# csukuangfj/kaldi-hmm-gmm

Hardware: AMD Instinct MI355X
Metric: frames/sec (whole node) per EM iter (align+acc-stats), 5k-pdf x 64-Gauss (higher is better)
Workload: dtype f32 via f16x2s

## Files before the change

### include/khg_hip.h

```cpp
#ifndef KHG_HIP_H_
#define KHG_HIP_H_
#include <stdint.h>

#ifdef __cplusplus
extern "C" {
#endif

#define KHG_OK 0
#define KHG_E_ARG (-1)
#define KHG_E_HIP (-2)
#define KHG_E_RUNTIME (-3)
#define KHG_E_UNSUPPORTED (-4)
#define KHG_MAX_DIM 512

typedef struct khg_ctx khg_ctx;
typedef struct khg_model khg_model;
typedef struct khg_tm khg_tm;
typedef struct khg_utts khg_utts;
typedef struct khg_accs khg_accs;

const char *khg_last_error(void);
int khg_version(void);

int khg_ctx_create(int device, void *stream, khg_ctx **out);
int khg_ctx_destroy(khg_ctx *ctx);
int khg_ctx_sync(khg_ctx *ctx);
int khg_ctx_set_timing(khg_ctx *ctx, int on);
int khg_ctx_get_timings(khg_ctx *ctx, char *names, int64_t names_cap, float *ms, int32_t cap,
                        int32_t *n_out);

#define KHG_K1_AUTO 0
#define KHG_K1_FP32_PDF 2
#define KHG_K1_FP32_UTT 3
#define KHG_K1_F16X2 4
#define KHG_K1_F16X2S 5
int khg_ctx_set_k1_form(khg_ctx *ctx, int form);

#define KHG_OPT_K1_FORM 0
#define KHG_OPT_K1_ORDER 1
#define KHG_OPT_K1_NF 2
#define KHG_OPT_K1P_TS 3
#define KHG_OPT_K1_INTERLEAVE 4
#define KHG_OPT_K1_DBG 5
#define KHG_OPT_K2_INORDER 6
#define KHG_OPT_K2_KS 7
#define KHG_OPT_K2_SERIAL 8
#define KHG_OPT_K2_PROF 9
#define KHG_OPT_K3_BUCKET 10
#define KHG_OPT_K3_FORM 11
#define KHG_OPT_K3_PHASE_B 12
#define KHG_OPT_K3_NY 13
#define KHG_OPT_DEBUG 14
#define KHG_OPT_K3_PHASE_A 15
#define KHG_OPT_K2_SPLIT 16
#define KHG_OPT_K2S_HUB 17
#define KHG_OPT_LAT_OPS_LDS 18
#define KHG_OPT_K1_LAUNCH 19
#define KHG_OPT_K1_PGRID 20
#define KHG_OPT_K1_PROF 21
#define KHG_OPT_COUNT 22
#define KHG_INFO_SCRATCH_BYTES 100
#define KHG_INFO_SCRATCH_BLOCKS 101
int khg_ctx_set_option(khg_ctx *ctx, int option, int value);
int khg_ctx_get_option(const khg_ctx *ctx, int option, int *value);
int khg_option_check(int option, int value);
int khg_option_from_env(const char *name, const char *text, int *option, int *value);

int khg_model_create(khg_ctx *ctx, int32_t num_pdfs, int32_t dim, const int32_t *gauss_off_h,
                     const float *gconsts_h, const float *means_invvars_h,
                     const float *inv_vars_h, khg_model **out);
int khg_model_destroy(khg_model *m);
int khg_model_invalidate(khg_model *m);

int khg_tm_create(khg_ctx *ctx, int32_t num_tids, const int32_t *id2pdf_h, khg_tm **out);
int khg_tm_set_trans_cost(khg_tm *tm, const float *trans_cost_h);
int khg_tm_destroy(khg_tm *tm);

int khg_utts_create(khg_ctx *ctx, const khg_tm *tm, int32_t n_utt, int32_t dim,
                    const int64_t *frame_off_h, const float *feats_h, const float *feats_d,
                    const int64_t *state_off_h, const int32_t *start_h, const int64_t *arc_off_h,
                    const int32_t *ilabel_h, const int32_t *olabel_h, const float *weight_h,
                    const int32_t *nextstate_h, const float *final_h, khg_utts **out);
int khg_utts_destroy(khg_utts *u);
typedef struct khg_graph khg_graph;
int khg_graph_create(khg_ctx *ctx, const khg_tm *tm, int32_t num_states, int32_t start, const int64_t *arc_off_h,
                     const int32_t *ilabel_h, const int32_t *olabel_h, const float *weight_h,
                     const int32_t *nextstate_h, const float *final_h, khg_graph **out);
int khg_graph_destroy(khg_graph *g);
int khg_graph_info(const khg_graph *g, int64_t *num_states, int64_t *num_arcs, int32_t *num_pdfs,
                   int32_t *max_in_degree, int64_t *device_bytes);
int khg_utts_create_on_graph(khg_ctx *ctx, const khg_tm *tm, khg_graph *g, int32_t n_utt, int32_t dim,
                             const int64_t *frame_off_h, const float *feats_h, const float *feats_d, khg_utts **out);
int khg_utts_graph_bytes(const khg_utts *u, int64_t *bytes);
int khg_utts_num_pdfs(const khg_utts *u, int64_t *pdf_off_h );
int khg_utts_pdfs(const khg_utts *u, int32_t *pdfs_h );
int khg_utts_k2_plan(khg_ctx *ctx, const khg_utts *u, int32_t out[8]);
int khg_utts_pdf_first(const khg_utts *u, int32_t *first_h );

int khg_loglikes(khg_ctx *ctx, const khg_model *m, khg_utts *u);
int khg_loglikes_reachable(khg_ctx *ctx, const khg_model *m, khg_utts *u);
int khg_loglikes_band(khg_ctx *ctx, const khg_model *m, khg_utts *u);
int khg_utts_pdf_last(const khg_utts *u, int32_t *last_h );
int khg_loglikes_layout(const khg_utts *u, int64_t *ll_off_h, int64_t *total);
int khg_loglikes_download(khg_ctx *ctx, const khg_utts *u, float *ll_h);
int khg_loglikes_upload(khg_ctx *ctx, khg_utts *u, const float *ll_h);
int khg_utts_set_pdf_list(khg_utts *u, int32_t n, const int32_t *pdfs_h);
int khg_utts_features_changed(khg_utts *u);

typedef struct {
  float beam;
  float retry_beam;
  int32_t careful;
  float acoustic_scale;
  int32_t max_active;
  int32_t min_active;
  float beam_delta;
  float hash_ratio;
  float like_scale;
} khg_align_config;
void khg_align_config_default(khg_align_config *c);

#define KHG_ALIGN_DONE 0
#define KHG_ALIGN_ERROR 1
#define KHG_ALIGN_RETRIED 2
#define KHG_ALIGN_EXACT_DP 4
#define KHG_ALIGN_FALLBACK 8

int khg_careful_graph(int32_t num_states, int32_t start, const int64_t *arc_off_h, const int32_t *ilabel_h,
                      const int32_t *olabel_h, const float *weight_h, const int32_t *nextstate_h, const float *final_h,
                      int32_t *out_num_states, int32_t *out_start, int64_t *out_arc_off_h, int32_t *out_ilabel_h,
                      int32_t *out_olabel_h, float *out_weight_h, int32_t *out_nextstate_h, float *out_final_h);

int khg_align(khg_ctx *ctx, const khg_tm *tm, khg_utts *u, const khg_align_config *cfg,
              int32_t *ali_h, int32_t *words_h, int64_t *words_off_h, int64_t words_cap,
              float *like_h, int32_t *status_h);
int khg_ali_upload(khg_ctx *ctx, khg_utts *u, const int32_t *ali_h);
int khg_ali_download(khg_ctx *ctx, khg_utts *u, int32_t *ali_h);

typedef struct {
  float beam;
  int32_t max_active;
  int32_t min_active;
  float lattice_beam;
  int32_t prune_interval;
  float beam_delta;
  float hash_ratio;
  float prune_scale;
  float acoustic_scale;
  int32_t allow_partial;
  int32_t scratch_per_frame;
} khg_lattice_faster_config;
void khg_lattice_faster_config_default(khg_lattice_faster_config *c);

#define KHG_LAT_SUCCEEDED 1
#define KHG_LAT_PARTIAL 2
#define KHG_LAT_SCRATCH 4
#define KHG_LAT_NO_PATH 8
#define KHG_LAT_EPS_LOOP 16
#define KHG_LAT_WORDS 32
#define KHG_LAT_NO_TRACEBACK 64

int khg_decode_lattice_faster(khg_ctx *ctx, const khg_tm *tm, khg_utts *u, const khg_lattice_faster_config *cfg,
                              int32_t *ali_h, int32_t *words_h, int64_t *words_off_h, int64_t words_cap,
                              double *like_h, int32_t *status_h);

typedef struct {
  float beam;
  float lattice_beam;
  int32_t prune_interval;
  float prune_scale;
  float acoustic_scale;
  int32_t allow_partial;
  int32_t scratch_per_frame;
} khg_lattice_simple_config;
void khg_lattice_simple_config_default(khg_lattice_simple_config *c);

#define KHG_LAT_NO_EPS_TOKEN 128
#define KHG_LAT_NAN 256

// ... 296 lines not shown
```

### kaldi_hmm_gmm_amd/_lib.py

```python
import ctypes as C
import os

import numpy as np

_HERE = os.path.dirname(os.path.abspath(__file__))
LIB_PATH = os.environ.get("KHG_LIBRARY") or os.path.join(_HERE, "libkhg_hip.so")


class KhgError(RuntimeError):
    """Mirror of the reference's std::runtime_error -> Python RuntimeError (csrc/log.h:46-53)."""


def _load():
    if not os.path.exists(LIB_PATH):
        raise ImportError(
            f"{LIB_PATH} not found: build it with `python -c 'import __graft_entry__ as g; g.build()'` "
            "(hipcc --offload-arch=gfx950). kaldi_hmm_gmm_amd has no CPU fallback."
        )
    try:
        import torch
    except ImportError:
        pass
    return C.CDLL(LIB_PATH)

# ... 41 lines not shown
class LatticeSimpleConfigC(C.Structure):
    _fields_ = [
        ("beam", C.c_float),
        ("lattice_beam", C.c_float),
        ("prune_interval", C.c_int32),
        ("prune_scale", C.c_float),
        ("acoustic_scale", C.c_float),
        ("allow_partial", C.c_int32),
        ("scratch_per_frame", C.c_int32),
    ]


class MleOptionsC(C.Structure):
    _fields_ = [
        ("min_gaussian_weight", C.c_float),
        ("min_gaussian_occupancy", C.c_float),
        ("min_variance", C.c_double),
        ("remove_low_count_gaussians", C.c_int32),
        ("variance_floor_vector", C.POINTER(C.c_double)),
    ]


class EbwOptionsC(C.Structure):
    _fields_ = [("E", C.c_double), ("tau", C.c_double)]


class EbwWeightOptionsC(C.Structure):
    _fields_ = [("min_num_count_weight_update", C.c_double), ("min_gaussian_weight", C.c_double), ("tau", C.c_double)]


class EbwResultsC(C.Structure):
    _fields_ = [("auxf_impr_gauss", C.c_double), ("count", C.c_double), ("auxf_impr_weights", C.c_double), ("floored", C.c_int32),
                ("failed", C.c_int32), ("skipped", C.c_int32), ("weights_skipped", C.c_int32)]


class FmllrOptionsC(C.Structure):
    _fields_ = [("min_count", C.c_double), ("num_iters", C.c_int32)]


class MlltOptionsC(C.Structure):
    _fields_ = [("num_iters", C.c_int32)]


class LdaOptionsC(C.Structure):
    _fields_ = [("target_dim", C.c_int32), ("remove_offset", C.c_int32), ("within_class_factor", C.c_double)]


class RescoreStatsC(C.Structure):
    _fields_ = [("arcs", C.c_int64), ("emitting_arcs", C.c_int64), ("cells", C.c_int64)]


SIGNATURES = {
    "khg_last_error": (C.c_char_p, []),
    "khg_version": (C.c_int, []),
    "khg_ctx_create": (C.c_int, [C.c_int, vp, C.POINTER(vp)]),
    "khg_ctx_destroy": (C.c_int, [vp]),
    "khg_ctx_sync": (C.c_int, [vp]),
    "khg_ctx_set_timing": (C.c_int, [vp, C.c_int]),
    "khg_ctx_set_k1_form": (C.c_int, [vp, C.c_int]),
    "khg_ctx_set_option": (C.c_int, [vp, C.c_int, C.c_int]),
    "khg_ctx_get_option": (C.c_int, [vp, C.c_int, C.POINTER(C.c_int)]),
    "khg_option_check": (C.c_int, [C.c_int, C.c_int]),
    "khg_option_from_env": (C.c_int, [C.c_char_p, C.c_char_p, C.POINTER(C.c_int), C.POINTER(C.c_int)]),
    "khg_ctx_get_timings": (C.c_int, [vp, C.c_char_p, C.c_int64, c_f32p, C.c_int32, c_i32p]),
    "khg_model_create": (C.c_int, [vp, C.c_int32, C.c_int32, c_i32p, c_f32p, c_f32p, c_f32p, C.POINTER(vp)]),
    "khg_model_destroy": (C.c_int, [vp]),
    "khg_tm_create": (C.c_int, [vp, C.c_int32, c_i32p, C.POINTER(vp)]),
    "khg_tm_set_trans_cost": (C.c_int, [vp, c_f32p]),
    "khg_tm_destroy": (C.c_int, [vp]),
    "khg_utts_create": (
        C.c_int,
        [vp, vp, C.c_int32, C.c_int32, c_i64p, c_f32p, vp, c_i64p, c_i32p, c_i64p, c_i32p, c_i32p, c_f32p, c_i32p,
         c_f32p, C.POINTER(vp)],
    ),
    "khg_utts_destroy": (C.c_int, [vp]),
    "khg_graph_create": (C.c_int, [vp, vp, C.c_int32, C.c_int32, c_i64p, c_i32p, c_i32p, c_f32p, c_i32p, c_f32p, C.POINTER(vp)]),
    "khg_graph_destroy": (C.c_int, [vp]),
    "khg_graph_info": (C.c_int, [vp, c_i64p, c_i64p, c_i32p, c_i32p, c_i64p]),
    "khg_utts_create_on_graph": (C.c_int, [vp, vp, vp, C.c_int32, C.c_int32, c_i64p, c_f32p, vp, C.POINTER(vp)]),
    "khg_utts_graph_bytes": (C.c_int, [vp, c_i64p]),
    "khg_utts_num_pdfs": (C.c_int, [vp, c_i64p]),
    "khg_utts_pdfs": (C.c_int, [vp, c_i32p]),
    "khg_utts_k2_plan": (C.c_int, [vp, vp, c_i32p]),
    "khg_utts_pdf_first": (C.c_int, [vp, c_i32p]),
    "khg_loglikes": (C.c_int, [vp, vp, vp]),
    "khg_loglikes_reachable": (C.c_int, [vp, vp, vp]),
    "khg_loglikes_band": (C.c_int, [vp, vp, vp]),
    "khg_utts_pdf_last": (C.c_int, [vp, c_i32p]),
    "khg_loglikes_layout": (C.c_int, [vp, c_i64p, c_i64p]),
    "khg_loglikes_download": (C.c_int, [vp, vp, c_f32p]),
    "khg_loglikes_upload": (C.c_int, [vp, vp, c_f32p]),
    "khg_utts_set_pdf_list": (C.c_int, [vp, C.c_int32, c_i32p]),
    "khg_utts_features_changed": (C.c_int, [vp]),
    "khg_comm_info": (C.c_int, [vp, c_i32p, c_i32p, c_i32p]),
    "khg_align_config_default": (None, [C.POINTER(AlignConfigC)]),
    "khg_align": (C.c_int, [vp, vp, vp, C.POINTER(AlignConfigC), c_i32p, c_i32p, c_i64p, C.c_int64, c_f32p, c_i32p]),
    "khg_ali_upload": (C.c_int, [vp, vp, c_i32p]),
    "khg_lattice_faster_config_default": (None, [C.POINTER(LatticeFasterConfigC)]),
    "khg_decode_lattice_faster": (C.c_int, [vp, vp, vp, C.POINTER(LatticeFasterConfigC), c_i32p, c_i32p, c_i64p, C.c_int64, c_f64p,
                                            c_i32p]),
    "khg_lattice_simple_config_default": (None, [C.POINTER(LatticeSimpleConfigC)]),
    "khg_decode_lattice_simple": (C.c_int, [vp, vp, vp, C.POINTER(LatticeSimpleConfigC), c_i32p, c_i32p, c_i64p, C.c_int64, c_f64p,
                                            c_i32p, c_i32p]),
    "khg_decode_lattice_simple_raw": (C.c_int, [vp, vp, vp, C.POINTER(LatticeSimpleConfigC), c_i32p, c_i32p, c_i64p, C.c_int64, c_f64p,
                                                c_i32p, c_i32p, C.POINTER(vp)]),
    "khg_decode_lattice_faster_raw": (C.c_int, [vp, vp, vp, C.POINTER(LatticeFasterConfigC), c_i32p, c_i32p, c_i64p, C.c_int64, c_f64p,
                                                c_i32p, C.POINTER(vp)]),
    "khg_lattices_sizes": (C.c_int, [vp, c_i64p, c_i64p]),
    "khg_lattices_download": (C.c_int, [vp, vp, c_i32p, c_i32p, c_f32p, c_f32p, c_f32p, c_i32p, c_i32p, c_i32p, c_f32p, c_f32p, c_i32p,
                                        c_i32p]),
    "khg_lattices_device_bytes": (C.c_int, [vp, c_i64p]),
    "khg_lattices_destroy": (C.c_int, [vp]),
    "khg_lattices_validate": (C.c_int, [C.c_int32, c_i64p, c_i64p, c_i32p, c_i32p, c_f32p, c_f32p, c_f32p, c_i32p, c_i32p, c_i32p, c_f32p,
                                        c_f32p, c_i32p, c_i32p]),
    "khg_lattices_upload": (C.c_int, [vp, C.c_int32, c_i64p, c_i64p, c_i32p, c_i32p, c_f32p, c_f32p, c_f32p, c_i32p, c_i32p, c_i32p, c_f32p,
                                      c_f32p, c_i32p, c_i32p, C.POINTER(vp)]),
    "khg_lattices_num_utts": (C.c_int, [vp, c_i32p]),
    "khg_lattices_ali_layout": (C.c_int, [vp, vp, c_i64p]),
    "khg_lattices_num_chunks": (C.c_int, [vp, c_i32p]),
    "khg_lattices_chunk_utts": (C.c_int, [vp, c_i32p]),
    "khg_lattices_best_path": (C.c_int, [vp, vp, C.c_int32, c_f32p, c_f32p, c_i32p, c_i32p, c_i64p, C.c_int64, c_f32p, c_i32p]),
    "khg_lattices_prune": (C.c_int, [vp, vp, C.c_float, C.c_float, C.c_float, c_i32p, C.POINTER(vp)]),
    "khg_lattices_posteriors": (C.c_int, [vp, vp, C.c_float, C.c_float, c_i32p, c_f64p, C.POINTER(vp)]),
    "khg_lattices_rescore": (C.c_int, [vp, vp, vp, vp, vp, C.c_float, C.c_int, C.POINTER(RescoreStatsC), C.POINTER(vp)]),
    "khg_lattices_op_status": (C.c_int, [vp, c_i32p]),
    "khg_lattices_boost": (C.c_int, [vp, vp, C.c_int32, c_i32p, C.c_int32, c_i32p, c_i64p, c_i32p, vp, C.c_float, C.c_float, c_i32p,
                                     C.POINTER(vp)]),
    "khg_lattices_mpe_posteriors": (C.c_int, [vp, vp, C.c_int32, c_i32p, c_i32p, C.c_int32, c_i32p, c_i64p, c_i32p, vp, C.c_int32, C.c_int32,
                                              C.c_float, C.c_float, c_i32p, c_f64p, c_f64p, C.POINTER(vp)]),
    "khg_posteriors_sizes": (C.c_int, [vp, c_i64p, c_i64p]),
    "khg_posteriors_download": (C.c_int, [vp, vp, c_i64p, c_i32p, c_f64p, c_f64p]),
    "khg_posteriors_device_bytes": (C.c_int, [vp, c_i64p]),
    "khg_posteriors_destroy": (C.c_int, [vp]),
    "khg_posteriors_validate": (C.c_int, [C.c_int32, c_i64p, c_i64p, C.c_int64, c_i32p, c_f64p]),
    "khg_posteriors_upload": (C.c_int, [vp, C.c_int32, c_i64p, c_i64p, c_i32p, c_f64p, C.POINTER(vp)]),
    "khg_ali_download": (C.c_int, [vp, vp, c_i32p]),
    "khg_accs_create": (C.c_int, [vp, vp, vp, C.POINTER(vp)]),
    "khg_accs_destroy": (C.c_int, [vp]),
    "khg_accs_zero": (C.c_int, [vp, vp]),
    "khg_accs_size": (C.c_int, [vp, c_i64p]),
    "khg_accs_device_ptr": (C.c_int, [vp, C.POINTER(vp)]),
    "khg_accs_download": (C.c_int, [vp, vp, c_f64p]),
    "khg_accs_upload": (C.c_int, [vp, vp, c_f64p]),
    "khg_acc_stats": (C.c_int, [vp, vp, vp, vp, C.c_float, vp]),
    "khg_acc_stats_post": (C.c_int, [vp, vp, vp, vp, vp, C.c_float, vp]),
    "khg_acc_stats_post2": (C.c_int, [vp, vp, vp, vp, vp, C.c_float, vp, vp]),
    "khg_accs_add": (C.c_int, [vp, vp, C.c_float, vp]),
    "khg_accs_scale": (C.c_int, [vp, vp, C.c_float]),
    "khg_accs_smooth_with_accum": (C.c_int, [vp, vp, C.c_float, vp, vp, c_i32p]),
    "khg_accs_allreduce": (C.c_int, [vp, vp, vp]),
    "khg_accs_allreduce_range": (C.c_int, [vp, vp, vp, C.c_int32, C.c_int32, vp]),
    "khg_acc_stats_reduce": (C.c_int, [vp, vp, vp, vp, C.c_float, vp, vp, C.c_int32]),
    "khg_accs_allreduce_f32": (C.c_int, [vp, vp, vp]),
    "khg_comm_unique_id": (C.c_int, [vp]),
    "khg_comm_create": (C.c_int, [vp, C.c_int32, C.c_int32, vp, C.POINTER(vp)]),
    "khg_comm_destroy": (C.c_int, [vp]),
    "khg_compute_gconsts": (C.c_int, [C.c_int32, C.c_int32, c_i32p, c_f32p, c_f32p, c_f32p, c_f32p, c_i32p]),
    "khg_mle_options_default": (None, [C.POINTER(MleOptionsC)]),
    "khg_mle_am_diag_gmm_update": (
        C.c_int,
        [C.POINTER(MleOptionsC), C.c_int32, C.c_int32, c_i32p, c_f64p, c_f64p, c_f64p, C.c_uint16, C.c_uint16, c_f32p,
         c_f32p, c_f32p, c_f32p, c_i32p, c_f32p, c_f32p, c_i32p, c_i32p, c_i32p],
    ),
    "khg_ebw_options_default": (None, [C.POINTER(EbwOptionsC)]),
    "khg_ebw_weight_options_default": (None, [C.POINTER(EbwWeightOptionsC)]),
    "khg_ebw_am_diag_gmm_update": (
# ... 104 lines not shown
```

### kaldi_hmm_gmm_amd/csrc/khg_ctx_model.hip

```cpp
#include "khg_internal.hpp"

#include <mutex>
#include "khg_k1_loglikes.hip.inc"

static thread_local std::string g_err;
extern "C" const char* khg_last_error(void) { return g_err.c_str(); }
int khg_set_error(int code, const std::string& msg) { g_err = msg; return code; }
extern "C" int khg_version(void) { return 100; }

static std::mutex g_ctx_mu;
static std::vector<khg_ctx*> g_ctxs;
static constexpr size_t KHG_ARENA_BYTES = size_t(24) << 20;
void* arena_alloc(khg_ctx* ctx, size_t bytes) {
  KhgArena& a = ctx->arena;
  if (!a.dev) {
    if (a.cap == SIZE_MAX) return nullptr;
    void *d = nullptr, *h = nullptr;
    if (hipMalloc(&d, KHG_ARENA_BYTES) != hipSuccess || hipHostMalloc(&h, KHG_ARENA_BYTES, hipHostMallocDefault) != hipSuccess) {
      if (d) (void)hipFree(d);
      (void)hipGetLastError();
      a.cap = SIZE_MAX;
      return nullptr;
    }
    a.dev = static_cast<char*>(d); a.host = static_cast<char*>(h); a.cap = KHG_ARENA_BYTES; a.top = a.base = 256;
// ... 51 lines not shown
  return false;
}
void khg_dev_free(void* p) {
  if (p && !khg_arena_release(p)) (void)hipFree(p);
}

static void ctx_defaults_from_env(khg_ctx* c);
extern "C" int khg_ctx_create(int device, void* stream, khg_ctx** out) {
  if (!out) return khg_set_error(KHG_E_ARG, "khg_ctx_create: out is NULL");
  int n = 0;
  hipError_t e = hipGetDeviceCount(&n);
  if (e != hipSuccess || n <= 0)
    return khg_set_error(KHG_E_HIP, "khg_ctx_create: no HIP device available (this library has no CPU fallback)");
  if (device < 0 || device >= n) return khg_set_error(KHG_E_ARG, "khg_ctx_create: bad device index");
  HIPCHK(hipSetDevice(device));
  hipDeviceProp_t prop;
  HIPCHK(hipGetDeviceProperties(&prop, device));
  if (std::string(prop.gcnArchName).rfind("gfx950", 0) != 0)
    return khg_set_error(KHG_E_UNSUPPORTED, std::string("khg_ctx_create: built for gfx950, device is ") + prop.gcnArchName);
  khg_ctx* c = new khg_ctx();
  c->device = device;
  if (stream) { c->stream = (hipStream_t)stream; c->own_stream = false; }
  else { HIPCHK(hipStreamCreateWithFlags(&c->stream, hipStreamNonBlocking)); c->own_stream = true; }
  for (auto& s : c->sides) HIPCHK(hipStreamCreateWithFlags(&s, hipStreamNonBlocking));
  ctx_defaults_from_env(c);
  int rc = dev_alloc(&c->err_flag_d, 1);
  if (!rc) rc = dev_alloc(&c->dump_d, 256);
  if (!rc && hipHostMalloc(reinterpret_cast<void**>(&c->err_host), 256, hipHostMallocDefault) != hipSuccess) rc = khg_set_error(KHG_E_HIP, "khg_ctx_create: hipHostMalloc failed");
  if (rc) { delete c; return rc; }
  HIPCHK(hipMemsetAsync(c->err_flag_d, 0, sizeof(int32_t), c->stream));
  { std::lock_guard<std::mutex> lk(g_ctx_mu); g_ctxs.push_back(c); }
  *out = c;
  return KHG_OK;
}
extern "C" int khg_ctx_destroy(khg_ctx* c) {
  if (!c) return KHG_OK;
  (void)hipStreamSynchronize(c->stream);
  for (auto& s : c->sides) (void)hipStreamSynchronize(s);
  {
    std::lock_guard<std::mutex> lk(g_ctx_mu);
    g_ctxs.erase(std::remove(g_ctxs.begin(), g_ctxs.end(), c), g_ctxs.end());
    if (c->arena.dev && !c->arena.blocks.empty()) {
      c->arena.dirty.clear();
      g_orphans.push_back(std::move(c->arena));
      c->arena = KhgArena();
    }
  }
  DEVFREE(c->err_flag_d); DEVFREE(c->dump_d); DEVFREE(c->k1_next_d);
  if (c->err_host) (void)hipHostFree(c->err_host);
  if (c->arena.dev) (void)hipFree(c->arena.dev);
  if (c->arena.host) (void)hipHostFree(c->arena.host);
  if (c->own_stream) (void)hipStreamDestroy(c->stream);
  for (auto& s : c->sides) (void)hipStreamDestroy(s);
  if (c->comm_stream) { (void)hipStreamSynchronize(c->comm_stream); (void)hipStreamDestroy(c->comm_stream); }
  if (c->ev_k3) (void)hipEventDestroy(c->ev_k3);
  if (c->ev_c1) (void)hipEventDestroy(c->ev_c1);
  delete c;
  return KHG_OK;
}
extern "C" int khg_ctx_set_timing(khg_ctx* c, int on) {
  if (!c) return khg_set_error(KHG_E_ARG, "ctx is NULL");
  c->timing = on != 0;
  return KHG_OK;
}
extern "C" int khg_ctx_get_timings(khg_ctx* c, char* names, int64_t names_cap, float* ms, int32_t cap, int32_t* n_out) {
  if (!c || !n_out) return khg_set_error(KHG_E_ARG, "bad arguments");
  HIPCHK(hipStreamSynchronize(c->stream));
  for (auto& s : c->sides) HIPCHK(hipStreamSynchronize(s));
  int n = 0; std::string all;
  for (auto& t : c->timings) {
    float v = 0.0f;
    (void)hipEventElapsedTime(&v, t.e0, t.e1);
    if (n < cap && ms) ms[n] = v;
    all += t.name; all += '\n';
    (void)hipEventDestroy(t.e0); (void)hipEventDestroy(t.e1);
    ++n;
  }
  c->timings.clear();
  if (names && names_cap > 0) { size_t k = std::min<size_t>(all.size(), (size_t)names_cap - 1); memcpy(names, all.data(), k); names[k] = 0; }
  *n_out = n;
  return KHG_OK;
}
static const struct { int lo, hi; } k_opt_range[KHG_OPT_COUNT] = {
  {KHG_K1_AUTO, KHG_K1_F16X2S}, {0, 4}, {0, 6}, {0, 1 << 20}, {-1, 1}, {0, 255}, {0, 1}, {0, 4}, {0, 3}, {0, 1}, {0, 2}, {0, 2}, {0, 2}, {0, 64}, {0, 1}, {0, 1}, {0, 1}, {0, 1 << 20}, {0, 1}, {0, 2}, {0, 1 << 16}, {0, 1}};
extern "C" int khg_option_check(int opt, int value) {
  if (opt < 0 || opt >= KHG_OPT_COUNT) return khg_set_error(KHG_E_ARG, "khg_option_check: no such option");
  if (value < k_opt_range[opt].lo || value > k_opt_range[opt].hi || (opt == KHG_OPT_K1_FORM && value == 1))
    return khg_set_error(KHG_E_ARG, "khg_ctx_set_option: option " + std::to_string(opt) + " takes values " + std::to_string(k_opt_range[opt].lo) + " .. " + std::to_string(k_opt_range[opt].hi));
  return KHG_OK;
}
extern "C" int khg_ctx_set_option(khg_ctx* c, int opt, int value) {
  if (!c || opt < 0 || opt >= KHG_OPT_COUNT) return khg_set_error(KHG_E_ARG, "khg_ctx_set_option: bad arguments");
  int rc = khg_option_check(opt, value);
  if (rc) return rc;
  c->opt[opt] = value;
  return KHG_OK;
}
extern "C" int khg_ctx_get_option(const khg_ctx* c, int opt, int* value) {
  if (c && value && (opt == KHG_INFO_SCRATCH_BYTES || opt == KHG_INFO_SCRATCH_BLOCKS)) {
    *value = opt == KHG_INFO_SCRATCH_BYTES ? (c->arena.dev ? (int)c->arena.top : 0) : (int)c->arena.blocks.size();
    return KHG_OK;
  }
  if (!c || !value || opt < 0 || opt >= KHG_OPT_COUNT) return khg_set_error(KHG_E_ARG, "khg_ctx_get_option: bad arguments");
  *value = c->opt[opt];
  return KHG_OK;
}
extern "C" int khg_ctx_set_k1_form(khg_ctx* c, int form) { return khg_ctx_set_option(c, KHG_OPT_K1_FORM, form); }
static const struct { const char* name; int opt; const char* words; } k_env_tab[] = {
  {"KHG_K1", KHG_OPT_K1_FORM, "auto=0,pdf=2,fp32=2,utt=3,f16x2=4,f16x2s=5"},
  {"KHG_K1_ORDER", KHG_OPT_K1_ORDER, "desc=0,none=1,asc=2,tiles=3,xcd=4"},
  {"KHG_K1_NF", KHG_OPT_K1_NF, ""}, {"KHG_K1P_TS", KHG_OPT_K1P_TS, ""}, {"KHG_K1_INTERLEAVE", KHG_OPT_K1_INTERLEAVE, ""},
  {"KHG_K1B_DBG", KHG_OPT_K1_DBG, ""}, {"KHG_K2_INORDER", KHG_OPT_K2_INORDER, ""}, {"KHG_K2_KS", KHG_OPT_K2_KS, ""},
  {"KHG_K2_SERIAL", KHG_OPT_K2_SERIAL, ""}, {"KHG_K2_PROF", KHG_OPT_K2_PROF, ""},
  {"KHG_K3_BUCKET", KHG_OPT_K3_BUCKET, "sort=0,atomic=1,count=2"}, {"KHG_K3_FORM", KHG_OPT_K3_FORM, "auto=0,block=1,valu=2"},
  {"KHG_K3_VALU", KHG_OPT_K3_FORM, "1=2"}, {"KHG_K3_PHASEB", KHG_OPT_K3_PHASE_B, "f64=0,f32=1,f16=2"},
  {"KHG_K3_NY", KHG_OPT_K3_NY, ""}, {"KHG_DEBUG", KHG_OPT_DEBUG, ""}, {"KHG_K3_PHASEA", KHG_OPT_K3_PHASE_A, "auto=0,f16=0,f32=1"},
  {"KHG_K2_SPLIT", KHG_OPT_K2_SPLIT, "on=0,off=1"}, {"KHG_K2S_HUB", KHG_OPT_K2S_HUB, ""},
  {"KHG_LAT_OPS_LDS", KHG_OPT_LAT_OPS_LDS, "on=0,off=1"},
  {"KHG_K1_LAUNCH", KHG_OPT_K1_LAUNCH, "auto=0,chunk=1,persistent=2"}, {"KHG_K1_PGRID", KHG_OPT_K1_PGRID, ""},
  {"KHG_K1_PROF", KHG_OPT_K1_PROF, ""}};
extern "C" int khg_option_from_env(const char* name, const char* text, int* option, int* value) {
  if (!name || !text || !*text || !option || !value) return khg_set_error(KHG_E_ARG, "khg_option_from_env: bad arguments");
  for (const auto& t : k_env_tab) {
    if (strcmp(t.name, name) != 0) continue;
    const char* e = text;
    int v = atoi(e);
    bool word = false;
    for (const char* w = t.words; *w;) {
      const char* eq = strchr(w, '=');
      const size_t n = (size_t)(eq - w);
      if (strlen(e) == n && strncmp(e, w, n) == 0) { v = atoi(eq + 1); word = true; break; }
      const char* comma = strchr(eq, ',');
      if (!comma) break;
      w = comma + 1;
    }
    if (!word && *t.words && !(e[0] >= '0' && e[0] <= '9') && e[0] != '-')
      return khg_set_error(KHG_E_ARG, std::string(name) + ": unknown word '" + text + "'");
    if (v < k_opt_range[t.opt].lo || v > k_opt_range[t.opt].hi)
      return khg_set_error(KHG_E_ARG, std::string(name) + " takes values " + std::to_string(k_opt_range[t.opt].lo) + " .. " + std::to_string(k_opt_range[t.opt].hi));
    *option = t.opt; *value = v;
    return KHG_OK;
  }
  return khg_set_error(KHG_E_ARG, std::string("khg_option_from_env: no such variable: ") + name);
}
static void ctx_defaults_from_env(khg_ctx* c) {
  c->opt[KHG_OPT_K1_INTERLEAVE] = -1;
  c->opt[KHG_OPT_K1P_TS] = 1024;
  c->opt[KHG_OPT_K2S_HUB] = 32;
  c->opt[KHG_OPT_K3_PHASE_B] = 2;
  for (const auto& t : k_env_tab) {
    const char* e = getenv(t.name);
    if (!e || !*e) continue;
    int opt = 0, v = 0;
    if (khg_option_from_env(t.name, e, &opt, &v) == KHG_OK) c->opt[opt] = v;
  }
}
extern "C" int khg_ctx_sync(khg_ctx* c) {
  if (!c) return khg_set_error(KHG_E_ARG, "ctx is NULL");
  return check_err_flag(c, "khg_ctx_sync");
}
int check_err_flag(khg_ctx* c, const char* where) {
  { int rf = arena_flush(c); if (rf) return rf; }
  for (int i = 0; i < khg_ctx::NSIDE; ++i)
    if (c->side_dirty[i]) { HIPCHK(hipStreamSynchronize(c->sides[i])); c->side_dirty[i] = false; }
  HIPCHK(hipMemcpyAsync(c->err_host, c->err_flag_d, sizeof(int32_t), hipMemcpyDeviceToHost, c->stream));
  HIPCHK(hipStreamSynchronize(c->stream));
  c->pageable_pending = false;
  const int32_t f = *c->err_host;
  if (f) {
    HIPCHK(hipMemsetAsync(c->err_flag_d, 0, sizeof(int32_t), c->stream));
    if (f & 1) return khg_set_error(KHG_E_RUNTIME, std::string(where) + ": Invalid answer (overflow or invalid variances/features?)");
    if (f & 2) return khg_set_error(KHG_E_RUNTIME, std::string(where) + ": internal queue overflow in the faithful decoder");
    if (f & 8) return khg_set_error(KHG_E_RUNTIME, std::string(where) + ": internal error: K3 work items exceed their bound");
    return khg_set_error(KHG_E_RUNTIME, std::string(where) + ": pdf-id out of range (graph/model mismatch)");
  }
  return KHG_OK;
}

template <int KQ>
__global__ __launch_bounds__(256) void k0_pack_tiles(const float* __restrict__ gconsts, const float* __restrict__ miv,
                                                      const float* __restrict__ iv, const int32_t* __restrict__ gauss_off,
                                                      const int32_t* __restrict__ pdf_tile_off, const int32_t* __restrict__ tile_pdf,
                                                      int D, float* __restrict__ wimg, float* __restrict__ nhiv) {
  constexpr int ROW = khg_row_floats(KQ), TILE = khg_tile_floats(KQ);
  const int t = blockIdx.x, p = tile_pdf[t];
  const int g_first = gauss_off[p] + 32 * (t - pdf_tile_off[p]);
  const int nrow = min(32, gauss_off[p + 1] - g_first);
  float* img = wimg + (size_t)t * TILE;
  for (int i = threadIdx.x; i < TILE; i += 256) {
    float v = 0.0f;
    if (i < 4 * 32 * ROW) {
      const int q = i / (32 * ROW), r = (i / ROW) & 31, s = i % ROW;
      const int d = 2 * s + (q & 1);
      if (r < nrow && d < D) {
        const size_t src = (size_t)(g_first + r) * D + d;
        v = (q & 2) ? -0.5f * iv[src] : miv[src];
      }
    } else if (i < 4 * 32 * ROW + 32) {
      const int r = i - 4 * 32 * ROW;
      v = r < nrow ? gconsts[g_first + r] : -INFINITY;
    }
    img[i] = v;
  }
// ... 271 lines not shown
```

### kaldi_hmm_gmm_amd/csrc/khg_internal.hpp

```cpp
#pragma once
#include <hip/hip_runtime.h>

#include <algorithm>
#include <climits>
#include <cmath>
#include <cstdint>
#include <cstdio>
#include <cstdlib>
#include <cstring>
#include <deque>
#include <limits>
#include <string>
#include <type_traits>
#include <utility>
#include <vector>

#include "../../include/khg_hip.h"
#include "khg_dev_types.hip.inc"

int khg_set_error(int code, const std::string& msg);

#define HIPCHK(expr)                                                                         \
  do {                                                                                       \
    hipError_t e_ = (expr);                                                                  \
// ... 86 lines not shown
    for (auto& r : readers)
      if (r.first != s) HIPCHK(hipStreamWaitEvent(s, r.second, 0));
    return KHG_OK;
  }
  int after_pack(hipStream_t s) {
    if (!packed) HIPCHK(hipEventCreateWithFlags(&packed, hipEventDisableTiming));
    HIPCHK(hipEventRecord(packed, s));
    pack_stream = s;
    return KHG_OK;
  }
  int before_read(hipStream_t s) {
    if (packed && pack_stream != s) HIPCHK(hipStreamWaitEvent(s, packed, 0));
    return KHG_OK;
  }
  int after_read(hipStream_t s) {
    for (auto& r : readers)
      if (r.first == s) { HIPCHK(hipEventRecord(r.second, s)); return KHG_OK; }
    hipEvent_t e = nullptr;
    HIPCHK(hipEventCreateWithFlags(&e, hipEventDisableTiming));
    HIPCHK(hipEventRecord(e, s));
    readers.emplace_back(s, e);
    return KHG_OK;
  }
  void destroy() {
    if (packed) (void)hipEventDestroy(packed);
    for (auto& r : readers) (void)hipEventDestroy(r.second);
    packed = nullptr; readers.clear();
  }
};

struct khg_model {
  khg_ctx* ctx = nullptr;
  uint64_t serial = 0;
  uint64_t version = 0;
  int32_t P = 0, D = 0, KQ = 0, ntiles = 0;
  int64_t sumG = 0;
  std::vector<int32_t> gauss_off, pdf_tile_off;
  float* wimg_d = nullptr;
  int32_t* pdf_tile_off_d = nullptr;
  int32_t* gauss_off_d = nullptr;
  float *gconsts_d = nullptr, *miv_d = nullptr, *iv_d = nullptr, *nhiv_d = nullptr;
  float* weights_d = nullptr;
  bool has_weights = false;
  int32_t wimg_tiles = 0;
  int32_t KS = 0;
  char* wimgh_d = nullptr;
  int32_t wimgh_tiles = 0;
  std::vector<int32_t> wimgh_ex;
  ImgSync wimgh_sync;
  char* wimgs_d = nullptr;
  int32_t wimgs_tiles = 0;
  std::vector<int32_t> wimgs_key;
  float* ubound_d = nullptr; int32_t ubound_tiles = 0; bool ubound_valid = false;
  std::vector<int32_t> xs_ex_seen;
  ImgSync wimgs_sync;
  std::vector<float> wmax;
  std::vector<float> k3_xb;
  std::vector<float> k3_xb_raw;
  uint32_t* stats_d = nullptr;
  std::vector<int32_t> k3_ex;
  int32_t k3_S = 0;
  bool k3_f16_ok = false;
  int32_t* k3_ex_d = nullptr;
  float gcmax = 0.0f;
  int32_t* tile_pdf_d = nullptr;
  K4Res* k4_res_d = nullptr;
  int32_t k4_res_P = 0;
};

struct khg_tm {
  khg_ctx* ctx = nullptr;
  int32_t num_tids = 0, max_pdf = -1;
  std::vector<int32_t> id2pdf;
  int32_t* id2pdf_d = nullptr;
  float* trans_cost_d = nullptr;
  bool has_trans_cost = false;
};

struct khg_graph {
  khg_ctx* ctx = nullptr;
  int32_t refs = 1;
  int64_t S = 0, A = 0, nwords = 0, device_bytes = 0;
  int32_t start = -1, max_indeg = 0, max_outdeg = 0;
  bool same_col = true, has_eps = false;
  std::vector<int32_t> pdfs, pdf_first, pdf_dfin;
  int64_t *state_off_d = nullptr, *in_off_d = nullptr, *out_off_d = nullptr;
  int32_t *start_d = nullptr, *in_src_d = nullptr, *in_col_d = nullptr, *in_tid_d = nullptr, *in_olabel_d = nullptr, *out_inidx_d = nullptr;
  float *in_w_d = nullptr, *final_d = nullptr;
};
void khg_graph_release(khg_graph* g);

struct khg_utts {
  khg_ctx* ctx = nullptr;
  khg_graph* graph = nullptr;
  int32_t* gidx_d = nullptr;
  int64_t graph_bytes = 0;
  bool small = false;
  int32_t n_utt = 0, D = 0;
  int64_t N = 0;
  bool has_graphs = false;
  std::vector<int64_t> frame_off, state_off, pdf_off, ll_off, bp_off, path_off, words_off;
  std::vector<int32_t> pdfs;
  int32_t max_states = 0, max_inarcs = 0, max_indeg = 0, max_outdeg = 0;
  bool same_col = true;
  int32_t pdfs_checked_P = -1;
  bool has_eps = false;
  const float* feats_d = nullptr; bool own_feats = false;
  int64_t *frame_off_d = nullptr, *state_off_d = nullptr, *pdf_off_d = nullptr, *ll_off_d = nullptr;
  int32_t *pdfs_d = nullptr, *start_d = nullptr;
  KwChunk* wchunks_d = nullptr;
  int32_t n_wchunks = 0;
  int64_t *in_off_d = nullptr, *out_off_d = nullptr;
  int32_t *in_src_d = nullptr, *in_col_d = nullptr, *in_tid_d = nullptr, *in_olabel_d = nullptr, *out_inidx_d = nullptr;
  float *in_w_d = nullptr, *final_d = nullptr;
  K1Chunk* chunks_d = nullptr; int32_t n_chunks = 0; int32_t chunk_kq = 0;
  int64_t* tile_off_d = nullptr; int32_t* tiles_d = nullptr;
  std::vector<int32_t> pdf_first;
  std::vector<int32_t> pdf_last;
  int ll_mode = 0;
  void* band_args = nullptr;
  khg_model* band_model = nullptr; int band_ks = 0; size_t band_lds = 0; uint64_t band_serial = 0, band_version = 0; std::vector<int32_t> band_key;
  int tiles_reach = -1;
  std::vector<int32_t> tiles_pto;
  float* ll_d = nullptr; int64_t ll_total = 0; bool ll_valid = false;
  float* xpl_d = nullptr; int64_t* utt_xtile_off_d = nullptr; int32_t xpl_kq = 0;
  K1pEntry* p_ents_d = nullptr; K1pSlice* p_slices_d = nullptr; int32_t p_nslices = 0; int p_reach = -1; int32_t p_P = -1;
  int32_t p_grp[10] = {0, 0, 0, 0, 0, 0, 0, 0, 0, 0};
  std::vector<int32_t> p_goff;
  int64_t* utt_x32_off_d = nullptr;
  K1bChunk* bchunks_d = nullptr; int32_t n_bchunks = 0, bchunk_nt = 0;
  int32_t* x32_utt_d = nullptr; int64_t n_x32 = 0;
  k1b_u32x4* xh_d = nullptr; int32_t xh_ks = 0; std::vector<int32_t> xh_ex; int32_t* xh_ex_d = nullptr;
  std::vector<float> xmax;
  k1b_u32x4* xs_d = nullptr; int32_t xs_ks = 0; std::vector<int32_t> xs_ex; int32_t* xs_ex_d = nullptr;
  K1sChunk* schunks_d = nullptr; int32_t n_schunks = 0, schunk_nmax = 0;
  K1sUnit* sunits_d = nullptr; std::vector<int32_t> sunits_pto; int sunits_reach = -1;
  uint8_t* bp_d = nullptr; int64_t *bp_off_d = nullptr, *path_off_d = nullptr, *words_off_d = nullptr;
  double* layer_best_d = nullptr; int32_t* layer_cnt_d = nullptr; int32_t* path_d = nullptr;
  unsigned char* k2_gscratch_d = nullptr; size_t k2_gscratch_bytes = 0;
  int32_t* k2_order_d = nullptr;
  int32_t *ali_d = nullptr, *words_d = nullptr, *num_words_d = nullptr, *status_d = nullptr;
  float* like_d = nullptr;
  bool ali_valid = false;
  char* out_blk_d = nullptr; size_t out_blk_bytes = 0;
  hipEvent_t ev_dp = nullptr, ev_ali = nullptr;
  bool ali_pending = false;
  int32_t *ali2_d = nullptr, *unc_d = nullptr, *unc_cnt_h = nullptr, *unc_cnt_dev = nullptr;
  int64_t* sub_off_d = nullptr;
  bool ali_split = false;
  int32_t *pdf_count_d = nullptr, *pdf_cursor_d = nullptr, *frame_ids_d = nullptr;
  uint32_t *sort_keys_d = nullptr, *sort_keys_out_d = nullptr, *sort_vals_d = nullptr; void* sort_tmp_d = nullptr; size_t sort_tmp_bytes = 0;
  int32_t* cs_hist_d = nullptr; size_t cs_hist_n = 0; int64_t* cs_tot_d = nullptr; size_t cs_tot_n = 0;
  double *k3_part_d = nullptr, *k3_llpart_d = nullptr; size_t k3_part_n = 0, k3_llpart_n = 0;
  void* k3_items_d = nullptr; int32_t* k3_item_off_d = nullptr; size_t k3_items_n = 0, k3_item_off_n = 0;
  int64_t* pdf_start_d = nullptr; unsigned long long* tid_count_d = nullptr;
  int32_t k3_P = 0, k3_tids = 0;
  int32_t *pe_row_d = nullptr, *pe_tid_d = nullptr, *pe_ids_d = nullptr; float* pe_w_d = nullptr; size_t pe_cap = 0;
  uint32_t *pe_keys_d = nullptr, *pe_keys_out_d = nullptr, *pe_vals_d = nullptr; void* pe_tmp_d = nullptr; size_t pe_tmp_bytes = 0;
  int64_t* pe_start_d = nullptr; int32_t pe_P = 0;
  uint64_t *rc_keys_d = nullptr, *rc_keys_out_d = nullptr; uint32_t *rc_vals_d = nullptr, *rc_vals_out_d = nullptr;
  int32_t *rc_flag_d = nullptr, *rc_inc_d = nullptr, *rc_row_d = nullptr; float* rc_cell_d = nullptr; size_t rc_cap = 0;
  void* rc_tmp_d = nullptr; size_t rc_tmp_bytes = 0;
  int32_t *rc_cell_start_d = nullptr, *rc_item_off_d = nullptr; int64_t* rc_stats_d = nullptr; int32_t rc_P = -1;
};

static inline int64_t utt_states(const khg_utts* u, int i) { return u->graph ? u->state_off[1] : u->state_off[(size_t)i + 1] - u->state_off[(size_t)i]; }

struct khg_accs {
  khg_ctx* ctx = nullptr;
  int64_t sumG = 0; int32_t D = 0, num_tids = 0;
  int64_t n = 0, cap = 0;
  double* buf_d = nullptr;
  float* wire_d = nullptr; int64_t wire_cap = 0;
  double* occ() const { return buf_d; }
  double* mean() const { return buf_d + sumG; }
  double* var() const { return buf_d + sumG + sumG * D; }
  double* trans() const { return buf_d + sumG + 2 * sumG * D; }
  double* scalars() const { return trans() + num_tids + 1; }
};

constexpr size_t KHG_ARENA_MAX_REQ = size_t(4) << 20;
template <class T>
inline int u_alloc(khg_utts* u, T** p, size_t n) {
  if (n == 0) n = 1;
  if (u->small && n * sizeof(T) <= KHG_ARENA_MAX_REQ) {
    *p = static_cast<T*>(arena_alloc(u->ctx, n * sizeof(T)));
    if (*p) return KHG_OK;
// ... 49 lines not shown
```

### kaldi_hmm_gmm_amd/csrc/khg_k2.hip

```cpp
#include "khg_internal.hpp"

#include "khg_k2_hashlist.hip.inc"
#include "khg_k2_viterbi.hip.inc"

extern "C" void khg_align_config_default(khg_align_config* c) {
  c->beam = 200.0f; c->retry_beam = 0.0f; c->careful = 0; c->acoustic_scale = 1.0f;
  c->max_active = INT32_MAX; c->min_active = 20; c->beam_delta = 0.5f; c->hash_ratio = 2.0f;
  c->like_scale = 0.0f;
}

static int ensure_ali(khg_ctx* ctx, khg_utts* u) {
  if (u->ali_d) return KHG_OK;
  if (u->small && u->has_graphs) {
    const size_t nu = (size_t)u->n_utt, nw = (size_t)u->words_off[u->n_utt];
    const size_t bytes = 4 * (3 * nu + nw + (size_t)u->N) + 64;
    int rc = u_alloc(u, &u->out_blk_d, bytes);
    if (rc) return rc;
    u->out_blk_bytes = bytes;
    int32_t* p = reinterpret_cast<int32_t*>(u->out_blk_d);
    u->status_d = p; u->like_d = reinterpret_cast<float*>(p + nu); u->num_words_d = p + 2 * nu; u->words_d = p + 3 * nu; u->ali_d = p + 3 * nu + nw;
    return KHG_OK;
  }
  return u_alloc(u, &u->ali_d, (size_t)u->N);
}

struct K2Plan {
  int KS = 1, DEG = 1;
  bool FAST = false, GMEM = false, SC = false;
  int nthr = 64;
  size_t lds_dp = 0;
  size_t max_npdf = 0;
  int faithful = 0;
  int odeg_w = 0, odeg_c = 1;
  size_t lds_f = 0, lds_w_mut = 0, lds_w_graph = 0, lds_chain = 0;
  size_t gscratch_stride = 0;
};

static K2Plan k2_plan(const khg_ctx* ctx, const khg_utts* u) {
  K2Plan p;
  const size_t S = (size_t)u->max_states, A = (size_t)u->max_inarcs;
  size_t max_npdf = 0;
  for (int i = 0; i < u->n_utt; ++i) max_npdf = std::max<size_t>(max_npdf, (size_t)(u->pdf_off[i + 1] - u->pdf_off[i]));
  p.max_npdf = max_npdf;
  int nthr = (int)std::min<size_t>(1024, (S + 63) / 64 * 64);
  const int ks_force = ctx->opt[KHG_OPT_K2_KS];
  if (ks_force == 2 || ks_force == 4) nthr = (int)std::min<size_t>(1024, ((S + ks_force - 1) / ks_force + 63) / 64 * 64);
  p.nthr = nthr;
  const size_t nwave = nthr / 64;
  const bool deg6 = !u->has_eps && u->max_indeg > 3 && u->max_indeg <= 6 && S <= 1024;
  const bool fast = deg6 || (!u->has_eps && u->max_indeg <= 3 && S <= 4096);
  const int KSsel = !fast ? 0 : ((ks_force == 2 || ks_force == 4) && !deg6 && S <= (size_t)1024 * ks_force ? ks_force : (S <= 1024 ? 1 : (S <= 2048 ? 2 : 4)));
  const size_t NSl = fast ? KSsel : 1;
  const size_t tb_bytes = fast ? std::max<size_t>(5 * (size_t)nthr * NSl * 4, 2560 * nwave) : (K2_FB + 1) * ((S + 15) & ~size_t(15));
  size_t lds_dp = 16 * S + 8 * K2_MAXW + 8 * A + 4 * (S + 1) + 8 * K2_FB * nwave + 32 + 8 * K2_MAXW + 16 +
                  std::max<size_t>(fast ? 0 : 4 * K2_SB * (max_npdf | 1), tb_bytes) + 64;
  size_t HB = std::max<size_t>(2 * S, 1000);
  const size_t lds_f = 32 * S + 8 * HB + 4 * (S + A) + 4 * S + 4 * (S + 1) + 16 * A + A + 64;
  const int odeg_w = u->max_outdeg <= 8 ? std::max(1, (int)u->max_outdeg) : 0;
  const bool use_pos = u->has_eps || S > 1000;
  const size_t lds_w_mut = 16 * S + 8 * S + 4 * 4 * S + 4 * S + 4 * max_npdf + (odeg_w ? 0 : 4 * A + 4 * S) + (use_pos ? 4 * S : 0) +
                           (u->has_eps ? 4 * (S + A + 1) : 0) + 8 + 8 * ((std::max(A, S * (size_t)odeg_w) + 63) / 64 + 1);
  const size_t lds_w_graph = 8 * (S + 1) + 5 * 4 * A + (u->has_eps ? 4 * (S + 1) + 4 * A : 0) + A + S + 64;
  const int fmode = ctx->opt[KHG_OPT_K2_SERIAL];
  const int odeg_c = (int)std::max<int32_t>(1, u->max_outdeg);
  const size_t S4 = (S + 3) & ~size_t(3);
  const size_t lds_chain = std::max<size_t>(36 * S4 + 21 * S4 * (size_t)odeg_c + 4 * max_npdf,
                                            4 * (S4 + 1) + 2 * A + 16 + 9 * ((S + 15) & ~size_t(15))) + 128;
  const bool chain = fmode == 0 && !u->has_eps && S <= 1000 && u->max_outdeg <= 4 && lds_chain <= 64 * 1024 && max_npdf <= 32767;
  const bool wave_lds = (fmode == 0 || fmode == 3) && S <= 65535 && lds_w_mut + lds_w_graph <= 160 * 1024;
  const bool wave_gm = fmode != 1 && !wave_lds && S <= 65535 && lds_w_mut <= 160 * 1024;
  const bool lane_gm = !wave_lds && !wave_gm && lds_f > 160 * 1024;
  p.faithful = chain ? 4 : wave_gm ? 3 : wave_lds ? 2 : lane_gm ? 1 : 0;
  p.odeg_w = odeg_w; p.odeg_c = odeg_c;
  p.lds_f = lds_f; p.lds_w_mut = lds_w_mut; p.lds_w_graph = lds_w_graph; p.lds_chain = lds_chain;
  const bool gmem = lds_dp > 160 * 1024;
  if (gmem)
    lds_dp = 16 * S + 8 * K2_MAXW + 8 * A + 4 * (S + 1) + 8 * K2_FB * nwave + 32 + 8 * K2_MAXW + 16 +
             std::max<size_t>(4 * K2_SB * (max_npdf | 1), (K2_FB + 1) * ((S + 15) & ~size_t(15))) + 64;
  p.lds_dp = lds_dp;
  if (gmem || wave_gm || lane_gm)
    p.gscratch_stride = (std::max(gmem ? lds_dp : 0, std::max(wave_gm ? lds_w_graph : 0, lane_gm ? lds_f : 0)) + 255) & ~size_t(255);
  if (gmem) { p.GMEM = true; return p; }
  const bool deg2 = fast && !deg6 && KSsel == 1 && u->max_indeg <= 2 && ctx->opt[KHG_OPT_K2_KS] != 3;
  const bool sc2 = deg2 && u->same_col;
  const bool sc3 = fast && !deg6 && !deg2 && KSsel == 1 && u->same_col && ctx->opt[KHG_OPT_K2_KS] != 3;
  const bool deg2m = fast && !deg6 && KSsel > 1 && u->max_indeg <= 2;
  auto form = [&](int ks, int deg, bool sc) { p.KS = ks; p.DEG = deg; p.FAST = true; p.SC = sc; };
  if (deg6) form(1, 6, false);
  else if (sc2) form(1, 2, true);
  else if (deg2) form(1, 2, false);
  else if (sc3) form(1, 3, true);
  else if (KSsel == 1) form(1, 3, false);
  else if (KSsel == 2 && deg2m && u->same_col) form(2, 2, true);
  else if (KSsel == 2 && deg2m) form(2, 2, false);
  else if (KSsel == 2) form(2, 3, false);
  else if (KSsel == 4 && deg2m && u->same_col) form(4, 2, true);
  else if (KSsel == 4 && deg2m) form(4, 2, false);
  else if (KSsel == 4) form(4, 3, false);
  return p;
}

extern "C" int khg_utts_k2_plan(khg_ctx* ctx, const khg_utts* u, int32_t out[8]) {
  if (ctx_dead(ctx) || !u || !out) return khg_set_error(KHG_E_ARG, "khg_utts_k2_plan: bad arguments");
  { int rf = utts_foreign_ctx(ctx, u, "khg_utts_k2_plan"); if (rf) return rf; }
  if (!u->has_graphs) return khg_set_error(KHG_E_ARG, "khg_utts_k2_plan: the utterance set has no decoding graphs");
  const K2Plan p = k2_plan(ctx, u);
  out[0] = p.KS; out[1] = p.DEG; out[2] = p.FAST ? 1 : 0; out[3] = p.GMEM ? 1 : 0; out[4] = p.SC ? 1 : 0;
  out[5] = p.nthr; out[6] = p.GMEM ? 0 : (int32_t)p.lds_dp; out[7] = p.faithful;
  return KHG_OK;
}

extern "C" int khg_align(khg_ctx* ctx, const khg_tm* tm, khg_utts* u, const khg_align_config* cfg,
                         int32_t* ali_h, int32_t* words_h, int64_t* words_off_h, int64_t words_cap,
                         float* like_h, int32_t* status_h) {
  if (ctx_dead(ctx) || !tm || !u || !cfg) return khg_set_error(KHG_E_ARG, "khg_align: bad arguments");
  { int rf = utts_foreign_ctx(ctx, u, "khg_align"); if (rf) return rf; }
  if (!u->has_graphs) return khg_set_error(KHG_E_ARG, "khg_align: the utterance set has no decoding graphs");
  if (!u->ll_valid) return khg_set_error(KHG_E_ARG, "khg_align: call khg_loglikes first");
  if (u->max_states > 65535)
    return khg_set_error(KHG_E_UNSUPPORTED, "khg_align: more than 65535 states in one decoding graph (" + std::to_string(u->max_states) + "); the aligner's limit");
  if (u->max_indeg > 254)
    return khg_set_error(KHG_E_UNSUPPORTED, "khg_align: a state has more than 254 incoming arcs (" + std::to_string(u->max_indeg) + "); the aligner's limit");
  if ((cfg->retry_beam != 0 && cfg->retry_beam <= cfg->beam) || cfg->beam <= 0.0)
    return khg_set_error(KHG_E_RUNTIME, "Beams do not make sense: beam " + std::to_string(cfg->beam) + ", retry-beam " + std::to_string(cfg->retry_beam));
  if (!(cfg->hash_ratio >= 1.0) || !(cfg->max_active > 1) || !(cfg->min_active >= 0 && cfg->min_active < cfg->max_active))
    return khg_set_error(KHG_E_RUNTIME, "FasterDecoderOptions assertion failed");
  int rc = wait_ali(ctx, u);
  if (!rc) rc = k1_band_check(ctx, u);
  if (!rc) rc = ensure_ali(ctx, u);
  if (rc) return rc;
  if (!u->bp_d) {
    rc = u_alloc(u, &u->bp_d, (size_t)u->bp_off[u->n_utt]);
    if (!rc) rc = u_alloc(u, &u->layer_best_d, (size_t)(u->N + u->n_utt));
    if (!rc) rc = u_alloc(u, &u->layer_cnt_d, (size_t)(u->N + u->n_utt));
    if (!rc) rc = u_alloc(u, &u->path_d, (size_t)u->path_off[u->n_utt]);
    if (!rc && !u->out_blk_d) {
      rc = u_alloc(u, &u->words_d, (size_t)u->words_off[u->n_utt]);
      if (!rc) rc = u_alloc(u, &u->num_words_d, (size_t)u->n_utt);
      if (!rc) rc = u_alloc(u, &u->status_d, (size_t)u->n_utt);
      if (!rc) rc = u_alloc(u, &u->like_d, (size_t)u->n_utt);
    }
    if (rc) return rc;
  }
  rc = arena_flush(ctx);
  if (rc) return rc;
  HIPCHK(hipMemsetAsync(u->ali_d, 0, sizeof(int32_t) * (size_t)u->N, ctx->stream));
  K2Args a;
  a.frame_off = u->frame_off_d; a.gidx = u->gidx_d; a.state_off = u->state_off_d; a.start = u->start_d;
  a.in_off = u->in_off_d; a.in_src = u->in_src_d; a.in_col = u->in_col_d; a.in_tid = u->in_tid_d;
  a.in_olabel = u->in_olabel_d; a.in_w = u->in_w_d; a.out_off = u->out_off_d; a.out_inidx = u->out_inidx_d;
  a.final_w = u->final_d; a.trans_cost = tm->has_trans_cost ? tm->trans_cost_d : nullptr;
  a.ll = u->ll_d; a.ll_off = u->ll_off_d;
  a.bp = u->bp_d; a.bp_off = u->bp_off_d; a.layer_best = u->layer_best_d; a.layer_cnt = u->layer_cnt_d;
  a.path = u->path_d; a.path_off = u->path_off_d;
  a.ali = u->ali_d; a.ali_fb = u->ali_d; a.unc = nullptr; a.unc_cnt = nullptr; a.words = u->words_d; a.words_off = u->words_off_d; a.num_words = u->num_words_d;
  a.like = u->like_d; a.status = u->status_d; a.err_flag = ctx->err_flag_d;
  a.prof = nullptr;
  if (!u->k2_order_d && u->n_utt > 1) {
    std::vector<int32_t> ord((size_t)u->n_utt);
    for (int i = 0; i < u->n_utt; ++i) ord[(size_t)i] = i;
    std::stable_sort(ord.begin(), ord.end(), [&](int32_t x, int32_t y) {
      return u->frame_off[x + 1] - u->frame_off[x] > u->frame_off[y + 1] - u->frame_off[y];
    });
    int rc2 = u_upload(ctx, u, &u->k2_order_d, ord);
    if (!rc2) rc2 = sync_pageable(ctx);
    if (rc2) return rc2;
  }
  a.order = ctx->opt[KHG_OPT_K2_INORDER] ? nullptr : u->k2_order_d;
  const bool split = !(ali_h || like_h || status_h || words_h) && u->n_utt > 64 && !u->small && ctx->opt[KHG_OPT_K2_SPLIT] == 0;
  if (split) {
    if (!u->ali2_d) {
      rc = u_alloc(u, &u->ali2_d, (size_t)u->N);
      if (!rc) rc = u_alloc(u, &u->unc_d, (size_t)u->n_utt + 2);
      if (rc) return rc;
      u->unc_cnt_dev = u->unc_d + u->n_utt;
      HIPCHK(hipHostMalloc(reinterpret_cast<void**>(&u->unc_cnt_h), 64, 0));
    }
    HIPCHK(hipMemsetAsync(u->unc_d, 0, sizeof(int32_t) * ((size_t)u->n_utt + 2), ctx->stream));
    a.ali_fb = u->ali2_d; a.unc = u->unc_d; a.unc_cnt = u->unc_cnt_dev;
  }
  const bool k2prof = ctx->opt[KHG_OPT_K2_PROF] != 0;
  if (k2prof) { HIPCHK(hipMalloc(reinterpret_cast<void**>(&a.prof), sizeof(long long) * 16 * (size_t)u->n_utt)); HIPCHK(hipMemset(a.prof, 0, sizeof(long long) * 16 * (size_t)u->n_utt)); }
  a.beam = cfg->beam; a.retry_beam = cfg->retry_beam; a.acoustic_scale = cfg->acoustic_scale;
  a.like_scale = cfg->like_scale != 0.0f ? cfg->like_scale : cfg->acoustic_scale;
  a.beam_delta = cfg->beam_delta; a.hash_ratio = cfg->hash_ratio;
  a.max_active = cfg->max_active; a.min_active = cfg->min_active;
  a.max_states = u->max_states; a.max_inarcs = u->max_inarcs;
  const K2Plan plan = k2_plan(ctx, u);
  const int nthr = plan.nthr;
  const size_t lds_dp = plan.lds_dp, max_npdf = plan.max_npdf;
  a.gscratch = nullptr; a.gscratch_stride = 0;
  if (plan.gscratch_stride) {
    const size_t need = plan.gscratch_stride * (size_t)u->n_utt;
    if (need > u->k2_gscratch_bytes) {
      DEVFREE(u->k2_gscratch_d);
      { int rg = u_alloc(u, &u->k2_gscratch_d, need); if (rg) return rg; }
      u->k2_gscratch_bytes = need;
    }
    a.gscratch = u->k2_gscratch_d; a.gscratch_stride = (int64_t)plan.gscratch_stride;
  }
  if (plan.GMEM) {
    KernelTimer kt(ctx, "k2_viterbi_dp");
    KHG_LAUNCH(ctx, (k2_viterbi_dp<1, 1, false, true>), dim3(u->n_utt), dim3(nthr), 0, ctx->stream, a);
  } else {
    const int form = plan.FAST ? 100 * plan.KS + 10 * plan.DEG + (plan.SC ? 1 : 0) : 0;
#define K2_DP_CASES(X)                                                                                         \
    if (form == 160) X((k2_viterbi_dp<1, 6, true>));                                                           \
    else if (form == 121) X((k2_viterbi_dp<1, 2, true, false, true>));                                         \
    else if (form == 120) X((k2_viterbi_dp<1, 2, true>));                                                      \
    else if (form == 131) X((k2_viterbi_dp<1, 3, true, false, true>));                                         \
    else if (form == 130) X((k2_viterbi_dp<1, 3, true>));                                                      \
    else if (form == 221) X((k2_viterbi_dp<2, 2, true, false, true>));                                         \
    else if (form == 220) X((k2_viterbi_dp<2, 2, true>));                                                      \
    else if (form == 230) X((k2_viterbi_dp<2, 3, true>));                                                      \
    else if (form == 421) X((k2_viterbi_dp<4, 2, true, false, true>));                                         \
    else if (form == 420) X((k2_viterbi_dp<4, 2, true>));                                                      \
    else if (form == 430) X((k2_viterbi_dp<4, 3, true>));                                                      \
    else X((k2_viterbi_dp<1, 1, false>));
#define K2_SET_LDS(FN) HIPCHK(hipFuncSetAttribute((const void*)FN, hipFuncAttributeMaxDynamicSharedMemorySize, (int)lds_dp))
#define K2_LAUNCH(FN) KHG_LAUNCH(ctx, FN, dim3(u->n_utt), dim3(nthr), lds_dp, ctx->stream, a)
    if (lds_dp > 48 * 1024) { K2_DP_CASES(K2_SET_LDS) }
    KernelTimer kt(ctx, "k2_viterbi_dp");
    K2_DP_CASES(K2_LAUNCH)
#undef K2_LAUNCH
#undef K2_SET_LDS
#undef K2_DP_CASES
  }
  HIPCHK(hipGetLastError());
  const bool sync_call = ali_h || like_h || status_h || words_h;
  hipStream_t side = ctx->stream;
  if (!sync_call) {
    if (!u->ev_dp) { HIPCHK(hipEventCreateWithFlags(&u->ev_dp, hipEventDisableTiming)); HIPCHK(hipEventCreateWithFlags(&u->ev_ali, hipEventDisableTiming)); }
    if (split) HIPCHK(hipMemcpyAsync(u->unc_cnt_h, u->unc_cnt_dev, 2 * sizeof(int32_t), hipMemcpyDeviceToHost, ctx->stream));
    HIPCHK(hipEventRecord(u->ev_dp, ctx->stream));
    side = ctx->sides[ctx->next_side];
    ctx->side_dirty[ctx->next_side] = true;
    ctx->next_side = (ctx->next_side + 1) % khg_ctx::NSIDE;
    HIPCHK(hipStreamWaitEvent(side, u->ev_dp, 0));
  }
  rc = k1_band_repair(ctx, u, u->status_d, K2_ST_NEED_FALLBACK, side);
  if (rc) return rc;
  {
    KernelTimer kt(ctx, "k2_viterbi_faithful", side);
    if (plan.faithful == 4) {
#define K2_CHAIN(OD)                                                                                                            \
  do {                                                                                                                          \
    if (plan.lds_chain > 48 * 1024) HIPCHK(hipFuncSetAttribute((const void*)k2_viterbi_faithful_chain<OD>, hipFuncAttributeMaxDynamicSharedMemorySize, (int)plan.lds_chain)); \
    KHG_LAUNCH(ctx, k2_viterbi_faithful_chain<OD>, dim3(u->n_utt), dim3(64), plan.lds_chain, side, a, (int)max_npdf);                \
  } while (0)
      switch (plan.odeg_c) { case 1: K2_CHAIN(1); break; case 2: K2_CHAIN(2); break; case 3: K2_CHAIN(3); break; default: K2_CHAIN(4); break; }
#undef K2_CHAIN
    } else if (plan.faithful == 3) {
      if (plan.lds_w_mut > 48 * 1024) HIPCHK(hipFuncSetAttribute((const void*)k2_viterbi_faithful_wave<true>, hipFuncAttributeMaxDynamicSharedMemorySize, (int)plan.lds_w_mut));
      KHG_LAUNCH(ctx, k2_viterbi_faithful_wave<true>, dim3(u->n_utt), dim3(64), plan.lds_w_mut, side, a, u->has_eps ? 1 : 0, plan.odeg_w, (int)max_npdf);
    } else if (plan.faithful == 2) {
      const size_t lds_w = plan.lds_w_mut + plan.lds_w_graph;
      if (lds_w > 48 * 1024) HIPCHK(hipFuncSetAttribute((const void*)k2_viterbi_faithful_wave<false>, hipFuncAttributeMaxDynamicSharedMemorySize, (int)lds_w));
      KHG_LAUNCH(ctx, k2_viterbi_faithful_wave<false>, dim3(u->n_utt), dim3(64), lds_w, side, a, u->has_eps ? 1 : 0, plan.odeg_w, (int)max_npdf);
    } else if (plan.faithful == 1) {
      KHG_LAUNCH(ctx, k2_viterbi_faithful<true>, dim3(u->n_utt), dim3(64), 0, side, a);
    } else {
      if (plan.lds_f > 48 * 1024) HIPCHK(hipFuncSetAttribute((const void*)k2_viterbi_faithful<false>, hipFuncAttributeMaxDynamicSharedMemorySize, (int)plan.lds_f));
      KHG_LAUNCH(ctx, k2_viterbi_faithful<false>, dim3(u->n_utt), dim3(64), plan.lds_f, side, a);
    }
  }
  HIPCHK(hipGetLastError());
  if (!sync_call) { HIPCHK(hipEventRecord(u->ev_ali, side)); u->ali_pending = true; }
  u->ali_split = split;
  u->ali_valid = true;
  if (k2prof) {
    std::vector<long long> pr(16 * (size_t)u->n_utt);
    HIPCHK(hipStreamSynchronize(ctx->stream));
    HIPCHK(hipStreamSynchronize(side));
    HIPCHK(hipMemcpy(pr.data(), a.prof, pr.size() * 8, hipMemcpyDeviceToHost));
    (void)hipFree(a.prof);
    double ph[4] = {0, 0, 0, 0}, sT = 0, sS = 0, sf = 0; int n = 0;
    for (int i = 0; i < u->n_utt; ++i) if (pr[i * 8 + 4]) { for (int k = 0; k < 4; ++k) ph[k] += (double)(pr[i * 8 + k + 1] - pr[i * 8 + k]); sT += pr[i * 8 + 5]; sS += pr[i * 8 + 6]; sf += pr[i * 8 + 7]; ++n; }
    if (n) fprintf(stderr, "[KHG_K2_PROF] %d utts, avg T %.1f S %.1f fast %.2f threads %d lds %zu | ticks: setup %.0f forward %.0f traceback %.0f replay %.0f\n",
                   n, sT / n, sS / n, sf / n, nthr, lds_dp, ph[0] / n, ph[1] / n, ph[2] / n, ph[3] / n);
    const long long* pc = pr.data() + 8 * (size_t)u->n_utt;
    double cs[3] = {0, 0, 0}, cf = 0, cp[3] = {0, 0, 0}; int nc = 0;
    for (int i = 0; i < u->n_utt; ++i) if (pc[i * 8 + 3]) { for (int k = 0; k < 3; ++k) { cs[k] += (double)(pc[i * 8 + k + 1] - pc[i * 8 + k]); cp[k] += (double)pc[i * 8 + 5 + k]; } cf += (double)pc[i * 8 + 4]; ++nc; }
    if (nc) fprintf(stderr, "[KHG_K2_PROF] chain decoder: %d utts, avg frames decoded %.1f | ticks: setup %.0f frames %.0f (%.1f per frame: GetCutoff %.1f, pass 1 %.1f, pass 2 %.1f, rest = row flush + score staging) finish %.0f\n",
                    nc, cf / nc, cs[0] / nc, cs[1] / nc, cs[1] / std::max(1.0, cf), cp[0] / std::max(1.0, cf), cp[1] / std::max(1.0, cf), cp[2] / std::max(1.0, cf), cs[2] / nc);
  }
  if (!ali_h && !like_h && !status_h && !words_h) return KHG_OK;
  rc = wait_ali(ctx, u);
  if (rc) return rc;
  if (u->out_blk_d && ctx->arena.owns(u->out_blk_d)) {
    char* hm = ctx->arena.mirror(u->out_blk_d);
// ... 76 lines not shown
```

### kaldi_hmm_gmm_amd/csrc/khg_k2_viterbi.hip.inc

```

struct K2Args {
  const int64_t* frame_off;
  const int32_t* gidx;
  const int64_t* state_off;
  const int32_t* start;
  const int64_t* in_off;
  const int32_t* in_src;
  const int32_t* in_col;
  const int32_t* in_tid;
  const int32_t* in_olabel;
  const float* in_w;
  const int64_t* out_off;
  const int32_t* out_inidx;
  const float* final_w;
  const float* trans_cost;
  const float* ll;
  const int64_t* ll_off;
  uint8_t* bp;
  const int64_t* bp_off;
  double* layer_best;
  int32_t* layer_cnt;
  int32_t* path;
  const int64_t* path_off;
  int32_t* ali;
// ... 54 lines not shown
    if (n >= path_cap) { overflow = true; break; }
    path[n++] = ai;
    if (s_col[ai] >= 0) --layer;
    s = s_src[ai];
  }
  if (overflow || layer != 0) return KHG_ALIGN_ERROR;

  double cost = 0.0;
  float v1 = 0.0f, v2 = 0.0f;
  int t = 0, nw = 0;
  const int64_t wcap = a.words_off[u + 1] - a.words_off[u];
  int32_t* words = a.words + a.words_off[u];
  bool ok = true;
  const double beam = (double)a.beam;
  auto node_ok = [&](double c, int L) {
    if (c < lbest[L] + beam) return true;
    return lcnt[L] <= a.min_active && (L == 0 || lcnt[L - 1] <= a.min_active);
  };
  if (certify) ok = node_ok(0.0, 0);
  for (int i = n - 1; i >= 0; --i) {
    int ai = path[i];
    float w = s_w[ai];
    double ncost;
    int col = s_col[ai];
    if (col >= 0) {
      float ac = -1 * (a.acoustic_scale * llu[(int64_t)col * tpad + t]);
      ncost = (cost + w) + ac;
      a.ali_fb[f0 + t] = a.in_tid[in0 + ai];
      ++t;
    } else {
      ncost = cost + w;
    }
    float tot_cost = (float)(ncost - cost);
    float ac_cost = tot_cost - w;
    v1 = w + v1;
    v2 = ac_cost + v2;
    int ol = a.in_olabel[in0 + ai];
    if (ol != 0) { if (nw < wcap) words[nw] = ol; ++nw; }
    cost = ncost;
    if (certify && ok) ok = node_ok(cost, t);
  }
  v1 = a.final_w[a.state_off[a.gidx[u]] + best_state] + v1;
  v2 = 0.0f + v2;
  a.num_words[u] = nw;
  a.like[u] = -(v1 + v2) / a.like_scale;
  if (certified) *certified = ok;
  if (nw > wcap) return KHG_ALIGN_ERROR;
  return KHG_ALIGN_DONE;
}

struct K2Arc { uint16_t src; int16_t col; float w; };

#define K2_FB 32
#define K2_SB 16
#define K2_MAXW 16

__device__ __forceinline__ void k2_lds_sync() {
  asm volatile("s_waitcnt lgkmcnt(0)" ::: "memory");
  __builtin_amdgcn_wave_barrier();
}
__device__ __forceinline__ void k2_block_sync() {
  asm volatile("s_waitcnt lgkmcnt(0)\n\ts_barrier" ::: "memory");
}
__device__ __forceinline__ void k2_global_sync() {
  asm volatile("s_waitcnt vmcnt(0) lgkmcnt(0)" ::: "memory");
  __builtin_amdgcn_wave_barrier();
}
__device__ __forceinline__ float k2_wave_minf_lane63(float v) {
  asm volatile("s_nop 1\n\t"
               "v_min_f32_dpp %0, %0, %0 row_ror:8 row_mask:0xf bank_mask:0xf\n\ts_nop 1\n\t"
               "v_min_f32_dpp %0, %0, %0 row_ror:4 row_mask:0xf bank_mask:0xf\n\ts_nop 1\n\t"
               "v_min_f32_dpp %0, %0, %0 row_ror:2 row_mask:0xf bank_mask:0xf\n\ts_nop 1\n\t"
               "v_min_f32_dpp %0, %0, %0 row_ror:1 row_mask:0xf bank_mask:0xf\n\ts_nop 1\n\t"
               "v_min_f32_dpp %0, %0, %0 row_bcast:15 row_mask:0xa bank_mask:0xf\n\ts_nop 1\n\t"
               "v_min_f32_dpp %0, %0, %0 row_bcast:31 row_mask:0xc bank_mask:0xf\n\ts_nop 1"
               : "+v"(v));
  return v;
}
__device__ __forceinline__ double k2_wave_min(double v) {
#pragma unroll
  for (int o = 32; o > 0; o >>= 1) { double t = __shfl_xor(v, o); v = t < v ? t : v; }
  return v;
}
__device__ __forceinline__ int k2_wave_sum(int v) {
#pragma unroll
  for (int o = 32; o > 0; o >>= 1) v += __shfl_xor(v, o);
  return v;
}
__device__ __forceinline__ float k2_round_down(double d) {
  float f = (float)d;
  if ((double)f > d) f = __int_as_float(__float_as_int(f) + (f > 0.0f ? -1 : (f < 0.0f ? 1 : (int)0x80000001)));
  return f;
}

template <int DEG, int NB>
__device__ __forceinline__ void k2_decode_nibble(int nib, int& ord, int& tie) {
  if constexpr (DEG == 2) { ord = (nib & 1) ? 0 : ((nib & 2) ? 1 : (1 << NB) - 1); tie = (nib & 3) == 3 ? 1 : 0; }
  else { ord = nib & ((1 << NB) - 1); tie = (nib >> NB) & 1; }
}

template <int KS, int DEG, bool FAST, bool GMEM = false, bool SC = false>
__global__ __attribute__((amdgpu_waves_per_eu(KS == 1 ? K2_WAVES_PER_EU : 4))) void k2_viterbi_dp(K2Args a) {
  extern __shared__ __attribute__((aligned(16))) unsigned char k2_lds[];
  unsigned char* const smem = GMEM ? a.gscratch + (size_t)blockIdx.x * a.gscratch_stride : k2_lds;
  constexpr int NS = FAST ? KS : 1;
  constexpr int NSD = FAST ? KS * DEG : 1;
  constexpr int NB = DEG <= 3 ? 2 : 3;
  constexpr int BNONE = (1 << NB) - 1;
  const int u = a.order ? a.order[blockIdx.x] : (int)blockIdx.x;
  const int tid = threadIdx.x, lane = tid & 63;
  const int nthr = min((int)blockDim.x, max(64, (((int)(a.state_off[a.gidx[u] + 1] - a.state_off[a.gidx[u]]) + (FAST ? KS : 1) - 1) / (FAST ? KS : 1) + 63) & ~63));
  if (tid >= nthr) return;
  const int wave = __builtin_amdgcn_readfirstlane(tid >> 6), nwave = nthr >> 6;
  const int64_t f0 = a.frame_off[u];
  const int T = (int)(a.frame_off[u + 1] - f0);
  const int tpad = (T + 31) & ~31;
  const int64_t s0 = a.state_off[a.gidx[u]];
  const int S = (int)(a.state_off[a.gidx[u] + 1] - s0);
  const int64_t in0 = a.in_off[s0];
  const int A = (int)(a.in_off[s0 + S] - in0);
  const int start = a.start[a.gidx[u]];
  const int npdf = (int)((a.ll_off[u + 1] - a.ll_off[u]) / (tpad > 0 ? tpad : 1));
  const int PP = npdf | 1;
  const int Sp = (S + 15) & ~15;
  const int GW = FAST ? nthr * KS : 0;
  const int LB = Sp;

  double* cur = reinterpret_cast<double*>(smem);
  double* nxt = cur + a.max_states;
  double* s_red = nxt + a.max_states;
  K2Arc* s_arc = reinterpret_cast<K2Arc*>(s_red + K2_MAXW);
  int32_t* s_in_off = reinterpret_cast<int32_t*>(s_arc + a.max_inarcs);
  float* s_wmin = reinterpret_cast<float*>(s_in_off + a.max_states + 1);
  int32_t* s_wcnt = reinterpret_cast<int32_t*>(s_wmin + K2_FB * nwave);
  int32_t* s_flags = s_wcnt + K2_FB * nwave;
  int32_t* s_redi = s_flags + 8;
  float* s_ac = reinterpret_cast<float*>(smem + (((reinterpret_cast<unsigned char*>(s_redi + 2 * K2_MAXW) - smem) + 15) & ~ptrdiff_t(15)));
  uint8_t* s_bp = reinterpret_cast<uint8_t*>(s_ac);

  if (tid == 0) { a.num_words[u] = 0; a.like[u] = 0.0f; }
  if (start < 0 || S == 0) {
    if (tid == 0) a.status[u] = KHG_ALIGN_ERROR;
    return;
  }
  if (a.prof && tid == 0) a.prof[u * 8 + 0] = clock64();
  if (tid < 8) s_flags[tid] = 0;
  for (int s = tid; s <= S; s += nthr) s_in_off[s] = (int32_t)(a.in_off[s0 + s] - in0);
  k2_block_sync();
  for (int i = tid; i < A; i += nthr) {
    int col = a.in_col[in0 + i];
    int tidl = a.in_tid[in0 + i];
    float w = a.in_w[in0 + i];
    if (a.trans_cost && tidl >= 1) w = w + a.trans_cost[tidl];
    s_arc[i] = K2Arc{(uint16_t)a.in_src[in0 + i], (int16_t)col, w};
    if (col < 0) s_flags[1] = 1;
  }
  for (int s = tid; s < S; s += nthr) cur[s] = (s == start) ? 0.0 : INFINITY;
  k2_block_sync();
  const bool has_eps = !FAST && s_flags[1] != 0;
  const float* llu = a.ll + a.ll_off[u];
  uint8_t* bp = a.bp + a.bp_off[u];
  double* lbest = a.layer_best + f0 + u;
  int32_t* lcnt = a.layer_cnt + f0 + u;

  int e_src[NSD], e_col[NSD];
  double e_w[NSD];
  const bool have_ll = npdf > 0 && T > 0;
  if (FAST) {
#pragma unroll
    for (int k = 0; k < NS; ++k) {
      const int sk = tid + nthr * k;
      const int ib = sk < S ? s_in_off[sk] : 0, ie = sk < S ? s_in_off[sk + 1] : 0;
#pragma unroll
      for (int j = 0; j < DEG; ++j) {
        const bool v = ib + j < ie;
        K2Arc ar = s_arc[v ? ib + j : 0];
        e_src[k * DEG + j] = v ? ar.src : 0;
        e_col[k * DEG + j] = v ? ar.col : 0;
        e_w[k * DEG + j] = v ? (double)ar.w : (double)INFINITY;
      }
    }
  } else {
    for (int s = tid; s < S; s += nthr) bp[s] = K2_BP_NONE;
  }
  if (a.prof && tid == 0) a.prof[u * 8 + 1] = clock64();
  int tie = 0;
  const double* g_even[NSD]; const double* g_odd[NSD];
  double* st_even[NS]; double* st_odd[NS];
#pragma unroll
  for (int i = 0; i < NSD; ++i) { g_even[i] = cur + (FAST ? e_src[i] : 0); g_odd[i] = nxt + (FAST ? e_src[i] : 0); }
#pragma unroll
  for (int k = 0; k < NS; ++k) { const int sk = min(tid + nthr * k, S > 0 ? S - 1 : 0); st_even[k] = nxt + sk; st_odd[k] = cur + sk; }
  double mine[NS];
  unsigned bpw[NS];
#pragma unroll
  for (int k = 0; k < NS; ++k) bpw[k] = 0u;
#pragma unroll
  for (int k = 0; k < NS; ++k) mine[k] = (tid + nthr * k == start) ? 0.0 : INFINITY;
  int mine_live[NS];
#pragma unroll
  for (int k = 0; k < NS; ++k) mine_live[k] = (tid + nthr * k == start) ? 1 : 0;
  constexpr int NSC = SC ? (FAST ? KS : 1) : NSD;
  f32x4 sc_a[NSC], sc_b[NSC];
  constexpr bool SC3 = FAST && NSC == 1;
  f32x4 sc_c[NSC];
  if (FAST) {
#pragma unroll
    for (int i = 0; i < NSC; ++i) {
      sc_a[i] = have_ll ? *reinterpret_cast<const f32x4*>(llu + (int64_t)e_col[SC ? i * DEG : i] * tpad) : f32x4{0, 0, 0, 0};
      sc_b[i] = f32x4{0, 0, 0, 0};
      sc_c[i] = (SC3 && have_ll) ? *reinterpret_cast<const f32x4*>(llu + (int64_t)e_col[SC ? i * DEG : i] * tpad + 4) : f32x4{0, 0, 0, 0};
    }
  }

  auto layer_step = [&](const int layer, auto subc) -> bool {
    constexpr int SUB8 = decltype(subc)::value;
    constexpr int SUB = SUB8 & 3;
    uint8_t* bpl = bp + (int64_t)layer * Sp;
    if (has_eps) {
      for (int it = 0; it <= S + 1; ++it) {
        if (tid == 0) s_flags[2] = 0;
        k2_block_sync();
        for (int s = tid; s < S; s += nthr) {
          double best = cur[s];
          int barg = -1;
          for (int i = s_in_off[s]; i < s_in_off[s + 1]; ++i) {
            K2Arc ar = s_arc[i];
            if (ar.col >= 0) continue;
            double c = cur[ar.src];
            if (c == INFINITY) continue;
            double nw = c + ar.w;
            if (nw < best) { best = nw; barg = i - s_in_off[s]; }
            else if (nw == best && (barg >= 0 ? barg : (int)bpl[s]) != i - s_in_off[s]) tie = 1;
          }
          nxt[s] = best;
          if (barg >= 0) { bpl[s] = (uint8_t)barg; s_flags[2] = 1; }
        }
        k2_block_sync();
        for (int s = tid; s < S; s += nthr) cur[s] = nxt[s];
        const int changed = s_flags[2];
        k2_block_sync();
        if (!changed) break;
      }
    }
    {
      double lm = INFINITY;
      int lc = 0;
      if (FAST) {
#pragma unroll
        for (int k = 0; k < NS; ++k) { lc += mine_live[k]; lm = k == 0 ? mine[0] : (mine[k] < lm ? mine[k] : lm); }
      } else {
        for (int s = tid; s < S; s += nthr) { double c = cur[s]; if (c != INFINITY) { ++lc; if (c < lm) lm = c; } }
      }
      const int slot = layer & (K2_FB - 1);
      if constexpr (FAST) {
        float* pm = s_ac + wave * 640;
        uint8_t* pc = reinterpret_cast<uint8_t*>(pm + 512);
        pm[(layer & 7) * 64 + lane] = (float)lm;
        pc[(layer & 7) * 64 + lane] = (uint8_t)lc;
        if ((layer & 7) == 7 || layer == T) {
          k2_lds_sync();
          const int ly = lane >> 3, sub = lane & 7;
          const f32x4 m0 = *reinterpret_cast<const f32x4*>(pm + ly * 64 + sub * 8), m1 = *reinterpret_cast<const f32x4*>(pm + ly * 64 + sub * 8 + 4);
          const uint2 cb = *reinterpret_cast<const uint2*>(pc + ly * 64 + sub * 8);
          auto vmin = [](float x, float y) { float r; asm("v_min_f32 %0, %1, %2" : "=v"(r) : "v"(x), "v"(y)); return r; };
          float m = vmin(vmin(vmin(m0[0], m0[1]), vmin(m0[2], m0[3])), vmin(vmin(m1[0], m1[1]), vmin(m1[2], m1[3])));
          int cn = (int)__builtin_amdgcn_sad_u8(cb.y, 0u, __builtin_amdgcn_sad_u8(cb.x, 0u, 0u));
          m = vmin(m, __int_as_float(__builtin_amdgcn_update_dpp(0, __float_as_int(m), 0xB1, 0xf, 0xf, false)));
          cn += __builtin_amdgcn_update_dpp(0, cn, 0xB1, 0xf, 0xf, false);
          m = vmin(m, __int_as_float(__builtin_amdgcn_update_dpp(0, __float_as_int(m), 0x4E, 0xf, 0xf, false)));
          cn += __builtin_amdgcn_update_dpp(0, cn, 0x4E, 0xf, 0xf, false);
          m = vmin(m, __int_as_float(__builtin_amdgcn_update_dpp(0, __float_as_int(m), 0x141, 0xf, 0xf, false)));
          cn += __builtin_amdgcn_update_dpp(0, cn, 0x141, 0xf, 0xf, false);
          if (sub == 0 && ly <= (layer & 7)) {
            const int sl = (layer & ~7 & (K2_FB - 1)) + ly;
            s_wmin[sl * nwave + wave] = m; s_wcnt[sl * nwave + wave] = cn;
          }
          k2_lds_sync();
        }
      } else {
        const float wm = k2_wave_minf_lane63((float)lm);
        const int wc = k2_wave_sum(lc);
        if (lane == 63) { s_wmin[slot * nwave + wave] = wm; s_wcnt[slot * nwave + wave] = wc; }
      }
      if (slot == K2_FB - 1 || layer == T) {
        k2_block_sync();
        if (tid <= slot) {
          float m = INFINITY; int cn = 0;
          for (int w2 = 0; w2 < nwave; ++w2) { m = fminf(m, s_wmin[tid * nwave + w2]); cn += s_wcnt[tid * nwave + w2]; }
          if (m == INFINITY) { if (cn > 0) m = 3.402823466e38f; }
          else m = __int_as_float(__float_as_int(m) + (m > 0.0f ? -1 : (m < 0.0f ? 1 : (int)0x80000001)));
          lbest[layer - slot + tid] = (double)m;
          lcnt[layer - slot + tid] = cn;
        }
      }
    }
    if (layer == T) return false;
    if (FAST) {
      if constexpr (SC3) {
        if constexpr (SUB8 == 0) {
#pragma unroll
          for (int i = 0; i < NSC; ++i) sc_b[i] = sc_c[i];
        }
        if constexpr (SUB8 == 4) {
#pragma unroll
          for (int i = 0; i < NSC; ++i)
            if (have_ll && layer + 4 < tpad) {
              const float* src = llu + (int64_t)e_col[SC ? i * DEG : i] * tpad + layer + 4;
              sc_a[i] = *reinterpret_cast<const f32x4*>(src);
              sc_c[i] = *reinterpret_cast<const f32x4*>(src + 4);
            }
        }
      } else if (SUB == 0) {
#pragma unroll
        for (int i = 0; i < NSC; ++i)
          if (have_ll && layer + 4 < tpad) {
            const f32x4 v = *reinterpret_cast<const f32x4*>(llu + (int64_t)e_col[SC ? i * DEG : i] * tpad + layer + 4);
            if constexpr ((SUB8 & 4) != 0) sc_a[i] = v; else sc_b[i] = v;
          }
      }
      double cc[NSD];
#pragma unroll
      for (int i = 0; i < NSD; ++i) cc[i] = (SUB & 1) ? *g_odd[i] : *g_even[i];
#pragma unroll
      for (int k = 0; k < NS; ++k) {
        double nwv[DEG];
#pragma unroll
        for (int j = 0; j < DEG; ++j) {
          const int i = k * DEG + j;
          const int si = SC ? k : i;
          float sc;
          if constexpr ((SUB8 & 4) != 0) sc = sc_b[si][SUB]; else sc = sc_a[si][SUB];
          const float ac = -1 * (a.acoustic_scale * sc);
          nwv[j] = (cc[i] + e_w[i]) + ac;
        }
        double best = INFINITY;
#pragma unroll
        for (int j = 0; j < DEG; ++j) best = __builtin_fmin(best, nwv[j]);
        const bool live = __double2hiint(best) != 0x7FF00000;
        int code;
        if constexpr (DEG == 2) {
          const bool e0 = live && nwv[0] == best, e1 = live && nwv[1] == best;
          code = (e0 ? 1 : 0) | (e1 ? 2 : 0);
        } else {
          int barg = BNONE, neq = 0;
#pragma unroll
          for (int j = DEG - 1; j >= 0; --j) {
            const bool e = nwv[j] == best;
            barg = e ? j : barg;
            neq += e ? 1 : 0;
          }
          barg = live ? barg : BNONE;
          const int ctie = (live && neq > 1) ? 1 : 0;
          code = barg | (ctie << NB);
        }
        const int sk = tid + nthr * k;
        if (sk < S) *((SUB & 1) ? st_odd[k] : st_even[k]) = best;
        mine[k] = best;
        mine_live[k] = live ? 1 : 0;
        bpw[k] = (bpw[k] >> 4) | ((unsigned)code << 28);
        const int lb = layer + 1;
        if ((lb & 7) == 7 || lb == T) {
          const unsigned wv = (lb & 7) == 7 ? bpw[k] : bpw[k] >> (4 * (7 - (lb & 7)));
          reinterpret_cast<unsigned*>(bp)[(int64_t)(lb >> 3) * GW + sk] = wv;
        }
      }
    } else {
      if ((layer & (K2_SB - 1)) == 0) {
        k2_block_sync();
        const int tt = tid & (K2_SB - 1), hh = tid / K2_SB, nh = nthr / K2_SB;
        for (int c0 = 0; c0 < npdf; c0 += 8 * nh) {
          float v[8];
#pragma unroll
          for (int k = 0; k < 8; ++k) {
            const int col = c0 + nh * k + hh;
            v[k] = col < npdf ? llu[(int64_t)col * tpad + layer + tt] : 0.0f;
          }
#pragma unroll
          for (int k = 0; k < 8; ++k) {
            const int col = c0 + nh * k + hh;
            if (col < npdf) s_ac[tt * PP + col] = -1 * (a.acoustic_scale * v[k]);
          }
        }
        k2_block_sync();
      }
      const float* acr = s_ac + (layer & (K2_SB - 1)) * PP;
      uint8_t* bpn = bp + (int64_t)(layer + 1) * Sp;
      for (int s = tid; s < S; s += nthr) {
        double best = INFINITY;
        int barg = K2_BP_NONE;
        const int ib = s_in_off[s], ie = s_in_off[s + 1];
        for (int i = ib; i < ie; ++i) {
          K2Arc ar = s_arc[i];
          if (ar.col < 0) continue;
          double c = cur[ar.src];
          if (c == INFINITY) continue;
          double nw = (c + ar.w) + acr[ar.col];
          if (nw < best) { best = nw; barg = i - ib; }
          else if (nw == best) tie = 1;
        }
        nxt[s] = best;
        bpn[s] = (uint8_t)barg;
      }
    }
    k2_block_sync();
    double* tsw = cur; cur = nxt; nxt = tsw;
    return true;
  };
  if constexpr (FAST) {
    for (int base = 0; base <= T; base += 8) {
      if (!layer_step(base, std::integral_constant<int, 0>{})) break;
      if (!layer_step(base + 1, std::integral_constant<int, 1>{})) break;
      if (!layer_step(base + 2, std::integral_constant<int, 2>{})) break;
      if (!layer_step(base + 3, std::integral_constant<int, 3>{})) break;
      if (!layer_step(base + 4, std::integral_constant<int, 4>{})) break;
      if (!layer_step(base + 5, std::integral_constant<int, 5>{})) break;
      if (!layer_step(base + 6, std::integral_constant<int, 6>{})) break;
      if (!layer_step(base + 7, std::integral_constant<int, 7>{})) break;
    }
  } else {
    for (int layer = 0; layer <= T; ++layer)
      if (!layer_step(layer, std::integral_constant<int, 0>{})) break;
  }
  {
    double bc = INFINITY;
    int bs = INT32_MAX;
    for (int s = tid; s < S; s += nthr) {
      double c = cur[s] + a.final_w[s0 + s];
      if (c != INFINITY && c < bc) { bc = c; bs = s; }
    }
    const double g = k2_wave_min(bc);
    int nb = 0;
    if (g != INFINITY) {
      for (int s = tid; s < S; s += nthr) { double c = cur[s] + a.final_w[s0 + s]; if (c == g) { ++nb; if (s < bs || bc != g) { bs = s; bc = g; } } }
    }
    if (bc != g || g == INFINITY) bs = INT32_MAX;
#pragma unroll
    for (int o = 32; o > 0; o >>= 1) { int t2 = __shfl_xor(bs, o); bs = t2 < bs ? t2 : bs; }
    nb = k2_wave_sum(nb);
    if (tie) s_flags[0] = 1;
    if (lane == 0) { s_red[wave] = g; s_redi[2 * wave] = bs; s_redi[2 * wave + 1] = nb; }
  }
  asm volatile("s_waitcnt vmcnt(0)" ::: "memory");
  k2_block_sync();
  if (a.prof && tid == 0) a.prof[u * 8 + 2] = clock64();
  if (wave != 0) return;
  int best_state = -1;
  {
    double g = INFINITY;
    for (int w2 = 0; w2 < nwave; ++w2) if (s_red[w2] < g) g = s_red[w2];
    int nb = 0;
    if (g != INFINITY)
      for (int w2 = 0; w2 < nwave; ++w2) if (s_red[w2] == g) { nb += s_redi[2 * w2 + 1]; if (best_state < 0 || s_redi[2 * w2] < best_state) best_state = s_redi[2 * w2]; }
    tie = s_flags[0] != 0 || nb > 1;
  }
  if (best_state < 0) {
    for (int t = lane; t < T; t += 64) a.ali[f0 + t] = 0;
    if (lane == 0) a.status[u] = KHG_ALIGN_ERROR | (a.retry_beam != 0.0f ? KHG_ALIGN_RETRIED : 0);
    return;
  }
  int32_t* path = a.path + a.path_off[u];
  const int path_cap = (int)(a.path_off[u + 1] - a.path_off[u]);
  int n = 0, st = best_state, bad = 0, ptie = 0;
  k2_global_sync();
  bool traced = false;
  if constexpr (FAST) {
    if (S <= 256 && T <= path_cap) {
      traced = true;
      const unsigned* W = reinterpret_cast<const unsigned*>(bp);
      const uint32_t* arcw = reinterpret_cast<const uint32_t*>(s_arc);
      auto trace = [&](auto nslot_c) {
        constexpr int NSLOT = decltype(nslot_c)::value;
        int ioff[NSLOT];
        unsigned w[NSLOT], wn[NSLOT];
        int g = T >> 3;
#pragma unroll
        for (int q = 0; q < NSLOT; ++q) {
          const int sq = lane + 64 * q;
          ioff[q] = sq < S ? s_in_off[sq] : 0;
          w[q] = W[(int64_t)g * GW + min(sq, GW - 1)];
          wn[q] = 0u;
        }
        int sst = __builtin_amdgcn_readfirstlane(st);
        for (; g >= 0 && !bad; --g) {
          if (g > 0) {
#pragma unroll
            for (int q = 0; q < NSLOT; ++q) wn[q] = W[(int64_t)(g - 1) * GW + min(lane + 64 * q, GW - 1)];
          }
          int aiv[8][NSLOT], srcv[8][NSLOT];
#pragma unroll
          for (int k = 0; k < 8; ++k)
#pragma unroll
// ... 899 lines not shown
  int st = best_state, bad = 0;
  for (int hi = T; hi > 0 && !bad; ) {
    const int lo = hi > K2_TB ? hi - K2_TB : 0;
    const int nv = (hi - lo) * (Sp >> 4);
    const uint4* src = reinterpret_cast<const uint4*>(bp + (int64_t)(lo + 1) * Sp);
    uint4* dst = reinterpret_cast<uint4*>(stage);
    for (int i0 = 0; i0 < nv; i0 += 256) {
      uint4 v[4];
#pragma unroll
      for (int k = 0; k < 4; ++k) { const int i = i0 + 64 * k + lane; if (i < nv) v[k] = src[i]; }
#pragma unroll
      for (int k = 0; k < 4; ++k) { const int i = i0 + 64 * k + lane; if (i < nv) dst[i] = v[k]; }
    }
    k2_lds_sync();
    int mine = 0;
    for (int layer = hi; layer > lo; --layer) {
      const int ord = stage[(layer - lo - 1) * Sp + st];
      if (ord == K2_BP_NONE) { bad = 1; break; }
      const int ai = s_in_off[st] + ord;
      if (lane == hi - layer) mine = ai;
      st = s_src[ai];
    }
    if (!bad && lane < hi - lo) path[T - hi + lane] = mine;
    hi = lo;
    k2_lds_sync();
  }
  if (bad) return KHG_ALIGN_ERROR;
  const int n = T;
  k2_global_sync();
  double cost = 0.0;
  float v1 = 0.0f, v2 = 0.0f;
  int nw = 0;
  const int64_t wcap = a.words_off[u + 1] - a.words_off[u];
  int32_t* words = a.words + a.words_off[u];
  for (int base = n - 1; base >= 0; base -= 64) {
    const int idx = base - lane;
    const int tf = n - 1 - base + lane;
    int ol = 0; float w = 0.0f, ac = 0.0f;
    if (idx >= 0) {
      const int ai = path[idx];
      const int tidl = a.in_tid[in0 + ai];
      w = a.in_w[in0 + ai];
      if (a.trans_cost && tidl >= 1) w = w + a.trans_cost[tidl];
      ol = a.in_olabel[in0 + ai];
      ac = -1 * (a.acoustic_scale * llu[(int64_t)a.in_col[in0 + ai] * tpad + tf]);
      a.ali_fb[f0 + tf] = tidl;
    }
    const int cnt = base >= 63 ? 64 : base + 1;
    const double cost_in = cost;
    double ca = 0.0;
    for (int k = 0; k < cnt; ++k) {
      const float wk = __int_as_float(__builtin_amdgcn_readlane(__float_as_int(w), k));
      const float ack = __int_as_float(__builtin_amdgcn_readlane(__float_as_int(ac), k));
      const double ncost = (cost + wk) + ack;
      ca = lane == k ? ncost : ca;
      cost = ncost;
    }
    double cb = __shfl_up(ca, 1);
    if (lane == 0) cb = cost_in;
    const bool mine = idx >= 0;
    const float tot_cost = (float)(ca - cb);
    const float ac_cost = tot_cost - w;
    {
      const unsigned long long wm = __ballot(mine && ol != 0);
      if (mine && ol != 0) { const int pos = nw + __popcll(wm & ((1ull << lane) - 1ull)); if (pos < wcap) words[pos] = ol; }
      nw += __popcll(wm);
    }
    for (int k = 0; k < cnt; ++k) {
      v1 = __int_as_float(__builtin_amdgcn_readlane(__float_as_int(w), k)) + v1;
      v2 = __int_as_float(__builtin_amdgcn_readlane(__float_as_int(ac_cost), k)) + v2;
    }
  }
  v1 = a.final_w[a.state_off[a.gidx[u]] + best_state] + v1;
  v2 = 0.0f + v2;
  if (lane == 0) {
    a.num_words[u] = nw;
    a.like[u] = -(v1 + v2) / a.like_scale;
  }
  return nw > wcap ? KHG_ALIGN_ERROR : KHG_ALIGN_DONE;
}

struct K2ChainArc { float w; int16_t col; uint16_t dst; };

template <int CTRL, int ROWMASK>
__device__ __forceinline__ double k2_dpp_d(double old, double v) {
  const int lo = __builtin_amdgcn_update_dpp(__double2loint(old), __double2loint(v), CTRL, ROWMASK, 0xf, false);
  const int hi = __builtin_amdgcn_update_dpp(__double2hiint(old), __double2hiint(v), CTRL, ROWMASK, 0xf, false);
  return __hiloint2double(hi, lo);
}
__device__ __forceinline__ double k2_scan_min_d(double v) {
  const double inf = INFINITY;
  v = __builtin_fmin(v, k2_dpp_d<0x111, 0xf>(inf, v));
  v = __builtin_fmin(v, k2_dpp_d<0x112, 0xf>(inf, v));
  v = __builtin_fmin(v, k2_dpp_d<0x114, 0xf>(inf, v));
  v = __builtin_fmin(v, k2_dpp_d<0x118, 0xf>(inf, v));
  v = __builtin_fmin(v, k2_dpp_d<0x142, 0xa>(inf, v));
  v = __builtin_fmin(v, k2_dpp_d<0x143, 0xc>(inf, v));
  return v;
}
__device__ __forceinline__ double k2_lane63_d(double v) {
  return __hiloint2double(__builtin_amdgcn_readlane(__double2hiint(v), 63), __builtin_amdgcn_readlane(__double2loint(v), 63));
}
__device__ __forceinline__ int k2_wave_min_i(int v) {
  v = min(v, __builtin_amdgcn_update_dpp(INT32_MAX, v, 0x111, 0xf, 0xf, false));
  v = min(v, __builtin_amdgcn_update_dpp(INT32_MAX, v, 0x112, 0xf, 0xf, false));
  v = min(v, __builtin_amdgcn_update_dpp(INT32_MAX, v, 0x114, 0xf, 0xf, false));
  v = min(v, __builtin_amdgcn_update_dpp(INT32_MAX, v, 0x118, 0xf, 0xf, false));
  v = min(v, __builtin_amdgcn_update_dpp(INT32_MAX, v, 0x142, 0xa, 0xf, false));
  v = min(v, __builtin_amdgcn_update_dpp(INT32_MAX, v, 0x143, 0xc, 0xf, false));
  return __builtin_amdgcn_readlane(v, 63);
}

template <int ODEG>
__global__ __launch_bounds__(64) void k2_viterbi_faithful_chain(K2Args a, int maxp) {
  extern __shared__ __attribute__((aligned(16))) unsigned char k2_lds[];
  unsigned char* const smem = k2_lds;
  const int u = blockIdx.x;
  if (a.status[u] != K2_ST_NEED_FALLBACK) return;
  const int lane = threadIdx.x;
  const int64_t f0 = a.frame_off[u];
  const int T = (int)(a.frame_off[u + 1] - f0);
  const int tpad = (T + 31) & ~31;
  const int64_t s0 = a.state_off[a.gidx[u]];
  const int S = (int)(a.state_off[a.gidx[u] + 1] - s0);
  const int64_t in0 = a.in_off[s0];
  const int A = (int)(a.in_off[s0 + S] - in0);
  const int64_t o0 = a.out_off[s0];
  const int start = a.start[a.gidx[u]];
  const float* llu = a.ll + a.ll_off[u];
  uint8_t* bp = a.bp + a.bp_off[u];
  const int Sp = (S + 15) & ~15;
  const int MS = (a.max_states + 3) & ~3, MA = a.max_inarcs;
  const int P = tpad > 0 ? (int)((a.ll_off[u + 1] - a.ll_off[u]) / tpad) : 0;

  double* tkc0 = reinterpret_cast<double*>(smem);
  double* tkc1 = tkc0 + MS;
  unsigned long long* st_key = reinterpret_cast<unsigned long long*>(tkc1 + MS);
  double* sl_cost = reinterpret_cast<double*>(st_key + MS);
  K2ChainArc* oarc = reinterpret_cast<K2ChainArc*>(sl_cost + MS * ODEG);
  int32_t* sl_info = reinterpret_cast<int32_t*>(oarc + MS * ODEG);
  float* tmp = reinterpret_cast<float*>(sl_info);
  int32_t* st_first = sl_info + MS * ODEG;
  int32_t* st_win = st_first + MS;
  float* sc = reinterpret_cast<float*>(st_win + MS);
  uint16_t* tks0 = reinterpret_cast<uint16_t*>(sc + maxp);
  uint16_t* tks1 = tks0 + MS;
  uint8_t* o_ord = reinterpret_cast<uint8_t*>(tks1 + MS);
  int32_t* s_in_off = reinterpret_cast<int32_t*>(smem);
  uint16_t* s_src = reinterpret_cast<uint16_t*>(s_in_off + MS + 1);
  uint8_t* stage = smem + (((reinterpret_cast<unsigned char*>(s_src + MA) - smem) + 15) & ~ptrdiff_t(15));
  long long* const prof = a.prof ? a.prof + 8 * ((size_t)gridDim.x + (size_t)u) : nullptr;
  int prof_frames = 0;
  long long pt[4] = {0, 0, 0, 0}, p0 = 0;
#define K2C_STAMP(k) do { if (prof) { const long long now_ = clock64(); pt[k] += now_ - p0; p0 = now_; } } while (0)
  if (prof && lane == 0) prof[0] = clock64();
  for (int s = lane; s <= S; s += 64) s_in_off[s] = (int32_t)(a.in_off[s0 + s] - in0);
  k2_lds_sync();
  for (int s = lane; s < S; s += 64) {
    const int ob = (int)(a.out_off[s0 + s] - o0), oe = (int)(a.out_off[s0 + s + 1] - o0);
#pragma unroll
    for (int j = 0; j < ODEG; ++j) {
      K2ChainArc r{INFINITY, (int16_t)-1, (uint16_t)0};
      int ord = 0;
      if (ob + j < oe) {
        const int ai = a.out_inidx[o0 + ob + j];
        int lo = 0, hi = S - 1;
        while (lo < hi) { const int mid = (lo + hi + 1) >> 1; if (s_in_off[mid] <= ai) lo = mid; else hi = mid - 1; }
        const int tidl = a.in_tid[in0 + ai];
        float w = a.in_w[in0 + ai];
        if (a.trans_cost && tidl >= 1) w = w + a.trans_cost[tidl];
        r = K2ChainArc{w, (int16_t)a.in_col[in0 + ai], (uint16_t)lo};
        ord = ai - s_in_off[lo];
// ... 252 lines not shown
```

### kaldi_hmm_gmm_amd/csrc/khg_pybind.cpp

```cpp
#include <chrono>

#include <pybind11/numpy.h>
#include <pybind11/pybind11.h>
#include <pybind11/stl.h>

#include <cstdint>
#include <cstring>
#include <limits>
#include <string>
#include <vector>

#include "../../include/khg_hip.h"
#include "khg_py_ebw.hpp"
#include "khg_py_lattices.hpp"

namespace py = pybind11;

namespace {

py::object g_khg_error;

void Check(int rc) {
  if (rc == KHG_OK) return;
  const char* msg = khg_last_error();
  if (g_khg_error && !g_khg_error.is_none()) {
    PyErr_SetString(g_khg_error.ptr(), msg ? msg : "khg error");
    throw py::error_already_set();
  }
  throw std::runtime_error(msg ? msg : "khg error");
}

template <class F>
int NoGil(F&& f) {
  py::gil_scoped_release release;
  return f();
}

template <class T>
using Arr = py::array_t<T, py::array::c_style | py::array::forcecast>;

template <class T>
Arr<T> Zeros(std::vector<py::ssize_t> shape) {
  Arr<T> a(shape);
  std::memset(a.mutable_data(), 0, sizeof(T) * (size_t)a.size());
  return a;
}

struct KContext {
  khg_ctx* h = nullptr;
  int device = 0;
  KContext(int dev, py::object stream) : device(dev) {
    void* st = stream.is_none() ? nullptr : reinterpret_cast<void*>(stream.cast<uintptr_t>());
    Check(khg_ctx_create(dev, st, &h));
  }
  ~KContext() { close(); }
  void close() { if (h) { khg_ctx_destroy(h); h = nullptr; } }
  void sync() { Check(NoGil([&] { return khg_ctx_sync(h); })); }
  void set_timing(bool on) { Check(khg_ctx_set_timing(h, on ? 1 : 0)); }
  void set_k1_form(const std::string& f) {
    int v = f == "auto" ? KHG_K1_AUTO : (f == "pdf" || f == "fp32") ? KHG_K1_FP32_PDF : f == "utt" ? KHG_K1_FP32_UTT : f == "f16x2" ? KHG_K1_F16X2 : f == "f16x2s" ? KHG_K1_F16X2S : -1;
    if (v < 0) throw py::key_error(f);
    Check(khg_ctx_set_k1_form(h, v));
  }
  static int opt_id(const py::object& o) {
    if (py::isinstance<py::int_>(o)) return o.cast<int>();
    static const char* names[KHG_OPT_COUNT] = {"k1_form", "k1_order", "k1_nf", "k1p_ts", "k1_interleave", "k1_dbg", "k2_inorder", "k2_ks", "k2_serial",
                                               "k2_prof", "k3_bucket", "k3_form", "k3_phase_b", "k3_ny", "debug", "k3_phase_a", "k2_split", "k2s_hub", "lat_ops_lds", "k1_launch", "k1_pgrid", "k1_prof"};
    const std::string n = o.cast<std::string>();
    for (int i = 0; i < KHG_OPT_COUNT; ++i) if (n == names[i]) return i;
    if (n == "scratch_bytes") return KHG_INFO_SCRATCH_BYTES;
    if (n == "scratch_blocks") return KHG_INFO_SCRATCH_BLOCKS;
    throw py::key_error(n);
  }
  int get_option(py::object name) { int v = 0; Check(khg_ctx_get_option(h, opt_id(name), &v)); return v; }
  int set_option(py::object name, int value) {
    const int id = opt_id(name);
    int old = 0;
    Check(khg_ctx_get_option(h, id, &old));
    Check(khg_ctx_set_option(h, id, value));
    return old;
  }
  py::list timings() {
    const int cap = 4096;
    std::vector<char> names(1 << 16);
    std::vector<float> ms(cap);
    int32_t n = 0;
    Check(khg_ctx_get_timings(h, names.data(), (int64_t)names.size(), ms.data(), cap, &n));
    py::list out;
    const char* p = names.data();
    for (int i = 0; i < n && i < cap; ++i) {
      const char* e = std::strchr(p, '\n');
      std::string nm = e ? std::string(p, e) : std::string(p);
      out.append(py::make_tuple(nm, ms[i]));
      if (!e) break;
      p = e + 1;
    }
    return out;
  }
};

struct KComm {
  void* h = nullptr;
  int nranks = 1, rank = 0;
  static py::bytes unique_id() {
    char id[KHG_COMM_ID_BYTES];
    Check(khg_comm_unique_id(id));
    return py::bytes(id, KHG_COMM_ID_BYTES);
  }
  KComm(KContext& ctx, int n, int r, py::bytes uid) : nranks(n), rank(r) {
    std::string s = uid;
    if (s.size() != KHG_COMM_ID_BYTES) throw py::value_error("Comm: the id is 128 bytes");
    Check(NoGil([&] { return khg_comm_create(ctx.h, n, r, s.data(), &h); }));
  }
  py::dict info() {
    int32_t n = 0, r = -1, v = 0;
    Check(khg_comm_info(h, &n, &r, &v));
    py::dict d;
    d["nranks"] = n; d["rank"] = r; d["version"] = v;
    return d;
  }
  ~KComm() { close(); }
  void close() { if (h) { khg_comm_destroy(h); h = nullptr; } }
};

struct KAccs;

struct KModel {
  khg_model* h = nullptr;
  py::object ctx_obj;
  KContext* ctx;
  int num_pdfs = 0, dim = 0;
  Arr<int32_t> gauss_off;
  KModel(py::object ctx_o, Arr<int32_t> go, Arr<float> gc, Arr<float> miv, Arr<float> iv, py::object weights)
      : ctx_obj(ctx_o), ctx(ctx_o.cast<KContext*>()), gauss_off(go) {
    num_pdfs = (int)go.shape(0) - 1;
    if (miv.ndim() != 2 || iv.ndim() != 2 || miv.shape(0) != iv.shape(0) || miv.shape(1) != iv.shape(1) || num_pdfs < 1 ||
        miv.shape(0) != go.at(num_pdfs) || gc.shape(0) != miv.shape(0))
      throw py::value_error("DeviceModel: inconsistent shapes");
    dim = (int)miv.shape(1);
    Check(khg_model_create(ctx->h, num_pdfs, dim, go.data(), gc.data(), miv.data(), iv.data(), &h));
    if (!weights.is_none()) set_weights(weights.cast<Arr<float>>());
  }
  ~KModel() { close(); }
  void close() { if (h) { khg_model_destroy(h); h = nullptr; } }
  int64_t sumG() const { return gauss_off.at(num_pdfs); }
  void set_weights(Arr<float> w) {
    if (w.shape(0) != sumG()) throw py::value_error("set_weights: one weight per Gaussian");
    Check(khg_model_set_weights(ctx->h, h, w.data()));
  }
  py::dict mle_update(KAccs& accs, py::object opts, int flags);
// ... 351 lines not shown
    Arr<int32_t> keys({K1, (py::ssize_t)N + 1});
    Arr<double> cnt({K1}), x({K1, (py::ssize_t)dim}), x2({K1, (py::ssize_t)dim});
    Check(NoGil([&] { return khg_tree_stats_download(ctx->h, h, keys.mutable_data(), cnt.mutable_data(), x.mutable_data(), x2.mutable_data()); }));
    py::dict d;
    const py::slice sl(0, K, 1);
    d["keys"] = py::array(keys)[sl]; d["count"] = py::array(cnt)[sl]; d["x"] = py::array(x)[sl]; d["x2"] = py::array(x2)[sl];
    return d;
  }
  void upload(Arr<int32_t> keys, Arr<double> cnt, Arr<double> x, Arr<double> x2) {
    const py::ssize_t K = cnt.size();
    if (keys.size() != K * (N + 1) || x.size() != K * dim || x2.size() != K * dim)
      throw py::value_error("DeviceTreeStats.upload: keys [num_keys, N + 1], count [num_keys], x and x2 [num_keys, dim]");
    Check(NoGil([&] { return khg_tree_stats_upload(ctx->h, h, (int64_t)K, keys.data(), cnt.data(), x.data(), x2.data()); }));
  }
  void add(float scale, KTreeStats& src) { Check(NoGil([&] { return khg_tree_stats_add(ctx->h, h, scale, src.h); })); }
};

struct KUtts {
  khg_utts* h = nullptr;
  py::object ctx_obj, keep, keep_model;
  KContext* ctx;
  Arr<int64_t> frame_off;
  int n_utt = 0, dim = 0;
  int64_t state_total = 0;
  KUtts(py::object ctx_o, py::object tm, Arr<int64_t> fo, py::object feats, py::object dim_o, py::object graphs, py::object graph)
      : ctx_obj(ctx_o), ctx(ctx_o.cast<KContext*>()), frame_off(fo) {
    if (!graphs.is_none() && !graph.is_none()) throw py::value_error("UtteranceSet: exactly one of graphs / graph");
    n_utt = (int)fo.shape(0) - 1;
    const float* feats_h = nullptr;
    const float* feats_d = nullptr;
    Arr<float> fh;
    if (py::isinstance<py::tuple>(feats)) {
      py::tuple t = feats;
      feats_d = reinterpret_cast<const float*>(t[0].cast<uintptr_t>());
      keep = t[1];
      if (dim_o.is_none()) throw py::value_error("UtteranceSet: dim is required with device features");
      dim = dim_o.cast<int>();
    } else {
      fh = feats.cast<Arr<float>>();
      if (fh.ndim() != 2 || fh.shape(0) != fo.at(n_utt)) throw py::value_error("UtteranceSet: feats must be [frames, dim]");
      dim = (int)fh.shape(1);
      feats_h = fh.data();
    }
    const khg_tm* tmh = tm.is_none() ? nullptr : tm.cast<KTransitions*>()->h;
    if (!graph.is_none()) {
      khg_graph* gh = reinterpret_cast<khg_graph*>(graph.attr("h").cast<uintptr_t>());
      if (!gh) throw py::value_error("UtteranceSet: the DecodingGraph is closed");
      Check(khg_utts_create_on_graph(ctx->h, tmh, gh, n_utt, dim, fo.data(), feats_h, feats_d, &h));
      state_total = graph.attr("num_states").cast<int64_t>() * n_utt;
    } else if (graphs.is_none()) {
      Check(khg_utts_create(ctx->h, tmh, n_utt, dim, fo.data(), feats_h, feats_d, nullptr, nullptr, nullptr, nullptr, nullptr, nullptr,
                            nullptr, nullptr, &h));
    } else {
      py::dict g = graphs;
      auto so = g["state_off"].cast<Arr<int64_t>>(); auto st = g["start"].cast<Arr<int32_t>>();
      auto ao = g["arc_off"].cast<Arr<int64_t>>(); auto il = g["ilabel"].cast<Arr<int32_t>>();
      auto ol = g["olabel"].cast<Arr<int32_t>>(); auto w = g["weight"].cast<Arr<float>>();
      auto ns = g["nextstate"].cast<Arr<int32_t>>(); auto fin = g["final"].cast<Arr<float>>();
      Check(khg_utts_create(ctx->h, tmh, n_utt, dim, fo.data(), feats_h, feats_d, so.data(), st.data(), ao.data(), il.data(), ol.data(),
                            w.data(), ns.data(), fin.data(), &h));
      state_total = so.at(n_utt);
    }
  }
  ~KUtts() { close(); }
  void close() { if (h) { khg_utts_destroy(h); h = nullptr; } }
  void set_pdf_list(Arr<int32_t> p) { Check(khg_utts_set_pdf_list(h, (int32_t)p.shape(0), p.data())); }
  void features_changed() { Check(khg_utts_features_changed(h)); }
  py::tuple pdf_lists() {
    Arr<int64_t> off({(py::ssize_t)n_utt + 1});
    Check(khg_utts_num_pdfs(h, off.mutable_data()));
    const py::ssize_t n = off.at(n_utt);
    Arr<int32_t> pdfs({n > 0 ? n : 1});
    Check(khg_utts_pdfs(h, pdfs.mutable_data()));
    return py::make_tuple(off, py::array(pdfs)[py::slice(0, n, 1)]);
  }
  py::dict k2_plan(py::object ctx_o) {
    int32_t o[8];
    Check(khg_utts_k2_plan(ctx_o.cast<KContext*>()->h, h, o));
    py::dict d;
    d["KS"] = o[0]; d["DEG"] = o[1]; d["FAST"] = o[2] != 0; d["GMEM"] = o[3] != 0; d["SC"] = o[4] != 0;
    d["nthr"] = o[5]; d["lds_bytes"] = o[6]; d["faithful_form"] = o[7];
    return d;
  }
  py::object pdf_first_frames() {
    Arr<int64_t> off({(py::ssize_t)n_utt + 1});
    Check(khg_utts_num_pdfs(h, off.mutable_data()));
    const py::ssize_t n = off.at(n_utt);
    Arr<int32_t> first({n > 0 ? n : 1});
    Check(khg_utts_pdf_first(h, first.mutable_data()));
    return py::array(first)[py::slice(0, n, 1)];
  }
  py::object pdf_last_frames() {
    Arr<int64_t> off({(py::ssize_t)n_utt + 1});
    Check(khg_utts_num_pdfs(h, off.mutable_data()));
    const py::ssize_t n = off.at(n_utt);
    Arr<int32_t> last({n > 0 ? n : 1});
    Check(khg_utts_pdf_last(h, last.mutable_data()));
    return py::array(last)[py::slice(0, n, 1)];
  }
  void loglikes(KModel& m, bool reachable_only, bool band) {
    keep_model = band ? py::cast(&m) : py::object();
    Check(NoGil([&] { return band ? khg_loglikes_band(ctx->h, m.h, h) : reachable_only ? khg_loglikes_reachable(ctx->h, m.h, h) : khg_loglikes(ctx->h, m.h, h); }));
  }
  py::tuple loglikes_layout() {
    Arr<int64_t> off({(py::ssize_t)n_utt + 1});
    int64_t tot = 0;
    Check(khg_loglikes_layout(h, off.mutable_data(), &tot));
    return py::make_tuple(off, tot);
  }
  py::list download_loglikes() {
    Arr<int64_t> off({(py::ssize_t)n_utt + 1}), poff({(py::ssize_t)n_utt + 1});
    int64_t tot = 0;
    Check(khg_loglikes_layout(h, off.mutable_data(), &tot));
    Check(khg_utts_num_pdfs(h, poff.mutable_data()));
    std::vector<float> buf((size_t)(tot > 0 ? tot : 1));
    Check(NoGil([&] { return khg_loglikes_download(ctx->h, h, buf.data()); }));
    py::list out;
    for (int u = 0; u < n_utt; ++u) {
      const int64_t T = frame_off.at(u + 1) - frame_off.at(u), tpad = (T + 31) / 32 * 32, n = poff.at(u + 1) - poff.at(u);
      Arr<float> m({(py::ssize_t)n, (py::ssize_t)T});
      for (int64_t j = 0; j < n; ++j) std::memcpy(m.mutable_data() + j * T, buf.data() + off.at(u) + j * tpad, sizeof(float) * (size_t)T);
      out.append(m);
    }
    return out;
  }
  void upload_loglikes(py::list mats) {
    Arr<int64_t> off({(py::ssize_t)n_utt + 1});
    int64_t tot = 0;
    Check(khg_loglikes_layout(h, off.mutable_data(), &tot));
    std::vector<float> buf((size_t)(tot > 0 ? tot : 1), 0.0f);
    for (int u = 0; u < n_utt && u < (int)mats.size(); ++u) {
      Arr<float> m = mats[u].cast<Arr<float>>();
      const int64_t T = frame_off.at(u + 1) - frame_off.at(u), tpad = (T + 31) / 32 * 32;
      for (py::ssize_t j = 0; j < m.shape(0); ++j) std::memcpy(buf.data() + off.at(u) + j * tpad, m.data() + j * m.shape(1), sizeof(float) * (size_t)T);
    }
    Check(NoGil([&] { return khg_loglikes_upload(ctx->h, h, buf.data()); }));
  }
  py::dict decode_lattice_faster(KTransitions& tm, float beam, int32_t max_active, int32_t min_active, float lattice_beam, int32_t prune_interval,
                                 float beam_delta, float hash_ratio, float prune_scale, float acoustic_scale, bool allow_partial, int32_t scratch_per_frame) {
    khg_lattice_faster_config c;
    khg_lattice_faster_config_default(&c);
    c.beam = beam; c.max_active = max_active; c.min_active = min_active; c.lattice_beam = lattice_beam; c.prune_interval = prune_interval;
    c.beam_delta = beam_delta; c.hash_ratio = hash_ratio; c.prune_scale = prune_scale; c.acoustic_scale = acoustic_scale;
    c.allow_partial = allow_partial ? 1 : 0; c.scratch_per_frame = scratch_per_frame;
    const int64_t N = frame_off.at(n_utt), wcap = 2 * N + 1024 * (int64_t)n_utt + 1024;
    Arr<int32_t> ali({(py::ssize_t)(N > 0 ? N : 1)}), words({(py::ssize_t)wcap}), status({(py::ssize_t)n_utt});
    Arr<int64_t> woff({(py::ssize_t)n_utt + 1});
    Arr<double> like({(py::ssize_t)n_utt});
    Check(NoGil([&] { return khg_decode_lattice_faster(ctx->h, tm.h, h, &c, ali.mutable_data(), words.mutable_data(), woff.mutable_data(), wcap,
                                                       like.mutable_data(), status.mutable_data()); }));
    py::dict d;
    d["ali"] = py::array(ali)[py::slice(0, N, 1)];
    d["like"] = like; d["status"] = status;
    d["words"] = py::array(words)[py::slice(0, woff.at(n_utt), 1)];
    d["words_off"] = woff;
    return d;
  }
  py::dict raw_lattice_faster_impl(KTransitions& tm, float beam, int32_t max_active, int32_t min_active, float lattice_beam, int32_t prune_interval,
                                   float beam_delta, float hash_ratio, float prune_scale, float acoustic_scale, bool allow_partial,
                                   int32_t scratch_per_frame, bool device) {
    khg_lattice_faster_config c;
    khg_lattice_faster_config_default(&c);
    c.beam = beam; c.max_active = max_active; c.min_active = min_active; c.lattice_beam = lattice_beam; c.prune_interval = prune_interval;
    c.beam_delta = beam_delta; c.hash_ratio = hash_ratio; c.prune_scale = prune_scale; c.acoustic_scale = acoustic_scale;
    c.allow_partial = allow_partial ? 1 : 0; c.scratch_per_frame = scratch_per_frame;
    const int64_t N = frame_off.at(n_utt), wcap = 2 * N + 1024 * (int64_t)n_utt + 1024;
// ... 225 lines not shown
    float* od = out.is_none() ? nullptr : reinterpret_cast<float*>(out.cast<uintptr_t>());
    Check(NoGil([&] { return khg_utts_transform_feats(ctx->h, h, n_spk, utt2spk.data(), wh, wd, od); }));
  }
};

}

void BindHost(py::module_& m, py::object* error_class);

PYBIND11_MODULE(_kaldi_hmm_gmm_amd, m) {
  m.doc() = "pybind11 host surface of libkhg_hip.so (include/khg_hip.h): the accelerated EM hot path of kaldi-hmm-gmm on MI355X";
  m.def("_set_error_class", [](py::object cls) { g_khg_error = cls; });
  BindHost(m, &g_khg_error);
  m.def("version", [] { return khg_version(); });
  m.attr("ALIGN_DONE") = KHG_ALIGN_DONE; m.attr("ALIGN_ERROR") = KHG_ALIGN_ERROR; m.attr("ALIGN_RETRIED") = KHG_ALIGN_RETRIED;
  m.attr("ALIGN_EXACT_DP") = KHG_ALIGN_EXACT_DP; m.attr("ALIGN_FALLBACK") = KHG_ALIGN_FALLBACK;

  py::class_<KContext>(m, "Context")
      .def(py::init<int, py::object>(), py::arg("device") = 0, py::arg("stream") = py::none())
      .def_property_readonly("h", [](KContext& c) { return reinterpret_cast<uintptr_t>(c.h); })
      .def_readonly("device", &KContext::device)
      .def("sync", &KContext::sync).def("set_timing", &KContext::set_timing).def("timings", &KContext::timings)
      .def("set_k1_form", &KContext::set_k1_form).def("set_option", &KContext::set_option, py::arg("name"), py::arg("value"))
      .def("get_option", &KContext::get_option, py::arg("name")).def("close", &KContext::close);

  py::class_<KComm>(m, "Comm")
      .def_static("unique_id", &KComm::unique_id)
      .def(py::init<KContext&, int, int, py::bytes>(), py::arg("ctx"), py::arg("nranks"), py::arg("rank"), py::arg("uid"), py::keep_alive<1, 2>())
      .def_property_readonly("h", [](KComm& c) { return reinterpret_cast<uintptr_t>(c.h); })
      .def_readonly("nranks", &KComm::nranks).def_readonly("rank", &KComm::rank).def("close", &KComm::close).def("info", &KComm::info)
      .def_property_readonly_static("ID_BYTES", [](py::object) { return KHG_COMM_ID_BYTES; });

  py::class_<KModel>(m, "DeviceModel")
      .def(py::init<py::object, Arr<int32_t>, Arr<float>, Arr<float>, Arr<float>, py::object>(), py::arg("ctx"), py::arg("gauss_off"),
           py::arg("gconsts"), py::arg("means_invvars"), py::arg("inv_vars"), py::arg("weights") = py::none())
      .def_property_readonly("h", [](KModel& x) { return reinterpret_cast<uintptr_t>(x.h); })
      .def_readonly("ctx", &KModel::ctx_obj).def_readonly("num_pdfs", &KModel::num_pdfs).def_readonly("dim", &KModel::dim)
      .def_readonly("gauss_off", &KModel::gauss_off)
      .def("set_weights", &KModel::set_weights)
      .def("mle_update", &KModel::mle_update, py::arg("accs"), py::arg("opts") = py::none(), py::arg("flags") = 0x7)
      .def("mle_update_sharded", &KModel::mle_update_sharded, py::arg("accs"), py::arg("opts") = py::none(), py::arg("flags") = 0x7,
           py::arg("comm") = py::none())
      .def("mle_update_range", &KModel::mle_update_range, py::arg("accs"), py::arg("opts"), py::arg("flags"), py::arg("first_pdf"), py::arg("n_pdf"))
      .def("mle_rows_download", &KModel::mle_rows_download).def("mle_rows_upload", &KModel::mle_rows_upload)
      .def("mle_update_finish", &KModel::mle_update_finish)
      .def("ebw_update", &KModel::ebw_update, py::arg("num_accs"), py::arg("den_accs"), py::arg("opts") = py::none(),
           py::arg("weight_opts") = py::none(), py::arg("flags") = 0x7)
      .def("scale_weights", &KModel::scale_weights)
      .def("invalidate", &KModel::invalidate)
      .def("transform_means", &KModel::transform_means, py::arg("M"))
      .def("split", &KModel::split, py::arg("targets"), py::arg("perturb_factor"), py::arg("randn"))
      .def("merge", &KModel::merge, py::arg("targets"))
      .def("download", &KModel::download, py::arg("weights") = true)
      .def("close", &KModel::close);

  py::class_<KTransitions>(m, "DeviceTransitions")
      .def(py::init<py::object, Arr<int32_t>>(), py::arg("ctx"), py::arg("id2pdf"))
      .def_property_readonly("h", [](KTransitions& x) { return reinterpret_cast<uintptr_t>(x.h); })
      .def_readonly("ctx", &KTransitions::ctx_obj).def_readonly("id2pdf", &KTransitions::id2pdf).def_readonly("num_tids", &KTransitions::num_tids)
      .def("set_trans_cost", &KTransitions::set_trans_cost).def("close", &KTransitions::close);

  py::class_<KAccs>(m, "DeviceAccs")
      .def(py::init<py::object, KModel&, KTransitions&>(), py::arg("ctx"), py::arg("model"), py::arg("tm"))
      .def_property_readonly("h", [](KAccs& x) { return reinterpret_cast<uintptr_t>(x.h); })
      .def_readonly("ctx", &KAccs::ctx_obj).def_readonly("sumG", &KAccs::sumG).def_readonly("dim", &KAccs::dim)
      .def_readonly("num_tids", &KAccs::num_tids).def_readonly("size", &KAccs::size)
      .def("zero", &KAccs::zero).def("device_ptr", &KAccs::device_ptr)
      .def("allreduce", &KAccs::allreduce, py::arg("comm") = py::none(), py::arg("wire_fp32") = false)
      .def("allreduce_range", &KAccs::allreduce_range, py::arg("model"), py::arg("first_pdf"), py::arg("n_pdf"), py::arg("comm") = py::none())
      .def("split", &KAccs::split).def("relayout", &KAccs::relayout).def("download_range", &KAccs::download_range)
      .def("download_occ", [](KAccs& a) { return a.download_range(0, a.sumG); })
      .def("download_trans", &KAccs::download_trans).def("download", &KAccs::download).def("upload", &KAccs::upload)
      .def("add", &KAccs::add, py::arg("scale"), py::arg("src")).def("scale", &KAccs::scale, py::arg("f"))
      .def("smooth_with_accum", &KAccs::smooth_with_accum, py::arg("tau"), py::arg("src"), py::arg("model"), py::arg("count") = true)
      .def("close", &KAccs::close);

  py::class_<KUtts>(m, "UtteranceSet")
      .def(py::init<py::object, py::object, Arr<int64_t>, py::object, py::object, py::object, py::object>(), py::arg("ctx"), py::arg("tm"), py::arg("frame_off"),
           py::arg("feats"), py::arg("dim") = py::none(), py::arg("graphs") = py::none(), py::arg("graph") = py::none())
      .def_property_readonly("graph_bytes", [](KUtts& x) { int64_t b = 0; Check(khg_utts_graph_bytes(x.h, &b)); return b; })
      .def_property_readonly("h", [](KUtts& x) { return reinterpret_cast<uintptr_t>(x.h); })
      .def_readonly("ctx", &KUtts::ctx_obj).def_readonly("frame_off", &KUtts::frame_off).def_readonly("n_utt", &KUtts::n_utt)
      .def_readonly("dim", &KUtts::dim)
      .def("set_pdf_list", &KUtts::set_pdf_list).def("features_changed", &KUtts::features_changed).def("pdf_lists", &KUtts::pdf_lists).def("k2_plan", &KUtts::k2_plan, py::arg("ctx")).def("pdf_first_frames", &KUtts::pdf_first_frames)
      .def("pdf_last_frames", &KUtts::pdf_last_frames)
      .def("loglikes", &KUtts::loglikes, py::arg("model"), py::arg("reachable_only") = false, py::arg("band") = false)
      .def("loglikes_layout", &KUtts::loglikes_layout).def("download_loglikes", &KUtts::download_loglikes)
      .def("upload_loglikes", &KUtts::upload_loglikes)
      .def("align", &KUtts::align, py::arg("tm"), py::arg("beam") = 200.0f, py::arg("retry_beam") = 0.0f, py::arg("acoustic_scale") = 1.0f,
           py::arg("careful") = false, py::arg("max_active") = (int64_t)std::numeric_limits<int32_t>::max(), py::arg("min_active") = 20,
           py::arg("beam_delta") = 0.5f, py::arg("hash_ratio") = 2.0f, py::arg("download") = true)
      .def("decode_lattice_faster", &KUtts::decode_lattice_faster, py::arg("tm"), py::arg("beam") = 16.0f,
           py::arg("max_active") = std::numeric_limits<int32_t>::max(), py::arg("min_active") = 200, py::arg("lattice_beam") = 10.0f,
           py::arg("prune_interval") = 25, py::arg("beam_delta") = 0.5f, py::arg("hash_ratio") = 2.0f, py::arg("prune_scale") = 0.1f,
           py::arg("acoustic_scale") = 1.0f, py::arg("allow_partial") = true, py::arg("scratch_per_frame") = 0)
      .def("raw_lattice_faster", &KUtts::raw_lattice_faster, py::arg("tm"), py::arg("beam") = 16.0f,
           py::arg("max_active") = std::numeric_limits<int32_t>::max(), py::arg("min_active") = 200, py::arg("lattice_beam") = 10.0f,
           py::arg("prune_interval") = 25, py::arg("beam_delta") = 0.5f, py::arg("hash_ratio") = 2.0f, py::arg("prune_scale") = 0.1f,
           py::arg("acoustic_scale") = 1.0f, py::arg("allow_partial") = true, py::arg("scratch_per_frame") = 0)
      .def("raw_lattices_faster_device", &KUtts::raw_lattices_faster_device, py::arg("tm"), py::arg("beam") = 16.0f,
           py::arg("max_active") = std::numeric_limits<int32_t>::max(), py::arg("min_active") = 200, py::arg("lattice_beam") = 10.0f,
           py::arg("prune_interval") = 25, py::arg("beam_delta") = 0.5f, py::arg("hash_ratio") = 2.0f, py::arg("prune_scale") = 0.1f,
           py::arg("acoustic_scale") = 1.0f, py::arg("allow_partial") = true, py::arg("scratch_per_frame") = 0)
      .def("decode_lattice_simple", &KUtts::decode_lattice_simple, py::arg("tm"), py::arg("beam") = 16.0f, py::arg("lattice_beam") = 10.0f,
           py::arg("prune_interval") = 25, py::arg("prune_scale") = 0.1f, py::arg("acoustic_scale") = 1.0f, py::arg("allow_partial") = true,
           py::arg("scratch_per_frame") = 0)
      .def("raw_lattice_simple", &KUtts::raw_lattice_simple, py::arg("tm"), py::arg("beam") = 16.0f, py::arg("lattice_beam") = 10.0f,
           py::arg("prune_interval") = 25, py::arg("prune_scale") = 0.1f, py::arg("acoustic_scale") = 1.0f, py::arg("scratch_per_frame") = 0)
      .def("raw_lattices_simple_device", &KUtts::raw_lattices_simple_device, py::arg("tm"), py::arg("beam") = 16.0f, py::arg("lattice_beam") = 10.0f,
           py::arg("prune_interval") = 25, py::arg("prune_scale") = 0.1f, py::arg("acoustic_scale") = 1.0f, py::arg("scratch_per_frame") = 0)
      .def("upload_ali", &KUtts::upload_ali).def("download_ali", &KUtts::download_ali)
      .def("acc_stats", &KUtts::acc_stats, py::arg("model"), py::arg("tm"), py::arg("accs"), py::arg("weight") = 1.0f)
      .def("acc_stats_post", &KUtts::acc_stats_post, py::arg("model"), py::arg("tm"), py::arg("post"), py::arg("accs"), py::arg("scale") = 1.0f)
      .def("acc_stats_post2", &KUtts::acc_stats_post2, py::arg("model"), py::arg("tm"), py::arg("post"), py::arg("num_accs"), py::arg("den_accs"),
           py::arg("scale") = 1.0f)
      .def("acc_stats_reduce", &KUtts::acc_stats_reduce, py::arg("model"), py::arg("tm"), py::arg("accs"), py::arg("weight") = 1.0f,
           py::arg("comm") = py::none(), py::arg("nparts") = 4)
      .def("acc_fmllr_stats_post", &KUtts::acc_fmllr_stats_post, py::arg("model"), py::arg("tm"), py::arg("post"), py::arg("utt2spk"), py::arg("stats"),
           py::arg("scale") = 1.0f)
      .def("acc_mllt_stats_post", &KUtts::acc_mllt_stats_post, py::arg("model"), py::arg("tm"), py::arg("post"), py::arg("stats"), py::arg("scale") = 1.0f)
      .def("acc_lda_stats_post", &KUtts::acc_lda_stats_post, py::arg("tm"), py::arg("post"), py::arg("stats"), py::arg("scale") = 1.0f)
      .def("_acc_tree_stats", &KUtts::acc_tree_stats, py::arg("tid2phone"), py::arg("tid2pdf_class"), py::arg("tid_flags"), py::arg("ci_phones"), py::arg("stats"))
      .def("splice_transform_feats", &KUtts::splice_transform_feats, py::arg("left"), py::arg("right"), py::arg("M"), py::arg("out"))
      .def("transform_feats", &KUtts::transform_feats, py::arg("utt2spk"), py::arg("W"), py::arg("out") = py::none(), py::arg("n_spk") = 0)
      .def("close", &KUtts::close);

  py::class_<KFmllrStats>(m, "DeviceFmllrStats")
      .def(py::init<py::object, int, int>(), py::arg("ctx"), py::arg("n_spk"), py::arg("dim"))
      .def_property_readonly("h", [](KFmllrStats& x) { return reinterpret_cast<uintptr_t>(x.h); })
      .def_readonly("ctx", &KFmllrStats::ctx_obj).def_readonly("n_spk", &KFmllrStats::n_spk).def_readonly("dim", &KFmllrStats::dim)
      .def("zero", &KFmllrStats::zero).def("download", &KFmllrStats::download)
      .def("upload", &KFmllrStats::upload, py::arg("beta"), py::arg("K"), py::arg("G"))
      .def("add", &KFmllrStats::add, py::arg("scale"), py::arg("src"))
      .def("estimate", &KFmllrStats::estimate, py::arg("min_count") = 500.0, py::arg("num_iters") = 40, py::arg("W_d") = py::none())
      .def("set_chunk_frames", &KFmllrStats::set_chunk_frames, py::arg("frames")).def("num_chunks", &KFmllrStats::num_chunks)
      .def("close", &KFmllrStats::close);

  py::class_<KMlltStats>(m, "DeviceMlltStats")
      .def(py::init<py::object, int>(), py::arg("ctx"), py::arg("dim"))
      .def_property_readonly("h", [](KMlltStats& x) { return reinterpret_cast<uintptr_t>(x.h); })
      .def_readonly("ctx", &KMlltStats::ctx_obj).def_readonly("dim", &KMlltStats::dim)
      .def("zero", &KMlltStats::zero).def("download", &KMlltStats::download)
      .def("upload", &KMlltStats::upload, py::arg("beta"), py::arg("G"))
      .def("add", &KMlltStats::add, py::arg("scale"), py::arg("src"))
      .def("set_chunk_frames", &KMlltStats::set_chunk_frames, py::arg("frames")).def("num_chunks", &KMlltStats::num_chunks)
      .def("close", &KMlltStats::close);

  py::class_<KLdaStats>(m, "DeviceLdaStats")
      .def(py::init<py::object, int, int, int, int>(), py::arg("ctx"), py::arg("num_classes"), py::arg("dim"), py::arg("left") = 4, py::arg("right") = 4)
      .def_property_readonly("h", [](KLdaStats& x) { return reinterpret_cast<uintptr_t>(x.h); })
      .def_readonly("ctx", &KLdaStats::ctx_obj).def_readonly("num_classes", &KLdaStats::num_classes).def_readonly("dim", &KLdaStats::dim)
      .def_readonly("left", &KLdaStats::left).def_readonly("right", &KLdaStats::right).def_readonly("dim_z", &KLdaStats::dim_z)
      .def("zero", &KLdaStats::zero).def("download", &KLdaStats::download)
      .def("upload", &KLdaStats::upload, py::arg("zero_acc"), py::arg("first_acc"), py::arg("total_second_acc"))
      .def("add", &KLdaStats::add, py::arg("scale"), py::arg("src"))
      .def("set_chunk_frames", &KLdaStats::set_chunk_frames, py::arg("frames")).def("num_chunks", &KLdaStats::num_chunks)
      .def("close", &KLdaStats::close);

  py::class_<KTreeStats>(m, "DeviceTreeStats", py::dynamic_attr())
      .def(py::init<py::object, int, int, int>(), py::arg("ctx"), py::arg("dim"), py::arg("N") = 3, py::arg("P") = 1)
      .def_property_readonly("h", [](KTreeStats& x) { return reinterpret_cast<uintptr_t>(x.h); })
      .def_readonly("ctx", &KTreeStats::ctx_obj).def_readonly("dim", &KTreeStats::dim).def_readonly("N", &KTreeStats::N).def_readonly("P", &KTreeStats::P)
      .def("zero", &KTreeStats::zero).def("num_keys", &KTreeStats::num_keys).def("download", &KTreeStats::download)
      .def("upload", &KTreeStats::upload, py::arg("keys"), py::arg("count"), py::arg("x"), py::arg("x2"))
      .def("add", &KTreeStats::add, py::arg("scale"), py::arg("src"))
      .def("close", &KTreeStats::close);

// ... 124 lines not shown
```

### kaldi_hmm_gmm_amd/csrc/khg_utts.hip

```cpp
#include "khg_internal.hpp"

static void plan_ll(khg_utts* u) {
  u->ll_off.assign(u->n_utt + 1, 0);
  for (int i = 0; i < u->n_utt; ++i) {
    int64_t T = u->frame_off[i + 1] - u->frame_off[i];
    int64_t tpad = (T + 31) & ~int64_t(31);
    u->ll_off[i + 1] = u->ll_off[i] + (u->pdf_off[i + 1] - u->pdf_off[i]) * tpad;
  }
  u->ll_total = u->ll_off[u->n_utt];
}

struct GraphTables {
  std::vector<int64_t> in_off;
  std::vector<int32_t> in_src, in_col, in_tid, in_ol, out_inidx;
  std::vector<float> in_w;
  void size(int64_t NS, int64_t NA) {
    in_off.assign((size_t)NS + 1, 0);
    in_src.resize((size_t)NA); in_col.resize((size_t)NA); in_tid.resize((size_t)NA); in_ol.resize((size_t)NA); out_inidx.resize((size_t)NA);
    in_w.resize((size_t)NA);
  }
};
struct GraphFacts {
  int32_t max_indeg = 0, max_outdeg = 0;
  bool same_col = true, has_eps = false;
  int64_t nwords = 0;
  std::vector<int32_t> pdfs, pdf_first, pdf_dfin;
};
static int plan_graph(const std::string& where, const khg_tm* tm, bool aligner_limits, int64_t s0, int64_t S, int32_t start,
                      const int64_t* arc_off, const int32_t* ilabel, const int32_t* olabel, const float* weight, const int32_t* nextstate,
                      const float* final_w, GraphTables* gt, GraphFacts* gf, std::string* msg) {
  auto fail = [&](int code, const std::string& m) { *msg = m; return code; };
  const int64_t a0 = arc_off[s0], a1 = arc_off[s0 + S], A = a1 - a0;
  if (S < 0 || A < 0) return fail(KHG_E_ARG, where + ": offsets not monotone");
  if (start >= S) return fail(KHG_E_ARG, where + ": start state out of range");
  if (aligner_limits && S > 65535) return fail(KHG_E_UNSUPPORTED, where + ": more than 65535 states in one decoding graph");
  if (S > INT32_MAX / 2 || A > INT32_MAX / 2) return fail(KHG_E_UNSUPPORTED, where + ": decoding graph too large");
  for (int64_t s = 0; s < S; ++s) gf->max_outdeg = std::max<int32_t>(gf->max_outdeg, (int32_t)(arc_off[s0 + s + 1] - arc_off[s0 + s]));
  std::vector<int32_t>& tmp_pdfs = gf->pdfs;
  tmp_pdfs.clear();
  for (int64_t a = a0; a < a1; ++a) {
    int l = ilabel[a];
    if (l < 0 || l > tm->num_tids)
      return fail(KHG_E_RUNTIME, "AddTransitionProbs: invalid symbol " + std::to_string(l) + " on graph input side.");
    if (l >= 1) tmp_pdfs.push_back(tm->id2pdf[l]); else gf->has_eps = true;
    if (nextstate[a] < 0 || nextstate[a] >= S) return fail(KHG_E_ARG, where + ": nextstate out of range");
    if (olabel[a] != 0) ++gf->nwords;
  }
  std::sort(tmp_pdfs.begin(), tmp_pdfs.end());
  tmp_pdfs.erase(std::unique(tmp_pdfs.begin(), tmp_pdfs.end()), tmp_pdfs.end());
  if (tmp_pdfs.size() > 32767) return fail(KHG_E_UNSUPPORTED, where + ": more than 32767 distinct pdfs on one decoding graph");
  {
    std::vector<int32_t> dmin((size_t)S, INT32_MAX);
    if (start >= 0) {
      std::deque<int32_t> q;
      dmin[start] = 0; q.push_back(start);
      while (!q.empty()) {
        const int s = q.front(); q.pop_front();
        for (int64_t a = arc_off[s0 + s]; a < arc_off[s0 + s + 1]; ++a) {
          const int d = nextstate[a], wgt = ilabel[a] >= 1 ? 1 : 0;
          if (dmin[s] + wgt < dmin[d]) {
            dmin[d] = dmin[s] + wgt;
            if (wgt) q.push_back(d); else q.push_front(d);
          }
        }
      }
    }
    std::vector<int32_t> dfin((size_t)S, INT32_MAX);
    {
      std::vector<int64_t> roff((size_t)S + 1, 0);
      for (int64_t a = a0; a < a1; ++a) roff[(size_t)nextstate[a] + 1]++;
      for (int64_t s = 0; s < S; ++s) roff[(size_t)s + 1] += roff[(size_t)s];
      std::vector<int32_t> rsrc((size_t)A), rw((size_t)A), rc_((size_t)S, 0);
      for (int64_t s = 0; s < S; ++s)
        for (int64_t a = arc_off[s0 + s]; a < arc_off[s0 + s + 1]; ++a) {
          const size_t pos = (size_t)(roff[(size_t)nextstate[a]] + rc_[(size_t)nextstate[a]]++);
          rsrc[pos] = (int32_t)s; rw[pos] = ilabel[a] >= 1 ? 1 : 0;
        }
      std::deque<int32_t> q;
      for (int64_t s = 0; s < S; ++s)
        if (final_w[s0 + s] != std::numeric_limits<float>::infinity()) { dfin[(size_t)s] = 0; q.push_back((int32_t)s); }
      while (!q.empty()) {
        const int d = q.front(); q.pop_front();
        for (int64_t k = roff[(size_t)d]; k < roff[(size_t)d + 1]; ++k) {
          const int s = rsrc[(size_t)k], wgt = rw[(size_t)k];
          if (dfin[(size_t)d] + wgt < dfin[(size_t)s]) {
            dfin[(size_t)s] = dfin[(size_t)d] + wgt;
            if (wgt) q.push_back(s); else q.push_front(s);
          }
        }
      }
    }
    gf->pdf_first.assign(tmp_pdfs.size(), INT32_MAX);
    gf->pdf_dfin.assign(tmp_pdfs.size(), INT32_MAX);
    for (int64_t s = 0; s < S; ++s) {
      if (dmin[s] == INT32_MAX) continue;
      for (int64_t a = arc_off[s0 + s]; a < arc_off[s0 + s + 1]; ++a) {
        if (ilabel[a] < 1) continue;
        const size_t j = (size_t)(std::lower_bound(tmp_pdfs.begin(), tmp_pdfs.end(), tm->id2pdf[ilabel[a]]) - tmp_pdfs.begin());
        gf->pdf_first[j] = std::min(gf->pdf_first[j], dmin[s]);
        gf->pdf_dfin[j] = std::min(gf->pdf_dfin[j], dfin[(size_t)nextstate[a]]);
      }
    }
  }
  std::vector<int64_t>& in_off = gt->in_off;
  for (int64_t a = a0; a < a1; ++a) in_off[s0 + nextstate[a] + 1]++;
  in_off[s0] = a0;
  for (int64_t s = 0; s < S; ++s) {
    if (aligner_limits && in_off[s0 + s + 1] > 254) return fail(KHG_E_UNSUPPORTED, where + ": a state has more than 254 incoming arcs");
    gf->max_indeg = std::max<int32_t>(gf->max_indeg, (int32_t)in_off[s0 + s + 1]);
    in_off[s0 + s + 1] += in_off[s0 + s];
  }
  std::vector<int32_t> cursor((size_t)S, 0);
  for (int64_t s = 0; s < S; ++s) {
    for (int64_t a = arc_off[s0 + s]; a < arc_off[s0 + s + 1]; ++a) {
      int d = nextstate[a];
      int64_t pos = in_off[s0 + d] + cursor[d]++;
      gt->in_src[pos] = (int32_t)s;
      gt->in_tid[pos] = ilabel[a];
      gt->in_ol[pos] = olabel[a];
      gt->in_w[pos] = weight[a];
      int col = -1;
      if (ilabel[a] >= 1)
        col = (int)(std::lower_bound(tmp_pdfs.begin(), tmp_pdfs.end(), tm->id2pdf[ilabel[a]]) - tmp_pdfs.begin());
      gt->in_col[pos] = col;
      gt->out_inidx[a] = (int32_t)(pos - a0);
    }
  }
  for (int64_t s = 0; s < S && gf->same_col; ++s)
    for (int64_t k = in_off[s0 + s] + 1; k < in_off[s0 + s + 1]; ++k)
      if (gt->in_col[k] != gt->in_col[in_off[s0 + s]]) { gf->same_col = false; break; }
  return KHG_OK;
}

static void plan_utt_on_graph(khg_utts* u, int i, int64_t T, int64_t S, const GraphFacts& gf) {
  u->pdf_off[i + 1] = u->pdf_off[i] + (int64_t)gf.pdfs.size();
  u->pdfs.insert(u->pdfs.end(), gf.pdfs.begin(), gf.pdfs.end());
  u->pdf_first.insert(u->pdf_first.end(), gf.pdf_first.begin(), gf.pdf_first.end());
  for (size_t j = 0; j < gf.pdfs.size(); ++j) {
    const int32_t first = gf.pdf_first[j], df = gf.pdf_dfin[j];
    u->pdf_last.push_back(first == INT32_MAX || df == INT32_MAX ? -1 : (int32_t)std::max<int64_t>(-1, T - 1 - df));
  }
  u->bp_off[i + 1] = u->bp_off[i] + std::max<int64_t>((T + 1) * std::max<int64_t>((S + 15) & ~int64_t(15), 512), ((T >> 3) + 1) * (S + 256) * 4);
  u->path_off[i + 1] = u->path_off[i] + T + S + 8;
  u->words_off[i + 1] = u->words_off[i] + gf.nwords;
}

static int utts_begin(const char* where, khg_ctx* ctx, int32_t n_utt, int32_t D, const int64_t* frame_off, const float* feats_h,
                      const float* feats_dv, bool small_graphs, khg_utts** out) {
  if (frame_off[0] != 0) return khg_set_error(KHG_E_ARG, std::string(where) + ": frame_off[0] != 0");
  for (int i = 0; i < n_utt; ++i)
    if (frame_off[i + 1] < frame_off[i]) return khg_set_error(KHG_E_ARG, std::string(where) + ": frame_off not monotone");
  khg_utts* u = new khg_utts();
  u->ctx = ctx; u->n_utt = n_utt; u->D = D;
  u->frame_off.assign(frame_off, frame_off + n_utt + 1);
  u->N = frame_off[n_utt];
  u->small = n_utt <= 16 && u->N <= 16384 && u->N * (int64_t)D <= (int64_t)(512 << 10) && small_graphs;
  int rc = KHG_OK;
  auto fail = [&](int code, const std::string& msg) { khg_utts_destroy(u); return khg_set_error(code, msg); };
  if (feats_dv) { u->feats_d = feats_dv; u->own_feats = false; }
  else {
    float* p = nullptr;
    rc = u_alloc(u, &p, (size_t)u->N * D);
    if (rc) { khg_utts_destroy(u); return rc; }
    u->feats_d = p; u->own_feats = true;
    if (u->N) {
      const size_t nb = sizeof(float) * (size_t)u->N * D;
      if (ctx->arena.owns(p)) { memcpy(ctx->arena.mirror(p), feats_h, nb); arena_mark_dirty(ctx, p, nb); }
      else {
        hipError_t e = hipMemcpyAsync(p, feats_h, nb, hipMemcpyHostToDevice, ctx->stream);
        if (e != hipSuccess) return fail(KHG_E_HIP, hipGetErrorString(e));
        ctx->pageable_pending = true;
      }
    }
    if (u->small && u->N > 0) {
      u->xmax.assign((size_t)D, 0.0f);
      for (int64_t t = 0; t < u->N; ++t) {
        const float* x = feats_h + (size_t)t * D;
        for (int d = 0; d < D; ++d) {
          const float v = x[d], m = u->xmax[(size_t)d];
          if (v == -std::numeric_limits<float>::infinity()) continue;
          u->xmax[(size_t)d] = (std::fabs(v) <= 3.0e38f) ? std::fmax(m, std::fabs(v)) : std::numeric_limits<float>::infinity();
        }
      }
    }
  }
  rc = u_upload(ctx, u, &u->frame_off_d, u->frame_off);
  if (rc) { khg_utts_destroy(u); return rc; }
  u->pdf_off.assign(n_utt + 1, 0);
  *out = u;
  return KHG_OK;
}
static int utts_finish(khg_ctx* ctx, khg_utts* u, khg_utts** out) {
  plan_ll(u);
  int rc = arena_flush(ctx);
  if (!rc) rc = sync_pageable(ctx);
  if (rc) { khg_utts_destroy(u); return rc; }
  *out = u;
  return KHG_OK;
}
static int64_t graph_table_bytes(int64_t rows, int64_t NS, int64_t NA) { return 8 * (rows + 1) + 4 * rows + 2 * 8 * (NS + 1) + 6 * 4 * NA + 4 * NS; }

extern "C" int khg_utts_create(khg_ctx* ctx, const khg_tm* tm, int32_t n_utt, int32_t D,
                               const int64_t* frame_off, const float* feats_h, const float* feats_dv,
                               const int64_t* state_off, const int32_t* start, const int64_t* arc_off,
                               const int32_t* ilabel, const int32_t* olabel, const float* weight,
                               const int32_t* nextstate, const float* final_w, khg_utts** out) {
  if (ctx_dead(ctx) || !out || n_utt <= 0 || D <= 0 || !frame_off || (!feats_h && !feats_dv))
    return khg_set_error(KHG_E_ARG, "khg_utts_create: bad arguments");
  khg_utts* u = nullptr;
  int rc = utts_begin("khg_utts_create", ctx, n_utt, D, frame_off, feats_h, feats_dv,
                      !state_off || (state_off[n_utt] <= 32768 && arc_off && arc_off[state_off[n_utt]] <= 65536), &u);
  if (rc) return rc;
  auto fail = [&](int code, const std::string& msg) { khg_utts_destroy(u); return khg_set_error(code, msg); };

  if (state_off && state_off[n_utt] > 0) {
    if (!tm || !start || !arc_off || !ilabel || !olabel || !weight || !nextstate || !final_w)
      return fail(KHG_E_ARG, "khg_utts_create: graph arrays / tm missing");
    u->has_graphs = true;
    u->state_off.assign(state_off, state_off + n_utt + 1);
    const int64_t NS = state_off[n_utt], NA = arc_off[NS];
    std::vector<int64_t> out_off(arc_off, arc_off + NS + 1);
    GraphTables gt;
    gt.size(NS, NA);
    u->bp_off.assign(n_utt + 1, 0); u->path_off.assign(n_utt + 1, 0); u->words_off.assign(n_utt + 1, 0);
    std::string msg;
    for (int i = 0; i < n_utt; ++i) {
      const int64_t s0 = state_off[i], S = state_off[i + 1] - s0;
      const int64_t T = frame_off[i + 1] - frame_off[i];
      GraphFacts gf;
      rc = plan_graph("khg_utts_create", tm, true, s0, S, start[i], arc_off, ilabel, olabel, weight, nextstate, final_w, &gt, &gf, &msg);
      if (rc) return fail(rc, msg);
      u->max_states = std::max<int64_t>(u->max_states, S);
      u->max_inarcs = std::max<int64_t>(u->max_inarcs, arc_off[s0 + S] - arc_off[s0]);
      u->max_outdeg = std::max(u->max_outdeg, gf.max_outdeg);
      u->max_indeg = std::max(u->max_indeg, gf.max_indeg);
      u->has_eps = u->has_eps || gf.has_eps;
      u->same_col = u->same_col && gf.same_col;
      plan_utt_on_graph(u, i, T, S, gf);
    }
    gt.in_off[NS] = NA;
    std::vector<int32_t> startv(start, start + n_utt), gidx((size_t)n_utt);
    for (int i = 0; i < n_utt; ++i) gidx[(size_t)i] = i;
    std::vector<float> finalv(final_w, final_w + NS);
    rc = u_upload(ctx, u, &u->state_off_d, u->state_off);
    if (!rc) rc = u_upload(ctx, u, &u->start_d, startv);
    if (!rc) rc = u_upload(ctx, u, &u->gidx_d, gidx);
    if (!rc) rc = u_upload(ctx, u, &u->in_off_d, gt.in_off);
    if (!rc) rc = u_upload(ctx, u, &u->out_off_d, out_off);
    if (!rc) rc = u_upload(ctx, u, &u->in_src_d, gt.in_src);
    if (!rc) rc = u_upload(ctx, u, &u->in_col_d, gt.in_col);
    if (!rc) rc = u_upload(ctx, u, &u->in_tid_d, gt.in_tid);
    if (!rc) rc = u_upload(ctx, u, &u->in_olabel_d, gt.in_ol);
    if (!rc) rc = u_upload(ctx, u, &u->out_inidx_d, gt.out_inidx);
    if (!rc) rc = u_upload(ctx, u, &u->in_w_d, gt.in_w);
    if (!rc) rc = u_upload(ctx, u, &u->final_d, finalv);
    if (!rc) rc = u_upload(ctx, u, &u->bp_off_d, u->bp_off);
    if (!rc) rc = u_upload(ctx, u, &u->path_off_d, u->path_off);
    if (!rc) rc = u_upload(ctx, u, &u->words_off_d, u->words_off);
    if (rc) { khg_utts_destroy(u); return rc; }
    u->graph_bytes = graph_table_bytes(n_utt, NS, NA);
  }
  return utts_finish(ctx, u, out);
}

extern "C" int khg_graph_create(khg_ctx* ctx, const khg_tm* tm, int32_t num_states, int32_t start, const int64_t* arc_off,
                                const int32_t* ilabel, const int32_t* olabel, const float* weight, const int32_t* nextstate,
                                const float* final_w, khg_graph** out) {
  if (ctx_dead(ctx) || !out || num_states <= 0)
    return khg_set_error(KHG_E_ARG, "khg_graph_create: bad arguments");
  if (!tm || !arc_off || !ilabel || !olabel || !weight || !nextstate || !final_w)
    return khg_set_error(KHG_E_ARG, "khg_graph_create: graph arrays / tm missing");
  const int64_t S = num_states, A = arc_off[S] - arc_off[0];
  if (arc_off[0] != 0) return khg_set_error(KHG_E_ARG, "khg_graph_create: arc_off[0] != 0");
  for (int64_t s = 0; s < S; ++s)
    if (arc_off[s + 1] < arc_off[s]) return khg_set_error(KHG_E_ARG, "khg_graph_create: offsets not monotone");
  GraphTables gt;
  gt.size(S, A);
  GraphFacts gf;
  std::string msg;
  int rc = plan_graph("khg_graph_create", tm, false, 0, S, start, arc_off, ilabel, olabel, weight, nextstate, final_w, &gt, &gf, &msg);
  if (rc) return khg_set_error(rc, msg);
  gt.in_off[S] = A;
  khg_graph* g = new khg_graph();
  g->ctx = ctx; g->S = S; g->A = A; g->start = start; g->nwords = gf.nwords;
  g->max_indeg = gf.max_indeg; g->max_outdeg = gf.max_outdeg; g->same_col = gf.same_col; g->has_eps = gf.has_eps;
  g->pdfs = gf.pdfs; g->pdf_first = gf.pdf_first; g->pdf_dfin = gf.pdf_dfin;
  std::vector<int64_t> so{0, S}, out_off(arc_off, arc_off + S + 1);
  std::vector<int32_t> startv{start};
  std::vector<float> finalv(final_w, final_w + S);
  rc = dev_upload(ctx, &g->state_off_d, so);
  if (!rc) rc = dev_upload(ctx, &g->start_d, startv);
  if (!rc) rc = dev_upload(ctx, &g->in_off_d, gt.in_off);
  if (!rc) rc = dev_upload(ctx, &g->out_off_d, out_off);
  if (!rc) rc = dev_upload(ctx, &g->in_src_d, gt.in_src);
  if (!rc) rc = dev_upload(ctx, &g->in_col_d, gt.in_col);
  if (!rc) rc = dev_upload(ctx, &g->in_tid_d, gt.in_tid);
  if (!rc) rc = dev_upload(ctx, &g->in_olabel_d, gt.in_ol);
  if (!rc) rc = dev_upload(ctx, &g->out_inidx_d, gt.out_inidx);
  if (!rc) rc = dev_upload(ctx, &g->in_w_d, gt.in_w);
  if (!rc) rc = dev_upload(ctx, &g->final_d, finalv);
  if (!rc) rc = sync_pageable(ctx);
  if (rc) { khg_graph_release(g); return rc; }
  g->device_bytes = graph_table_bytes(1, S, A);
  *out = g;
  return KHG_OK;
}
void khg_graph_release(khg_graph* g) {
  if (!g || --g->refs > 0) return;
  DEVFREE(g->state_off_d); DEVFREE(g->start_d); DEVFREE(g->in_off_d); DEVFREE(g->out_off_d); DEVFREE(g->in_src_d); DEVFREE(g->in_col_d);
  DEVFREE(g->in_tid_d); DEVFREE(g->in_olabel_d); DEVFREE(g->out_inidx_d); DEVFREE(g->in_w_d); DEVFREE(g->final_d);
  delete g;
}
extern "C" int khg_graph_destroy(khg_graph* g) {
  khg_graph_release(g);
  return KHG_OK;
}
extern "C" int khg_graph_info(const khg_graph* g, int64_t* num_states, int64_t* num_arcs, int32_t* num_pdfs, int32_t* max_in_degree,
                              int64_t* device_bytes) {
  if (!g) return khg_set_error(KHG_E_ARG, "khg_graph_info: bad arguments");
  if (num_states) *num_states = g->S;
  if (num_arcs) *num_arcs = g->A;
  if (num_pdfs) *num_pdfs = (int32_t)g->pdfs.size();
  if (max_in_degree) *max_in_degree = g->max_indeg;
  if (device_bytes) *device_bytes = g->device_bytes;
  return KHG_OK;
}

extern "C" int khg_utts_create_on_graph(khg_ctx* ctx, const khg_tm* tm, khg_graph* g, int32_t n_utt, int32_t D, const int64_t* frame_off,
                                        const float* feats_h, const float* feats_dv, khg_utts** out) {
  (void)tm;
  if (ctx_dead(ctx) || !out || !g || n_utt <= 0 || D <= 0 || !frame_off || (!feats_h && !feats_dv))
    return khg_set_error(KHG_E_ARG, "khg_utts_create_on_graph: bad arguments");
  if (g->ctx != ctx)
    return khg_set_error(KHG_E_ARG, "khg_utts_create_on_graph: a decoding graph must be used with the context that created it");
  khg_utts* u = nullptr;
  int rc = utts_begin("khg_utts_create_on_graph", ctx, n_utt, D, frame_off, feats_h, feats_dv, g->S <= 32768 && g->A <= 65536, &u);
  if (rc) return rc;
  u->has_graphs = true;
  u->graph = g; ++g->refs;
  u->state_off.assign({0, g->S});
  u->max_states = (int32_t)g->S; u->max_inarcs = (int32_t)g->A; u->max_indeg = g->max_indeg; u->max_outdeg = g->max_outdeg;
  u->has_eps = g->has_eps; u->same_col = g->same_col;
  u->bp_off.assign(n_utt + 1, 0); u->path_off.assign(n_utt + 1, 0); u->words_off.assign(n_utt + 1, 0);
  GraphFacts gf;
  gf.pdfs = g->pdfs; gf.pdf_first = g->pdf_first; gf.pdf_dfin = g->pdf_dfin; gf.nwords = g->nwords;
  for (int i = 0; i < n_utt; ++i) plan_utt_on_graph(u, i, frame_off[i + 1] - frame_off[i], g->S, gf);
  u->state_off_d = g->state_off_d; u->start_d = g->start_d; u->in_off_d = g->in_off_d; u->out_off_d = g->out_off_d;
  u->in_src_d = g->in_src_d; u->in_col_d = g->in_col_d; u->in_tid_d = g->in_tid_d; u->in_olabel_d = g->in_olabel_d;
  u->out_inidx_d = g->out_inidx_d; u->in_w_d = g->in_w_d; u->final_d = g->final_d;
  std::vector<int32_t> gidx((size_t)n_utt, 0);
  rc = u_upload(ctx, u, &u->gidx_d, gidx);
  if (!rc) rc = u_upload(ctx, u, &u->bp_off_d, u->bp_off);
  if (!rc) rc = u_upload(ctx, u, &u->path_off_d, u->path_off);
  if (!rc) rc = u_upload(ctx, u, &u->words_off_d, u->words_off);
  if (rc) { khg_utts_destroy(u); return rc; }
  return utts_finish(ctx, u, out);
}
extern "C" int khg_utts_graph_bytes(const khg_utts* u, int64_t* bytes) {
  if (!u || !bytes) return khg_set_error(KHG_E_ARG, "khg_utts_graph_bytes: bad arguments");
  *bytes = u->graph_bytes;
  return KHG_OK;
}

extern "C" int khg_utts_set_pdf_list(khg_utts* u, int32_t n, const int32_t* pdfs) {
  if (!u || n <= 0 || !pdfs) return khg_set_error(KHG_E_ARG, "khg_utts_set_pdf_list: bad arguments");
  if (u->has_graphs) return khg_set_error(KHG_E_ARG, "khg_utts_set_pdf_list: set has graphs; its pdf lists come from them");
  u->pdfs.clear();
  u->pdf_first.clear(); u->pdf_last.clear();
  for (int i = 0; i < u->n_utt; ++i) { u->pdf_off[i + 1] = u->pdf_off[i] + n; u->pdfs.insert(u->pdfs.end(), pdfs, pdfs + n); }
  plan_ll(u);
  DEVFREE(u->pdf_off_d); DEVFREE(u->pdfs_d); DEVFREE(u->ll_off_d); DEVFREE(u->ll_d); DEVFREE(u->chunks_d); DEVFREE(u->wchunks_d);
  DEVFREE(u->tile_off_d); DEVFREE(u->tiles_d); u->tiles_pto.clear(); u->tiles_reach = -1;
  DEVFREE(u->p_ents_d); DEVFREE(u->p_slices_d); u->p_reach = -1;
  DEVFREE(u->sunits_d); u->sunits_pto.clear(); u->sunits_reach = -1;
  u->pdfs_checked_P = -1;
  u->ll_valid = false;
  return KHG_OK;
}

extern "C" int khg_utts_features_changed(khg_utts* u) {
  if (!u) return khg_set_error(KHG_E_ARG, "khg_utts_features_changed: bad arguments");
  u->xmax.clear();
  u->xs_ks = 0; u->xs_ex.clear();
  u->xh_ks = 0; u->xh_ex.clear();
  u->ll_valid = false;
  return KHG_OK;
}

int utts_foreign_ctx(const khg_ctx* ctx, const khg_utts* u, const char* where) {
  if (u && u->small && u->ctx != ctx)
    return khg_set_error(KHG_E_ARG, std::string(where) + ": a small utterance set (<= 16 utterances: scratch in its context's arena) must be used with the context that created it");
  return KHG_OK;
}

extern "C" int khg_utts_destroy(khg_utts* u) {
  if (!u) return KHG_OK;
  if (u->small && u->ctx && khg_ctx_alive(u->ctx)) {
    khg_ctx* c = u->ctx;
    for (int i = 0; i < khg_ctx::NSIDE; ++i)
      if (c->side_dirty[i]) { (void)hipStreamSynchronize(c->sides[i]); c->side_dirty[i] = false; }
    (void)hipStreamSynchronize(c->stream);
    c->pageable_pending = false;
  }
  if (u->out_blk_d) {
    u->ali_d = nullptr; u->words_d = nullptr; u->num_words_d = nullptr; u->status_d = nullptr; u->like_d = nullptr;
    DEVFREE(u->out_blk_d);
  }
  if (u->own_feats) DEVFREE(u->feats_d);
  if (u->graph) {
    u->state_off_d = nullptr; u->start_d = nullptr; u->in_off_d = nullptr; u->out_off_d = nullptr; u->in_src_d = nullptr; u->in_col_d = nullptr;
    u->in_tid_d = nullptr; u->in_olabel_d = nullptr; u->out_inidx_d = nullptr; u->in_w_d = nullptr; u->final_d = nullptr;
    khg_graph_release(u->graph); u->graph = nullptr;
  }
  DEVFREE(u->gidx_d);
  DEVFREE(u->frame_off_d); DEVFREE(u->state_off_d); DEVFREE(u->pdf_off_d); DEVFREE(u->ll_off_d);
  DEVFREE(u->pdfs_d); DEVFREE(u->wchunks_d); DEVFREE(u->start_d); DEVFREE(u->in_off_d); DEVFREE(u->out_off_d);
  DEVFREE(u->in_src_d); DEVFREE(u->in_col_d); DEVFREE(u->in_tid_d); DEVFREE(u->in_olabel_d); DEVFREE(u->out_inidx_d);
  DEVFREE(u->in_w_d); DEVFREE(u->final_d); DEVFREE(u->chunks_d); DEVFREE(u->ll_d); DEVFREE(u->tile_off_d); DEVFREE(u->tiles_d);
  DEVFREE(u->xpl_d); DEVFREE(u->utt_xtile_off_d); DEVFREE(u->p_ents_d); DEVFREE(u->p_slices_d);
  DEVFREE(u->utt_x32_off_d); DEVFREE(u->bchunks_d); DEVFREE(u->x32_utt_d); DEVFREE(u->xh_d); DEVFREE(u->xh_ex_d);
  DEVFREE(u->xs_d); DEVFREE(u->xs_ex_d); DEVFREE(u->schunks_d); DEVFREE(u->sunits_d);
  DEVFREE(u->bp_d); DEVFREE(u->bp_off_d); DEVFREE(u->path_off_d); DEVFREE(u->words_off_d);
  DEVFREE(u->ali2_d); DEVFREE(u->unc_d); DEVFREE(u->sub_off_d);
  if (u->unc_cnt_h) { (void)hipHostFree(u->unc_cnt_h); u->unc_cnt_h = nullptr; }
  DEVFREE(u->layer_best_d); DEVFREE(u->layer_cnt_d); DEVFREE(u->path_d); DEVFREE(u->k2_gscratch_d); DEVFREE(u->k2_order_d);
// ... 43 lines not shown
```

Before: 442.7 million.

## Add wavefront-pipelined ladder Viterbi DP for left-to-right chain graphs

Detects graphs whose every state has only a self-loop and an arc from the previous state. For these it adds a K2 Viterbi variant that processes frames in groups of eight as a diagonal wavefront across waves. The previous-state value comes from a DPP lane shift, and wave boundaries pass through small LDS hand-off buffers. This replaces the per-frame block-wide sync with one sync per group step, and per-layer min/count reductions are done with DPP and accumulated across waves. It adds a new template instantiation and an option to disable it, and risks subtle tie-breaking or boundary bugs.

Measured after the change: 447.4 million, median of 6. +1.1%, better.

```diff
diff --git a/include/khg_hip.h b/include/khg_hip.h
--- a/include/khg_hip.h
+++ b/include/khg_hip.h
@@ -58,7 +58,8 @@
 #define KHG_OPT_K1_LAUNCH 19
 #define KHG_OPT_K1_PGRID 20
 #define KHG_OPT_K1_PROF 21
-#define KHG_OPT_COUNT 22
+#define KHG_OPT_K2_LADDER 22
+#define KHG_OPT_COUNT 23
 #define KHG_INFO_SCRATCH_BYTES 100
 #define KHG_INFO_SCRATCH_BLOCKS 101
 int khg_ctx_set_option(khg_ctx *ctx, int option, int value);
@@ -95,6 +96,7 @@
 int khg_utts_num_pdfs(const khg_utts *u, int64_t *pdf_off_h );
 int khg_utts_pdfs(const khg_utts *u, int32_t *pdfs_h );
 int khg_utts_k2_plan(khg_ctx *ctx, const khg_utts *u, int32_t out[8]);
+int khg_utts_k2_ladder(khg_ctx *ctx, const khg_utts *u, int32_t *out);
 int khg_utts_pdf_first(const khg_utts *u, int32_t *first_h );
 
 int khg_loglikes(khg_ctx *ctx, const khg_model *m, khg_utts *u);
diff --git a/kaldi_hmm_gmm_amd/_lib.py b/kaldi_hmm_gmm_amd/_lib.py
--- a/kaldi_hmm_gmm_amd/_lib.py
+++ b/kaldi_hmm_gmm_amd/_lib.py
@@ -147,6 +147,7 @@
     "khg_utts_num_pdfs": (C.c_int, [vp, c_i64p]),
     "khg_utts_pdfs": (C.c_int, [vp, c_i32p]),
     "khg_utts_k2_plan": (C.c_int, [vp, vp, c_i32p]),
+    "khg_utts_k2_ladder": (C.c_int, [vp, vp, c_i32p]),
     "khg_utts_pdf_first": (C.c_int, [vp, c_i32p]),
     "khg_loglikes": (C.c_int, [vp, vp, vp]),
     "khg_loglikes_reachable": (C.c_int, [vp, vp, vp]),
diff --git a/kaldi_hmm_gmm_amd/csrc/khg_ctx_model.hip b/kaldi_hmm_gmm_amd/csrc/khg_ctx_model.hip
--- a/kaldi_hmm_gmm_amd/csrc/khg_ctx_model.hip
+++ b/kaldi_hmm_gmm_amd/csrc/khg_ctx_model.hip
@@ -157,7 +157,7 @@
   return KHG_OK;
 }
 static const struct { int lo, hi; } k_opt_range[KHG_OPT_COUNT] = {
-  {KHG_K1_AUTO, KHG_K1_F16X2S}, {0, 4}, {0, 6}, {0, 1 << 20}, {-1, 1}, {0, 255}, {0, 1}, {0, 4}, {0, 3}, {0, 1}, {0, 2}, {0, 2}, {0, 2}, {0, 64}, {0, 1}, {0, 1}, {0, 1}, {0, 1 << 20}, {0, 1}, {0, 2}, {0, 1 << 16}, {0, 1}};
+  {KHG_K1_AUTO, KHG_K1_F16X2S}, {0, 4}, {0, 6}, {0, 1 << 20}, {-1, 1}, {0, 255}, {0, 1}, {0, 4}, {0, 3}, {0, 1}, {0, 2}, {0, 2}, {0, 2}, {0, 64}, {0, 1}, {0, 1}, {0, 1}, {0, 1 << 20}, {0, 1}, {0, 2}, {0, 1 << 16}, {0, 1}, {0, 1}};
 extern "C" int khg_option_check(int opt, int value) {
   if (opt < 0 || opt >= KHG_OPT_COUNT) return khg_set_error(KHG_E_ARG, "khg_option_check: no such option");
   if (value < k_opt_range[opt].lo || value > k_opt_range[opt].hi || (opt == KHG_OPT_K1_FORM && value == 1))
@@ -193,7 +193,7 @@
   {"KHG_K2_SPLIT", KHG_OPT_K2_SPLIT, "on=0,off=1"}, {"KHG_K2S_HUB", KHG_OPT_K2S_HUB, ""},
   {"KHG_LAT_OPS_LDS", KHG_OPT_LAT_OPS_LDS, "on=0,off=1"},
   {"KHG_K1_LAUNCH", KHG_OPT_K1_LAUNCH, "auto=0,chunk=1,persistent=2"}, {"KHG_K1_PGRID", KHG_OPT_K1_PGRID, ""},
-  {"KHG_K1_PROF", KHG_OPT_K1_PROF, ""}};
+  {"KHG_K1_PROF", KHG_OPT_K1_PROF, ""}, {"KHG_K2_LADDER", KHG_OPT_K2_LADDER, "on=0,off=1"}};
 extern "C" int khg_option_from_env(const char* name, const char* text, int* option, int* value) {
   if (!name || !text || !*text || !option || !value) return khg_set_error(KHG_E_ARG, "khg_option_from_env: bad arguments");
   for (const auto& t : k_env_tab) {
diff --git a/kaldi_hmm_gmm_amd/csrc/khg_internal.hpp b/kaldi_hmm_gmm_amd/csrc/khg_internal.hpp
--- a/kaldi_hmm_gmm_amd/csrc/khg_internal.hpp
+++ b/kaldi_hmm_gmm_amd/csrc/khg_internal.hpp
@@ -192,7 +192,7 @@
   int32_t refs = 1;
   int64_t S = 0, A = 0, nwords = 0, device_bytes = 0;
   int32_t start = -1, max_indeg = 0, max_outdeg = 0;
-  bool same_col = true, has_eps = false;
+  bool same_col = true, has_eps = false, ladder = true;
   std::vector<int32_t> pdfs, pdf_first, pdf_dfin;
   int64_t *state_off_d = nullptr, *in_off_d = nullptr, *out_off_d = nullptr;
   int32_t *start_d = nullptr, *in_src_d = nullptr, *in_col_d = nullptr, *in_tid_d = nullptr, *in_olabel_d = nullptr, *out_inidx_d = nullptr;
@@ -213,6 +213,7 @@
   std::vector<int32_t> pdfs;
   int32_t max_states = 0, max_inarcs = 0, max_indeg = 0, max_outdeg = 0;
   bool same_col = true;
+  bool ladder = true;
   int32_t pdfs_checked_P = -1;
   bool has_eps = false;
   const float* feats_d = nullptr; bool own_feats = false;
diff --git a/kaldi_hmm_gmm_amd/csrc/khg_k2.hip b/kaldi_hmm_gmm_amd/csrc/khg_k2.hip
--- a/kaldi_hmm_gmm_amd/csrc/khg_k2.hip
+++ b/kaldi_hmm_gmm_amd/csrc/khg_k2.hip
@@ -27,6 +27,7 @@
 struct K2Plan {
   int KS = 1, DEG = 1;
   bool FAST = false, GMEM = false, SC = false;
+  bool LAD = false;
   int nthr = 64;
   size_t lds_dp = 0;
   size_t max_npdf = 0;
@@ -97,6 +98,7 @@
   else if (KSsel == 4 && deg2m && u->same_col) form(4, 2, true);
   else if (KSsel == 4 && deg2m) form(4, 2, false);
   else if (KSsel == 4) form(4, 3, false);
+  p.LAD = p.FAST && p.KS == 1 && p.DEG == 2 && u->ladder && nthr <= 256 && ctx->opt[KHG_OPT_K2_LADDER] == 0;
   return p;
 }
 
@@ -107,6 +109,14 @@
   const K2Plan p = k2_plan(ctx, u);
   out[0] = p.KS; out[1] = p.DEG; out[2] = p.FAST ? 1 : 0; out[3] = p.GMEM ? 1 : 0; out[4] = p.SC ? 1 : 0;
   out[5] = p.nthr; out[6] = p.GMEM ? 0 : (int32_t)p.lds_dp; out[7] = p.faithful;
+  return KHG_OK;
+}
+
+extern "C" int khg_utts_k2_ladder(khg_ctx* ctx, const khg_utts* u, int32_t* out) {
+  if (ctx_dead(ctx) || !u || !out) return khg_set_error(KHG_E_ARG, "khg_utts_k2_ladder: bad arguments");
+  { int rf = utts_foreign_ctx(ctx, u, "khg_utts_k2_ladder"); if (rf) return rf; }
+  if (!u->has_graphs) return khg_set_error(KHG_E_ARG, "khg_utts_k2_ladder: the utterance set has no decoding graphs");
+  *out = k2_plan(ctx, u).LAD ? 1 : 0;
   return KHG_OK;
 }
 
@@ -203,9 +213,11 @@
     KernelTimer kt(ctx, "k2_viterbi_dp");
     KHG_LAUNCH(ctx, (k2_viterbi_dp<1, 1, false, true>), dim3(u->n_utt), dim3(nthr), 0, ctx->stream, a);
   } else {
-    const int form = plan.FAST ? 100 * plan.KS + 10 * plan.DEG + (plan.SC ? 1 : 0) : 0;
+    const int form = plan.FAST ? 100 * plan.KS + 10 * plan.DEG + (plan.SC ? 1 : 0) + (plan.LAD ? 1000 : 0) : 0;
 #define K2_DP_CASES(X)                                                                                         \
-    if (form == 160) X((k2_viterbi_dp<1, 6, true>));                                                           \
+    if (form == 1121) X((k2_viterbi_dp<1, 2, true, false, true, true>));                                       \
+    else if (form == 1120) X((k2_viterbi_dp<1, 2, true, false, false, true>));                                 \
+    else if (form == 160) X((k2_viterbi_dp<1, 6, true>));                                                      \
     else if (form == 121) X((k2_viterbi_dp<1, 2, true, false, true>));                                         \
     else if (form == 120) X((k2_viterbi_dp<1, 2, true>));                                                      \
     else if (form == 131) X((k2_viterbi_dp<1, 3, true, false, true>));                                         \
diff --git a/kaldi_hmm_gmm_amd/csrc/khg_k2_viterbi.hip.inc b/kaldi_hmm_gmm_amd/csrc/khg_k2_viterbi.hip.inc
--- a/kaldi_hmm_gmm_amd/csrc/khg_k2_viterbi.hip.inc
+++ b/kaldi_hmm_gmm_amd/csrc/khg_k2_viterbi.hip.inc
@@ -160,6 +160,12 @@
   for (int o = 32; o > 0; o >>= 1) { double t = __shfl_xor(v, o); v = t < v ? t : v; }
   return v;
 }
+template <int CTRL, int ROWMASK>
+__device__ __forceinline__ double k2_dpp_d(double old, double v) {
+  const int lo = __builtin_amdgcn_update_dpp(__double2loint(old), __double2loint(v), CTRL, ROWMASK, 0xf, false);
+  const int hi = __builtin_amdgcn_update_dpp(__double2hiint(old), __double2hiint(v), CTRL, ROWMASK, 0xf, false);
+  return __hiloint2double(hi, lo);
+}
 __device__ __forceinline__ int k2_wave_sum(int v) {
 #pragma unroll
   for (int o = 32; o > 0; o >>= 1) v += __shfl_xor(v, o);
@@ -177,8 +183,9 @@
   else { ord = nib & ((1 << NB) - 1); tie = (nib >> NB) & 1; }
 }
 
-template <int KS, int DEG, bool FAST, bool GMEM = false, bool SC = false>
+template <int KS, int DEG, bool FAST, bool GMEM = false, bool SC = false, bool LAD = false>
 __global__ __attribute__((amdgpu_waves_per_eu(KS == 1 ? K2_WAVES_PER_EU : 4))) void k2_viterbi_dp(K2Args a) {
+  static_assert(!LAD || (FAST && KS == 1 && DEG == 2 && !GMEM), "the ladder form is a variant of <1, 2, true, false, *>");
   extern __shared__ __attribute__((aligned(16))) unsigned char k2_lds[];
   unsigned char* const smem = GMEM ? a.gscratch + (size_t)blockIdx.x * a.gscratch_stride : k2_lds;
   constexpr int NS = FAST ? KS : 1;
@@ -234,6 +241,7 @@
     if (col < 0) s_flags[1] = 1;
   }
   for (int s = tid; s < S; s += nthr) cur[s] = (s == start) ? 0.0 : INFINITY;
+  if (LAD && tid < 8) s_red[tid] = INFINITY;
   k2_block_sync();
   const bool has_eps = !FAST && s_flags[1] != 0;
   const float* llu = a.ll + a.ll_off[u];
@@ -261,6 +269,14 @@
   } else {
     for (int s = tid; s < S; s += nthr) bp[s] = K2_BP_NONE;
   }
+  int lad_bit[2] = {1, 2};
+  if constexpr (LAD) {
+    if (e_src[0] != tid) {
+      const double tw = e_w[0]; e_w[0] = e_w[1]; e_w[1] = tw;
+      if (!SC) { const int tc = e_col[0]; e_col[0] = e_col[1]; e_col[1] = tc; }
+      lad_bit[0] = 2; lad_bit[1] = 1;
+    }
+  }
   if (a.prof && tid == 0) a.prof[u * 8 + 1] = clock64();
   int tie = 0;
   const double* g_even[NSD]; const double* g_odd[NSD];
@@ -291,6 +307,32 @@
     }
   }
 
+  auto score_fetch = [&](const int layer, auto subc) {
+    constexpr int SUB8 = decltype(subc)::value;
+    constexpr int SUB = SUB8 & 3;
+    if constexpr (SC3) {
+      if constexpr (SUB8 == 0) {
+#pragma unroll
+        for (int i = 0; i < NSC; ++i) sc_b[i] = sc_c[i];
+      }
+      if constexpr (SUB8 == 4) {
+#pragma unroll
+        for (int i = 0; i < NSC; ++i)
+          if (have_ll && layer + 4 < tpad) {
+            const float* src = llu + (int64_t)e_col[SC ? i * DEG : i] * tpad + layer + 4;
+            sc_a[i] = *reinterpret_cast<const f32x4*>(src);
+            sc_c[i] = *reinterpret_cast<const f32x4*>(src + 4);
+          }
+      }
+    } else if (SUB == 0) {
+#pragma unroll
+      for (int i = 0; i < NSC; ++i)
+        if (have_ll && layer + 4 < tpad) {
+          const f32x4 v = *reinterpret_cast<const f32x4*>(llu + (int64_t)e_col[SC ? i * DEG : i] * tpad + layer + 4);
+          if constexpr ((SUB8 & 4) != 0) sc_a[i] = v; else sc_b[i] = v;
+        }
+    }
+  };
   auto layer_step = [&](const int layer, auto subc) -> bool {
     constexpr int SUB8 = decltype(subc)::value;
     constexpr int SUB = SUB8 & 3;
@@ -375,28 +417,7 @@
     }
     if (layer == T) return false;
     if (FAST) {
-      if constexpr (SC3) {
-        if constexpr (SUB8 == 0) {
-#pragma unroll
-          for (int i = 0; i < NSC; ++i) sc_b[i] = sc_c[i];
-        }
-        if constexpr (SUB8 == 4) {
-#pragma unroll
-          for (int i = 0; i < NSC; ++i)
-            if (have_ll && layer + 4 < tpad) {
-              const float* src = llu + (int64_t)e_col[SC ? i * DEG : i] * tpad + layer + 4;
-              sc_a[i] = *reinterpret_cast<const f32x4*>(src);
-              sc_c[i] = *reinterpret_cast<const f32x4*>(src + 4);
-            }
-        }
-      } else if (SUB == 0) {
-#pragma unroll
-        for (int i = 0; i < NSC; ++i)
-          if (have_ll && layer + 4 < tpad) {
-            const f32x4 v = *reinterpret_cast<const f32x4*>(llu + (int64_t)e_col[SC ? i * DEG : i] * tpad + layer + 4);
-            if constexpr ((SUB8 & 4) != 0) sc_a[i] = v; else sc_b[i] = v;
-          }
-      }
+      score_fetch(layer, subc);
       double cc[NSD];
 #pragma unroll
       for (int i = 0; i < NSD; ++i) cc[i] = (SUB & 1) ? *g_odd[i] : *g_even[i];
@@ -485,7 +506,92 @@
     double* tsw = cur; cur = nxt; nxt = tsw;
     return true;
   };
-  if constexpr (FAST) {
+  if constexpr (LAD) {
+    const int ngrp = (T >> 3) + 1;
+    float* const pm = s_ac + wave * 640;
+    uint8_t* const pc = reinterpret_cast<uint8_t*>(pm + 512);
+    const double* const bin = wave == 0 ? s_red : cur + (wave - 1) * 16;
+    const int bpar = wave == 0 ? 0 : 8;
+    double* const bout = cur + wave * 16;
+    const bool pub = lane == 63 && wave + 1 < nwave;
+    float* const acc_m = s_wmin;
+    int32_t* const acc_c = s_wcnt;
+    auto vmin = [](float x, float y) { float r; asm("v_min_f32 %0, %1, %2" : "=v"(r) : "v"(x), "v"(y)); return r; };
+    for (int step = 0; step < ngrp + nwave - 1; ++step) {
+      const int g = step - wave;
+      if (g >= 0 && g < ngrp) {
+        const int base = 8 * g;
+        const double* const bi = bin + (g & 1) * bpar;
+        double* const bo = bout + (g & 1) * 8;
+        double bv[8];
+        bv[0] = bi[0]; bv[1] = bi[1];
+        auto lad_step = [&](auto subc) -> bool {
+          constexpr int SUB8 = decltype(subc)::value;
+          constexpr int SUB = SUB8 & 3;
+          const int layer = base + SUB8;
+          pm[SUB8 * 64 + lane] = (float)mine[0];
+          pc[SUB8 * 64 + lane] = (uint8_t)mine_live[0];
+          if (pub) bo[SUB8] = mine[0];
+          if (layer == T) return false;
+          if constexpr (SUB8 + 2 < 8) bv[SUB8 + 2] = bi[SUB8 + 2];
+          score_fetch(layer, subc);
+          float sc0, sc1;
+          if constexpr ((SUB8 & 4) != 0) { sc0 = sc_b[0][SUB]; sc1 = sc_b[SC ? 0 : 1][SUB]; } else { sc0 = sc_a[0][SUB]; sc1 = sc_a[SC ? 0 : 1][SUB]; }
+          const float ac0 = -1 * (a.acoustic_scale * sc0);
+          const float ac1 = SC ? ac0 : -1 * (a.acoustic_scale * sc1);
+          const double prev = k2_dpp_d<0x138, 0xf>(bv[SUB8], mine[0]);
+          const double n_self = (mine[0] + e_w[0]) + ac0;
+          const double n_prev = (prev + e_w[1]) + ac1;
+          double best = INFINITY;
+          best = __builtin_fmin(best, n_self);
+          best = __builtin_fmin(best, n_prev);
+          const bool live = __double2hiint(best) != 0x7FF00000;
+          const bool e_s = live && n_self == best, e_p = live && n_prev == best;
+          const int code = (e_s ? lad_bit[0] : 0) | (e_p ? lad_bit[1] : 0);
+          mine[0] = best;
+          mine_live[0] = live ? 1 : 0;
+          bpw[0] = (bpw[0] >> 4) | ((unsigned)code << 28);
+          const int lb = layer + 1;
+          if ((lb & 7) == 7 || lb == T) {
+            const unsigned wv = (lb & 7) == 7 ? bpw[0] : bpw[0] >> (4 * (7 - (lb & 7)));
+            reinterpret_cast<unsigned*>(bp)[(int64_t)(lb >> 3) * GW + tid] = wv;
+          }
+          return true;
+        };
+        (void)(lad_step(std::integral_constant<int, 0>{}) && lad_step(std::integral_constant<int, 1>{}) &&
+               lad_step(std::integral_constant<int, 2>{}) && lad_step(std::integral_constant<int, 3>{}) &&
+               lad_step(std::integral_constant<int, 4>{}) && lad_step(std::integral_constant<int, 5>{}) &&
+               lad_step(std::integral_constant<int, 6>{}) && lad_step(std::integral_constant<int, 7>{}));
+        const int lastsub = min(7, T - base);
+        k2_lds_sync();
+        const int ly = lane >> 3, sub = lane & 7;
+        const f32x4 m0 = *reinterpret_cast<const f32x4*>(pm + ly * 64 + sub * 8), m1 = *reinterpret_cast<const f32x4*>(pm + ly * 64 + sub * 8 + 4);
+        const uint2 cb = *reinterpret_cast<const uint2*>(pc + ly * 64 + sub * 8);
+        float m = vmin(vmin(vmin(m0[0], m0[1]), vmin(m0[2], m0[3])), vmin(vmin(m1[0], m1[1]), vmin(m1[2], m1[3])));
+        int cn = (int)__builtin_amdgcn_sad_u8(cb.y, 0u, __builtin_amdgcn_sad_u8(cb.x, 0u, 0u));
+        m = vmin(m, __int_as_float(__builtin_amdgcn_update_dpp(0, __float_as_int(m), 0xB1, 0xf, 0xf, false)));
+        cn += __builtin_amdgcn_update_dpp(0, cn, 0xB1, 0xf, 0xf, false);
+        m = vmin(m, __int_as_float(__builtin_amdgcn_update_dpp(0, __float_as_int(m), 0x4E, 0xf, 0xf, false)));
+        cn += __builtin_amdgcn_update_dpp(0, cn, 0x4E, 0xf, 0xf, false);
+        m = vmin(m, __int_as_float(__builtin_amdgcn_update_dpp(0, __float_as_int(m), 0x141, 0xf, 0xf, false)));
+        cn += __builtin_amdgcn_update_dpp(0, cn, 0x141, 0xf, 0xf, false);
+        if (sub == 0 && ly <= lastsub) {
+          const int sl = (g & 3) * 8 + ly;
+          if (wave > 0) { m = vmin(m, acc_m[sl]); cn += acc_c[sl]; }
+          if (wave + 1 < nwave) {
+            acc_m[sl] = m; acc_c[sl] = cn;
+          } else {
+            if (m == INFINITY) { if (cn > 0) m = 3.402823466e38f; }
+            else m = __int_as_float(__float_as_int(m) + (m > 0.0f ? -1 : (m < 0.0f ? 1 : (int)0x80000001)));
+            lbest[base + ly] = (double)m;
+            lcnt[base + ly] = cn;
+          }
+        }
+      }
+      k2_block_sync();
+    }
+    if (tid < S) cur[tid] = mine[0];
+  } else if constexpr (FAST) {
     for (int base = 0; base <= T; base += 8) {
       if (!layer_step(base, std::integral_constant<int, 0>{})) break;
       if (!layer_step(base + 1, std::integral_constant<int, 1>{})) break;
@@ -1551,12 +1657,6 @@
 
 struct K2ChainArc { float w; int16_t col; uint16_t dst; };
 
-template <int CTRL, int ROWMASK>
-__device__ __forceinline__ double k2_dpp_d(double old, double v) {
-  const int lo = __builtin_amdgcn_update_dpp(__double2loint(old), __double2loint(v), CTRL, ROWMASK, 0xf, false);
-  const int hi = __builtin_amdgcn_update_dpp(__double2hiint(old), __double2hiint(v), CTRL, ROWMASK, 0xf, false);
-  return __hiloint2double(hi, lo);
-}
 __device__ __forceinline__ double k2_scan_min_d(double v) {
   const double inf = INFINITY;
   v = __builtin_fmin(v, k2_dpp_d<0x111, 0xf>(inf, v));
diff --git a/kaldi_hmm_gmm_amd/csrc/khg_pybind.cpp b/kaldi_hmm_gmm_amd/csrc/khg_pybind.cpp
--- a/kaldi_hmm_gmm_amd/csrc/khg_pybind.cpp
+++ b/kaldi_hmm_gmm_amd/csrc/khg_pybind.cpp
@@ -65,7 +65,7 @@
   static int opt_id(const py::object& o) {
     if (py::isinstance<py::int_>(o)) return o.cast<int>();
     static const char* names[KHG_OPT_COUNT] = {"k1_form", "k1_order", "k1_nf", "k1p_ts", "k1_interleave", "k1_dbg", "k2_inorder", "k2_ks", "k2_serial",
-                                               "k2_prof", "k3_bucket", "k3_form", "k3_phase_b", "k3_ny", "debug", "k3_phase_a", "k2_split", "k2s_hub", "lat_ops_lds", "k1_launch", "k1_pgrid", "k1_prof"};
+                                               "k2_prof", "k3_bucket", "k3_form", "k3_phase_b", "k3_ny", "debug", "k3_phase_a", "k2_split", "k2s_hub", "lat_ops_lds", "k1_launch", "k1_pgrid", "k1_prof", "k2_ladder"};
     const std::string n = o.cast<std::string>();
     for (int i = 0; i < KHG_OPT_COUNT; ++i) if (n == names[i]) return i;
     if (n == "scratch_bytes") return KHG_INFO_SCRATCH_BYTES;
@@ -583,6 +583,11 @@
     d["nthr"] = o[5]; d["lds_bytes"] = o[6]; d["faithful_form"] = o[7];
     return d;
   }
+  bool k2_ladder(py::object ctx_o) {
+    int32_t o = 0;
+    Check(khg_utts_k2_ladder(ctx_o.cast<KContext*>()->h, h, &o));
+    return o != 0;
+  }
   py::object pdf_first_frames() {
     Arr<int64_t> off({(py::ssize_t)n_utt + 1});
     Check(khg_utts_num_pdfs(h, off.mutable_data()));
@@ -974,7 +979,7 @@
       .def_property_readonly("h", [](KUtts& x) { return reinterpret_cast<uintptr_t>(x.h); })
       .def_readonly("ctx", &KUtts::ctx_obj).def_readonly("frame_off", &KUtts::frame_off).def_readonly("n_utt", &KUtts::n_utt)
       .def_readonly("dim", &KUtts::dim)
-      .def("set_pdf_list", &KUtts::set_pdf_list).def("features_changed", &KUtts::features_changed).def("pdf_lists", &KUtts::pdf_lists).def("k2_plan", &KUtts::k2_plan, py::arg("ctx")).def("pdf_first_frames", &KUtts::pdf_first_frames)
+      .def("set_pdf_list", &KUtts::set_pdf_list).def("features_changed", &KUtts::features_changed).def("pdf_lists", &KUtts::pdf_lists).def("k2_plan", &KUtts::k2_plan, py::arg("ctx")).def("k2_ladder", &KUtts::k2_ladder, py::arg("ctx")).def("pdf_first_frames", &KUtts::pdf_first_frames)
       .def("pdf_last_frames", &KUtts::pdf_last_frames)
       .def("loglikes", &KUtts::loglikes, py::arg("model"), py::arg("reachable_only") = false, py::arg("band") = false)
       .def("loglikes_layout", &KUtts::loglikes_layout).def("download_loglikes", &KUtts::download_loglikes)
diff --git a/kaldi_hmm_gmm_amd/csrc/khg_utts.hip b/kaldi_hmm_gmm_amd/csrc/khg_utts.hip
--- a/kaldi_hmm_gmm_amd/csrc/khg_utts.hip
+++ b/kaldi_hmm_gmm_amd/csrc/khg_utts.hip
@@ -23,6 +23,7 @@
 struct GraphFacts {
   int32_t max_indeg = 0, max_outdeg = 0;
   bool same_col = true, has_eps = false;
+  bool ladder = true;
   int64_t nwords = 0;
   std::vector<int32_t> pdfs, pdf_first, pdf_dfin;
 };
@@ -129,6 +130,13 @@
   for (int64_t s = 0; s < S && gf->same_col; ++s)
     for (int64_t k = in_off[s0 + s] + 1; k < in_off[s0 + s + 1]; ++k)
       if (gt->in_col[k] != gt->in_col[in_off[s0 + s]]) { gf->same_col = false; break; }
+  gf->ladder = !gf->has_eps;
+  for (int64_t s = 0; s < S && gf->ladder; ++s) {
+    const int64_t k0 = in_off[s0 + s], n = in_off[s0 + s + 1] - k0;
+    if (n > 2 || (n == 2 && gt->in_src[k0] == gt->in_src[k0 + 1])) gf->ladder = false;
+    for (int64_t k = k0; k < k0 + n && gf->ladder; ++k)
+      if (gt->in_src[k] != s && gt->in_src[k] != s - 1) gf->ladder = false;
+  }
   return KHG_OK;
 }
 
@@ -236,6 +244,7 @@
       u->max_indeg = std::max(u->max_indeg, gf.max_indeg);
       u->has_eps = u->has_eps || gf.has_eps;
       u->same_col = u->same_col && gf.same_col;
+      u->ladder = u->ladder && gf.ladder;
       plan_utt_on_graph(u, i, T, S, gf);
     }
     gt.in_off[NS] = NA;
@@ -283,7 +292,7 @@
   gt.in_off[S] = A;
   khg_graph* g = new khg_graph();
   g->ctx = ctx; g->S = S; g->A = A; g->start = start; g->nwords = gf.nwords;
-  g->max_indeg = gf.max_indeg; g->max_outdeg = gf.max_outdeg; g->same_col = gf.same_col; g->has_eps = gf.has_eps;
+  g->max_indeg = gf.max_indeg; g->max_outdeg = gf.max_outdeg; g->same_col = gf.same_col; g->ladder = gf.ladder; g->has_eps = gf.has_eps;
   g->pdfs = gf.pdfs; g->pdf_first = gf.pdf_first; g->pdf_dfin = gf.pdf_dfin;
   std::vector<int64_t> so{0, S}, out_off(arc_off, arc_off + S + 1);
   std::vector<int32_t> startv{start};
@@ -340,7 +349,7 @@
   u->graph = g; ++g->refs;
   u->state_off.assign({0, g->S});
   u->max_states = (int32_t)g->S; u->max_inarcs = (int32_t)g->A; u->max_indeg = g->max_indeg; u->max_outdeg = g->max_outdeg;
-  u->has_eps = g->has_eps; u->same_col = g->same_col;
+  u->has_eps = g->has_eps; u->same_col = g->same_col; u->ladder = g->ladder;
   u->bp_off.assign(n_utt + 1, 0); u->path_off.assign(n_utt + 1, 0); u->words_off.assign(n_utt + 1, 0);
   GraphFacts gf;
   gf.pdfs = g->pdfs; gf.pdf_first = g->pdf_first; gf.pdf_dfin = g->pdf_dfin; gf.nwords = g->nwords;
```
